# gligen/GLIGEN

Hardware: AMD Instinct MI355X
Metric: 512x512 images/sec @ 50 PLMS steps, box+text (CFG 7.5), UNet step ms (higher is better)
Workload: dtype bf16; 1 GPU; C2: box+text, 8 boxes (30 grounding tokens), 512x512, 50 PLMS steps, CFG 7.5, bf16 storage / fp32 accumulate; plms_steps=50, unet_evals_per_image=102, hipgraph=True, batches_in_flight=3

## Files before the change

gligen_amd/_lib.py:

```python
from __future__ import annotations

import ctypes as C
from pathlib import Path

_HERE = Path(__file__).resolve().parent
LIB_PATH = _HERE / "libgligen_amd.so"


class GligenAmdError(RuntimeError):
    pass


class UNetConfig(C.Structure):
    _fields_ = [
        ("in_channels", C.c_int), ("out_channels", C.c_int), ("model_channels", C.c_int),
        ("num_res_blocks", C.c_int), ("num_heads", C.c_int), ("context_dim", C.c_int),
        ("n_mult", C.c_int), ("channel_mult", C.c_int * 8),
        ("n_attn", C.c_int), ("attention_resolutions", C.c_int * 8),
        ("inpaint_mode", C.c_int), ("grounding_kind", C.c_int),
        ("gr_in_dim", C.c_int), ("gr_out_dim", C.c_int), ("max_persons", C.c_int), ("fuser_kind", C.c_int),
        ("extra_channels", C.c_int), ("tok_resize", C.c_int), ("tok_in_dim", C.c_int),
    ]


# ... 180 lines not shown
    "gl_op_block_train_fuser": (_I, [_P, _I, _P, C.POINTER(_P), _P, _P, _P, _P, _P, _P, _P, _P, C.POINTER(_P), _P]),
    "gl_op_grid_resize": (_I, [_P, _P, _I, _I, _I, _I, _P, _P]),
    "gl_op_grid_resize_backward": (_I, [_P, _P, _I, _I, _I, _I, _P, _P]),
}

_F = C.c_float
TRAIN_PRIM_SYMBOLS = {
    "gl_op_train_attention": (_I, [_P, _I, _I, _I, _I, _I] + [_P] * 9 + [_P]),
    "gl_op_train_linear": (_I, [_P, _I, _I, _I] + [_P] * 8 + [_P]),
    "gl_op_train_layernorm": (_I, [_P, _I, _I, _F, _P, _P, _P, _P, _I] + [_P] * 6 + [_P]),
    "gl_op_train_groupnorm": (_I, [_P, _I, _I, _I, _I, _F, _P, _P, _P, _P, _I] + [_P] * 4 + [_P]),
    "gl_op_train_geglu": (_I, [_P, _I, _I, _P, _P, _P, _P, _P]),
    "gl_op_train_dot": (_I, [_P, C.c_int64, _P, _P, _P, _F, _I, _P, _P]),
}

TRAINER_SYMBOLS = {
    "gl_op_adamw_ema_step": (_I, [_P, _P, _P, _P, _P, _P, C.c_int64, C.c_double, C.c_double, C.c_double, C.c_double, C.c_double, C.c_double, _I, _P]),
}

SAMPLER_SYMBOLS = {
    "gl_set_cfg_shared_prefix": (_I, [_I]),
}

SOLVER_SYMBOLS = {
    "gl_sample_solver": (_I, [_P, C.POINTER(SolverArgs), _P]),
    "gl_op_solver_update": (_I, [_P, _P, _I, C.c_float, C.c_float, _P, _P, _P, _P, _P, _P] + [C.c_float] * 5 + [C.c_int64, _P]),
}


class GemmPlanRecord(C.Structure):
    _fields_ = [("kernel", C.c_char * 96)] + [(n, C.c_int) for n in ("family", "M", "N", "K", "tm", "tn", "splits", "grid", "n_items", "box", "rm", "rz",
                                                                     "units_per_split", "xcd")]


class AttnProjLayout(C.Structure):
    _fields_ = [(n, C.c_int) for n in ("d", "dp", "dpv", "tq", "tk", "tq_pad", "tk_pad", "vt_perm32")]


GEMM_PLAN_SYMBOLS = {
    "gl_gemm_force_plan": (_I, [_I, _I, _I, _I]),
    "gl_gemm_force_knobs": (_I, [_I, _I, _I, _I, _I, _I]),
    "gl_gemm_force_clear": (_I, []),
    "gl_gemm_plan_log_clear": (_I, []),
    "gl_gemm_plan_log": (_I, [C.POINTER(GemmPlanRecord), _I, C.POINTER(_I), C.POINTER(_I)]),
    "gl_op_attention_project": (_I, [_P, _P, _P, _I, _I, _I, _I, _I, _I, _P, _P, _P, _P, _P, _P, C.POINTER(AttnProjLayout), _P]),
}

ATTENTION_CORE_SYMBOLS = {
    "gl_op_attention_core": (_I, [_P, _P, _P, _P, C.POINTER(AttnProjLayout), _I, _I, _I, _I, _P, _I, _I, _I, _P]),
}
ATTN_CORE_KERNELS = {"auto": 0, "attn_kernel": 1, "attn2_kernel_w4": 2, "attn2_kernel_w8": 3, "attn3_kernel": 4}
GL_ERR_UNSUPPORTED = 5

VAE_SYMBOLS = {
    "gl_vae_set_attention": (_I, [_P, _I]),
    "gl_op_vae_attention": (_I, [_P, _P, _P, _P, _I, _I, _I, _I, _P, _P]),
}
VAE_ATTN_MODES = {"auto": 0, "matrix": 1, "flash": 2}

LATENT_SYMBOLS = {
    "gl_op_latent_renoise": (_I, [_P, _P, _I, _I, _I, _I, _P, _I, _I, _I, _F, _F, _P, _I, _P]),
    "gl_latent_resize_taps": (_I, [_I, _I, _I, C.POINTER(_I), C.POINTER(_F)]),
}
LATENT_RESIZE_MODES = {"nearest-exact": 0, "bilinear": 1, "bicubic": 2}

LORA_SYMBOLS = {
    "gl_op_lora_merge": (_I, [_P, _P, _P, _P, _I, _I, _I, _F, _P]),
}

FUSER_KINDS = {"gatedSA": 0, "gatedSA2": 1, "gatedCA": 2}


def fuser_kind(fuser_type) -> int:
    try:
        return FUSER_KINDS[fuser_type or "gatedSA"]
    except KeyError:
        raise ValueError(f"fuser_type {fuser_type!r}: one of {sorted(FUSER_KINDS)}") from None


_lib = None


def load() -> C.CDLL:
    global _lib
    if _lib is not None:
        return _lib
    if not LIB_PATH.exists():
        raise GligenAmdError(
            f"{LIB_PATH} not found: build it with `python -m gligen_amd.build` "
            "(gligen_amd has no fallback path without its HIP library)")
    import torch
    lib = C.CDLL(str(LIB_PATH))
    for name, (res, args) in {**SYMBOLS, **IMAGE_SYMBOLS, **MAP_SYMBOLS, **TRAIN_MAP_SYMBOLS, **TRAIN_INPUT_SYMBOLS, **TRAIN_FUSER_SYMBOLS, **TRAIN_PRIM_SYMBOLS,
                              **TRAINER_SYMBOLS, **SAMPLER_SYMBOLS, **SOLVER_SYMBOLS, **GEMM_PLAN_SYMBOLS, **ATTENTION_CORE_SYMBOLS, **VAE_SYMBOLS, **LATENT_SYMBOLS, **LORA_SYMBOLS}.items():
        fn = getattr(lib, name)
        fn.restype = res
        fn.argtypes = args
    _lib = lib
    return lib


def check(rc: int) -> None:
    if rc != 0:
        msg = load().gl_last_error()
        raise GligenAmdError(f"libgligen_amd error {rc}: {msg.decode() if msg else '?'}")
```

gligen_amd/csrc/capi.hip:

```cpp
#include "classmap.h"
#include "engine_impl.h"
#include "image.h"
#include "latent.h"
#include "lora.h"
#include "train.h"
#include "train_fusers.h"
#include "../../include/gligen_amd_train_maps.h"
#include "../../include/gligen_amd_train_inputs.h"
#include "../../include/gligen_amd_train_fusers.h"
#include "../../include/gligen_amd_train_prims.h"
#include "../../include/gligen_amd_trainer.h"
#include "../../include/gligen_amd_sampler.h"
#include "../../include/gligen_amd_gemm_plans.h"
#include "../../include/gligen_amd_attention_core.h"
#include "../../include/gligen_amd_vae.h"
#include "../../include/gligen_amd_latent.h"
#include "../../include/gligen_amd_lora.h"
#include "gemm_plan.h"

#include <cstdlib>

#include <cmath>

using namespace gl;

struct gl_ctx {
    std::shared_ptr<Engine> holder;
    Engine* eng;
    ImageStage image_stage;
};

#define GL_API_BEGIN try {
#define GL_API_END                                       \
    }                                                    \
    catch (const gl::GlError& e) {                       \
        return gl::set_error(e.code, "%s", e.what());    \
    }                                                    \
    catch (const std::exception& e) {                    \
        return gl::set_error(GL_ERR_STATE, "%s", e.what()); \
    }                                                    \
    return GL_OK;

struct DeviceGuard {
    int prev = -1;
    bool ok = true;
    explicit DeviceGuard(int dev) {
        if (hipGetDevice(&prev) != hipSuccess) prev = -1;
        if (prev != dev) ok = hipSetDevice(dev) == hipSuccess;
        else prev = -1;
    }
    ~DeviceGuard() {
        if (prev >= 0) (void)hipSetDevice(prev);
    }
};
#define NEED(ctx)                                                         \
    if (!(ctx) || !(ctx)->eng) return gl::set_error(GL_ERR_ARG, "null context"); \
    DeviceGuard device_guard_((ctx)->eng->device());                      \
    if (!device_guard_.ok) return gl::set_error(GL_ERR_HIP, "hipSetDevice(%d) failed", (ctx)->eng->device());

static inline hipStream_t S(gl_stream s) { return reinterpret_cast<hipStream_t>(s); }
#define HIPCK_API(expr)                                                                           \
    do {                                                                                          \
        hipError_t _e = (expr);                                                                   \
        if (_e != hipSuccess) throw GlError(GL_ERR_HIP, std::string(#expr) + ": " + hipGetErrorString(_e)); \
    } while (0)

extern "C" {

const char* gl_last_error(void) { return gl::last_error(); }

// ... 1092 lines not shown
        bf16* w4 = ar.get<bf16>((size_t)16 * Cout * Cin);
        const int rp = pack_upconv_phases_launch(w_oihw, w4, Cout, Cin, Cout, S(s));
        if (rp != GL_OK) throw GlError(rp, gl::last_error());
        c.w4 = w4;
        ctx->eng->conv3x3(TRef{(const bf16*)x0, C0, (const bf16*)x1, C1}, B, H, W, c, 1, 1, 1, nullptr, 0, nullptr, S(s), (bf16*)y);
        return GL_OK;
    }
    bf16* wp = ar.get<bf16>((size_t)Cout * 9 * Cin);
    int r = pack_conv_weight_launch(w_oihw, wp, Cout, Cin, 3, 3, Cout, S(s));
    if (r != GL_OK) throw GlError(r, gl::last_error());
    const int Hup = H << ups, Wup = W << ups;
    const int Ho = stride == 1 ? Hup : (pad_lo ? (Hup + 2 - 3) / 2 + 1 : (Hup + 1 - 3) / 2 + 1);
    const int Wo = stride == 1 ? Wup : (pad_lo ? (Wup + 2 - 3) / 2 + 1 : (Wup + 1 - 3) / 2 + 1);
    AOperand A{};
    A.p0 = (const bf16*)x0; A.C0 = C0; A.ld0 = C0; A.p1 = (const bf16*)x1; A.C1 = C1; A.ld1 = C1;
    A.mode = A_CONV3; A.Hin = H; A.Win = W; A.Ho = Ho; A.Wo = Wo; A.stride = stride; A.ups = ups; A.pad_lo = pad_lo;
    Epilogue E;
    epilogue_defaults(E);
    E.out = y; E.ldo = Cout; E.bias = bias; E.res = (const bf16*)res; E.ldres = Cout; E.rows_per_b = Ho * Wo;
    r = gemm_launch(A, wp, B * Ho * Wo, Cout, 9 * Cin, E, ctx->eng->splitk_ws(), ctx->eng->splitk_ws_bytes(), S(s));
    if (r != GL_OK) throw GlError(r, gl::last_error());
    GL_API_END
}

int gl_op_gn_silu_conv3x3(gl_ctx* ctx, const void* x0, int C0, const void* x1, int C1, int B, int H, int W, const float* gamma, const float* beta,
                          float eps, const float* w_oihw, const float* bias, int Cout, const float* bias2, const void* res, void* y, int mode,
                          int* used_prologue, gl_stream s) {
    NEED(ctx);
    if (!x0 || !gamma || !beta || !w_oihw || !y || !used_prologue) return gl::set_error(GL_ERR_ARG, "gl_op_gn_silu_conv3x3: null pointer");
    GL_API_BEGIN
    Engine& eng = *ctx->eng;
    Arena& ar = eng.arena();
    ar.reset();
    const int Cin = C0 + C1;
    bf16* wp = ar.get<bf16>((size_t)Cout * 9 * Cin);
    int r = pack_conv_weight_launch(w_oihw, wp, Cout, Cin, 3, 3, Cout, S(s));
    if (r != GL_OK) throw GlError(r, gl::last_error());
    NormW n;
    n.g = gamma; n.b = beta; n.C = Cin;
    ConvW c;
    c.w = wp; c.b = bias; c.Cin = Cin; c.Cout = Cout;
    const bool saved = eng.gn_prologue_;
    if (mode >= 0) eng.gn_prologue_ = mode != 0;
    const int64_t n0 = eng.n_prologue_convs;
    try {
        eng.gn_silu_conv3x3(TRef{(const bf16*)x0, C0, (const bf16*)x1, C1}, B, H, W, n, eps, c, bias2, Cout, (const bf16*)res, (bf16*)y, S(s));
    } catch (...) {
        eng.gn_prologue_ = saved;
        throw;
    }
    eng.gn_prologue_ = saved;
    *used_prologue = eng.n_prologue_convs > n0 ? 1 : 0;
    if (mode == 1 && !*used_prologue) throw GlError(GL_ERR_UNSUPPORTED, "gl_op_gn_silu_conv3x3: this shape has no GroupNorm prologue (conv_halo_kernel, H W % 256 == 0)");
    GL_API_END
}

int gl_op_groupnorm(gl_ctx* ctx, const void* x0, int C0, const void* x1, int C1, int B, int HW,
                    const float* gamma, const float* beta, float eps, int silu, void* y, gl_stream s) {
    NEED(ctx);
    GL_API_BEGIN
    Arena& ar = ctx->eng->arena();
    ar.reset();
    GNParams P{};
    P.x0 = (const bf16*)x0; P.C0 = C0; P.x1 = (const bf16*)x1; P.C1 = C1; P.B = B; P.HW = HW; P.eps = eps;
    P.gamma = gamma; P.beta = beta; P.y = (bf16*)y; P.silu = silu;
    P.partial = reinterpret_cast<float*>(ar.alloc(gn_partial_bytes(B, HW)));
    int r = groupnorm_launch(P, S(s));
    if (r != GL_OK) throw GlError(r, gl::last_error());
    GL_API_END
}

int gl_op_layernorm(gl_ctx* ctx, const void* x, const void* x2, int B, int N1, int N2, int Tpad, int C,
                    const float* gamma, const float* beta, float eps, void* y, gl_stream s) {
    NEED(ctx);
    GL_API_BEGIN
    LNParams P{};
    P.x = (const bf16*)x; P.x2 = (const bf16*)x2; P.B = B; P.N1 = N1; P.N2 = N2; P.Tpad = Tpad; P.C = C; P.eps = eps;
    P.gamma = gamma; P.beta = beta; P.y = (bf16*)y;
    int r = layernorm_launch(P, S(s));
    if (r != GL_OK) throw GlError(r, gl::last_error());
    GL_API_END
}

static void attention_project(Engine& eng, const void* xq, const void* xkv, int B, int Nq, int Nk, int C, int Ck, int H, const float* wq,
                              const float* wk, const float* wv, bf16* q, bf16* k, bf16* vt, int Tq_pad, int Tk_pad, int dp, int dpv, int vt_layout,
                              hipStream_t s) {
    Arena& ar = eng.arena();
    const int d = C / H, Tq = round_up(Nq, 64), Tk = round_up(Nk, 64);
    bf16* wqb = ar.get<bf16>((size_t)C * C);
    bf16* wkb = ar.get<bf16>((size_t)C * Ck);
    bf16* wvb = ar.get<bf16>((size_t)C * Ck);
    bf16* xqp = ar.get<bf16>((size_t)B * Tq * C);
    bf16* xkp = ar.get<bf16>((size_t)B * Tk * Ck);
    auto ck = [&](int rc) { if (rc != GL_OK) throw GlError(rc, gl::last_error()); };
    ck(cast_f32_bf16_launch(wq, wqb, (int64_t)C * C, s));
    ck(cast_f32_bf16_launch(wk, wkb, (int64_t)C * Ck, s));
    ck(cast_f32_bf16_launch(wv, wvb, (int64_t)C * Ck, s));
    ck(pad_rows_bf16_launch((const bf16*)xq, xqp, B, Nq, Tq, C, s));
    ck(pad_rows_bf16_launch((const bf16*)xkv, xkp, B, Nk, Tk, Ck, s));
    const bool fused = xq == xkv && C == Ck && Nq == Nk && gemm_supports_qkv() && (2 * C) % 128 == 0 &&
                       !(dev_env("GL_QKV_FUSED") && atoi(dev_env("GL_QKV_FUSED")) == 0);
    if (fused) {
        bf16* wqkv = ar.get<bf16>((size_t)3 * C * C);
        ck(cast_f32_bf16_launch(wq, wqkv, (int64_t)C * C, s));
        ck(cast_f32_bf16_launch(wk, wqkv + (size_t)C * C, (int64_t)C * C, s));
        ck(cast_f32_bf16_launch(wv, wqkv + (size_t)2 * C * C, (int64_t)C * C, s));
// ... 159 lines not shown
```

gligen_amd/csrc/engine.h:

```cpp
#pragma once
#include <array>
#include <map>
#include <memory>
#include <stdexcept>
#include <string>
#include <unordered_map>
#include <unordered_set>
#include <vector>

#include "arena.h"
#include "attention.h"
#include "clip.h"
#include "common.h"
#include "convnext.h"
#include "ffn.h"
#include "gemm.h"
#include "misc.h"
#include "norm.h"
#include "train.h"
#include "vae_attention.h"
#include "../../include/gligen_amd.h"
#include "../../include/gligen_amd_solver.h"

namespace gl {
// ... 99 lines not shown
    int sd_conv_step;
};

class Engine {
   public:
    explicit Engine(int device);
    ~Engine();
    static std::shared_ptr<Engine> fork(const std::shared_ptr<Engine>& parent, size_t arena_bytes);
    size_t weight_bytes() const { return persist_bytes_; }
    size_t arena_bytes() const { return arena_.committed(); }
    bool is_fork() const { return (bool)parent_; }

    void upload(const std::string& key, const void* src, int ndim, const int64_t* shape, bool is_device);
    void configure_unet(const gl_unet_config& c);
    void configure_vae(const gl_vae_config& c);
    void configure_clip_text(const gl_clip_text_config& c);
    void configure_clip_vision(const gl_clip_vision_config& c);
    void finalize();
    bool finalized() const { return finalized_; }

    void set_cond(int Beff, const float* context, int n_ctx, const gl_grounding& g, hipStream_t s);
    void set_fuser_scale(float v, hipStream_t s);
    void set_fuser_scales(const float* scales_host, int n, hipStream_t s);
    int n_fusers() const { return (int)unet_.st.size(); }
    void grounding_tokens(float* out, hipStream_t s);
    void spatial_tokens(int B, const float* image, int C, int H, int W, const float* mask, float* out, hipStream_t s);
    void spatial_tokens_classes(int B, const uint8_t* cls, int H, int W, const float* mask, float* out, hipStream_t s);
    int spatial_token_count() const { return unet_.cnx.tokens; }
    void restore_first_conv(const float* w, const float* b, hipStream_t s);
    void unet_forward(int Beff, int h, int w, const float* x, int xB, const int64_t* t, const float* extra,
                      int extraB, float* eps, hipStream_t s, const float* emb_row = nullptr);
    void vae_decode(int B, int h, int w, const float* z, float* out, hipStream_t s);
    void vae_encode(int B, int H, int W, const float* img, const float* noise, float* z, hipStream_t s);
    bool has_vae_encoder() const { return vae_.enc.present; }
    void set_vae_attention(int mode);
    void op_vae_attention(const bf16* q, const bf16* k, const bf16* v, int B, int T, int C, int mode, bf16* o, hipStream_t s);
    void clip_text_encode(const int32_t* ids, const int32_t* eos_index, int S, int T, float* last_hidden, float* pooled, hipStream_t s);
    void clip_vision_encode(const float* pixel_values, int S, float* last_hidden, float* pooled, float* image_embeds, hipStream_t s);
    int clip_vision_tokens() const { const int g = clipv_.cfg.patch ? clipv_.cfg.image_size / clipv_.cfg.patch : 0; return g * g + 1; }
    void sample_plms(const gl_plms_args& a, hipStream_t s);
    void sample_solver(const gl_solver_args& a, hipStream_t s);
    void sampler_timing(float* avg_ms, float* first_ms, int* n);

    Arena& arena() { return arena_; }
    float* splitk_ws() { return ws_; }
    size_t splitk_ws_bytes() const { return ws_bytes_; }
    void* persist(size_t bytes, bool zero);
    void init_workspace();
    AttnBufs& attn_bufs(int B, int H, int d, int Tq, int Tk, int dpv_layout = 0, int slot = 0);
    void attn_regime_counters(int enable, unsigned* out);
    unsigned* attn_counters() const { return attn_counting_ ? attn_ctr_ : nullptr; }

    bf16* gn_silu_conv3x3(const TRef& x, int B, int H, int W, const NormW& n, float eps, const ConvW& c, const float* bias2, int bias2_ld,
                          const bf16* res, bf16* out, hipStream_t s);
    bf16* conv3x3(const TRef& x, int B, int Hin, int Win, const ConvW& c, int stride, int ups, int pad_lo,
                  const float* bias2, int bias2_ld, const bf16* res, hipStream_t s, bf16* out = nullptr);
    static bool upconv_phase_form(int Cin, int Cout);
    bool gn_prologue_ = dev_env("GL_GN_PROLOGUE") && atoi(dev_env("GL_GN_PROLOGUE")) == 1;
    int64_t n_prologue_convs = 0;
    int device() const { return device_; }
    int64_t n_launches = 0;
    static constexpr int kTrainEvents = 64;
    hipEvent_t* train_events();
    bool train_events_recorded = false;
    TrainWeightCache* train_cache = nullptr;

    struct ProfRec { std::string name; int calls = 0; double ms = 0, flops = 0, bytes = 0; };
    void profile_begin();
    std::vector<ProfRec> profile_end(hipStream_t s);

   private:
    struct ProfEvt { std::string name; double flops, bytes; hipEvent_t e0, e1; };
    bool profiling_ = false;
    std::vector<ProfEvt> prof_;
    std::vector<hipEvent_t> prof_pool_;
    struct ProfScope {
        Engine* e; hipStream_t s; size_t idx;
        ProfScope(Engine* eng, hipStream_t st, const std::string& name, double flops, double bytes);
        ~ProfScope();
        void rename(const std::string& n) { if (e->profiling_) e->prof_[idx].name = n; }
    };
    friend struct ProfScope;
    const RawTensor& raw(const std::string& key) const;
    bool has(const std::string& key) const { return raw_.count(key) != 0; }
    const float* F(const std::string& key) const { return raw(key).p; }
    const float* FK(const std::string& key) { keep_raw_.insert(key); return raw(key).p; }
    std::unordered_set<std::string> keep_raw_;
    NormW norm(const std::string& prefix);
    LinW linear(const std::string& prefix, bool bias = true);
    ConvW conv3(const std::string& prefix, int Npad = 0, bool up2x = false);
    ConvW conv3_small(const std::string& prefix, int Cout);
    LinW conv1(const std::string& prefix);
    const bf16* cast_rows(const std::vector<std::string>& weight_keys);
    FFW ffw(const std::string& prefix, int C, const NormW* fold = nullptr, const std::string& pre_key = "", const std::string& post_key = "",
            const float* post_q_w = nullptr, const float* post_q_b = nullptr);
    struct FoldTmp { float* w = nullptr; float* b = nullptr; int N = 0, K = 0; };
    FoldTmp fold_ln(const std::string& weight_key, const float* bias, const NormW& n);
    std::vector<void*> fold_tmps_;
    ResW resw(const std::string& prefix, int Cin, int Cout, bool unet);

    void gemm(const AOperand& A, const bf16* W, int M, int N, int K, const Epilogue& E, hipStream_t s);
    bf16* linear_rows(const bf16* x, int M, const LinW& L, int act, const bf16* res, const float* gate, hipStream_t s, RowStats* stats = nullptr);
    bf16* layernorm_plain(const bf16* x, int B, int N, int C, bool pad64, hipStream_t s);
    bf16* groupnorm(const TRef& x, int B, int HW, const NormW& n, float eps, bool silu, hipStream_t s);
    bf16* layernorm(const bf16* x, int B, int N, int C, const NormW& n, bool pad64, hipStream_t s);
    bf16* conv3x3_small(const ConvW& c, Im2colParams P, int reps, hipStream_t s);
    void gn_silu_conv3x3_nchw(const bf16* x, int C, int B, int H, int W, const NormW& n, float eps, const ConvW& c, int n_real, float* out, hipStream_t s);
    bf16* resblock(const ResW& r, const TRef& x, int B, int H, int W, const float* embout, int emb_ld, float eps, hipStream_t s, bf16* out = nullptr);
    void replicate(const bf16* src, bf16* dst, size_t n, int reps, hipStream_t s);
    void attention(const bf16* q, const bf16* k, const bf16* vt, bf16* o, int B, int H, int d, int Nq, int Nk, int Tq_pad, int Tk_pad, int vt_layout,
                   hipStream_t s);
    void spatial_tokens_tail(int B, const float* img, const float* mask, float* out, hipStream_t s);

    Engine(const Engine&) = default;
    Engine& operator=(const Engine&) = delete;
    std::shared_ptr<Engine> parent_;
    size_t persist_bytes_ = 0;
    int device_;
    bool finalized_ = false;
    std::unordered_map<std::string, RawTensor> raw_;
    std::vector<void*> owned_;
    Arena arena_;
    float* ws_ = nullptr;
    size_t ws_bytes_ = 0;
    typedef std::array<int, 7> AttnKey;
    std::map<AttnKey, AttnBufs> attn_bufs_;
    unsigned* attn_ctr_ = nullptr;
    bool attn_counting_ = false;
    std::vector<hipEvent_t> train_events_;

    struct Unet {
        bool present = false;
        gl_unet_config cfg{};
        LinW te0, te2;
        LinW embcat;
        ConvW conv_in_small;
        std::vector<ResW> res;
        std::vector<STW> st;
        std::vector<ConvW> updown;
        std::vector<UNetBlock> in_blocks, out_blocks;
        UNetBlock mid_block;
        NormW out_norm;
        ConvW out_conv;
        const float* const* alpha_ptrs = nullptr;
        int gkind = 0;
        LinW pn[2][3];
        const float* pn_null_feat[2] = {nullptr, nullptr};
        const float* pn_null_pos = nullptr;
        const float* kp_table = nullptr;
        CnxNet cnx;
    } unet_;
    bool ln_fold_ = false;
    bool ff_rows_ = true;
    int ff_chain_ = 2;
    int qkv_rows_ = 1;
    bool fuser_hoist_ = true;
    void build_unet();
    float* gates_ = nullptr;
    float* fuser_scale_ = nullptr;
    bool fuser_off_ = false;
    struct Cond {
        int Beff = 0, Ng = 0, ctx_T = 0, ctx_Tpad = 0, obj_Tpad = 0;
        bf16* tokens = nullptr;
        int obj_stride = 0;
        std::vector<bf16*> objs;
        std::vector<bf16*> obj_k;
        std::vector<bf16*> obj_vt;
        std::vector<bf16*> ctx_k;
        std::vector<bf16*> ctx_vt;
        std::vector<void*> allocs;
    } cond_;
    void fuser_kv_fill(const STW& t, int B, int HW, hipStream_t s);
    void ensure_fuser_kv(const STW& t, int B, int HW, hipStream_t s);
    struct FuserKV { uint64_t epoch = 0; int B = 0, HW = 0; };
    std::vector<FuserKV> fuser_kv_;
    uint64_t cond_epoch_ = 0;

    bf16* transformer(const STW& t, const bf16* x, int B, int Bp, int H, int W, hipStream_t s);
    bf16* feedforward(const FFW& f, const bf16* ln, int M, const bf16* res, const float* gate, hipStream_t s, const RowStats* in_stats = nullptr,
                      RowStats* out_stats = nullptr, bool raw_rows = false, bool use_rows = false);
    bf16* fuser_ff_tail(const STW& t, const bf16* o, const bf16* t1, int B, int HW, bool rows, hipStream_t s, RowStats* st3, bool* q_done = nullptr);
    AttnBufs& to_q_heads(const LinW& q, const bf16* ln, int B, int Tp, int C, int d, int Tk_pad, const RowStats* st, const float* csum, hipStream_t s);
// ... 107 lines not shown
```

gligen_amd/csrc/engine.hip:

```cpp
#include "engine_impl.h"

#include <algorithm>
#include <cmath>
#include <cstdarg>
#include <cstring>

namespace gl {

static thread_local char g_err[2048] = "";
int set_error(int code, const char* fmt, ...) {
    va_list ap;
    va_start(ap, fmt);
    vsnprintf(g_err, sizeof(g_err), fmt, ap);
    va_end(ap);
    return code;
}
const char* last_error() { return g_err; }

void Arena::init(size_t bytes) {
    off_ = hw_ = 0;
    HIPCK(hipGetDevice(&dev_));
    int vmm = 0;
    const char* sw = dev_env("GL_ARENA_VMM");
    if (!(sw && atoi(sw) == 0) && hipDeviceGetAttribute(&vmm, hipDeviceAttributeVirtualMemoryManagementSupported, dev_) == hipSuccess && vmm) {
// ... 130 lines not shown
    HIPCK(hipStreamSynchronize(s));
    std::vector<ProfRec> out;
    for (auto& pe : prof_) {
        float ms = 0.f;
        HIPCK(hipEventElapsedTime(&ms, pe.e0, pe.e1));
        prof_pool_.push_back(pe.e0);
        prof_pool_.push_back(pe.e1);
        auto it = std::find_if(out.begin(), out.end(), [&](const ProfRec& r) { return r.name == pe.name; });
        if (it == out.end()) { out.push_back(ProfRec{pe.name}); it = out.end() - 1; }
        it->calls += 1; it->ms += ms; it->flops += pe.flops; it->bytes += pe.bytes;
    }
    prof_.clear();
    std::sort(out.begin(), out.end(), [](const ProfRec& a, const ProfRec& b) { return a.ms > b.ms; });
    return out;
}

void Engine::init_workspace() {
    if (ws_) return;
    ws_bytes_ = size_t(256) << 20;
    ws_ = reinterpret_cast<float*>(persist(ws_bytes_, false));
}

void Engine::attn_regime_counters(int enable, unsigned* out) {
    HIPCK(hipDeviceSynchronize());
    if (!attn_ctr_) attn_ctr_ = reinterpret_cast<unsigned*>(persist(ATTN_CTR_N * sizeof(unsigned), true));
    HIPCK(hipMemcpy(out, attn_ctr_, ATTN_CTR_N * sizeof(unsigned), hipMemcpyDeviceToHost));
    HIPCK(hipMemset(attn_ctr_, 0, ATTN_CTR_N * sizeof(unsigned)));
    attn_counting_ = enable != 0;
}

void* Engine::persist(size_t bytes, bool zero) {
    void* p = nullptr;
    HIPCK(hipMalloc(&p, std::max<size_t>(bytes, 256)));
    if (zero) HIPCK(hipMemset(p, 0, std::max<size_t>(bytes, 256)));
    owned_.push_back(p);
    persist_bytes_ += std::max<size_t>(bytes, 256);
    return p;
}

std::shared_ptr<Engine> Engine::fork(const std::shared_ptr<Engine>& parent, size_t arena_bytes) {
    if (!parent || !parent->finalized_) throw GlError(GL_ERR_STATE, "gl_ctx_fork: the parent context is not finalized");
    HIPCK(hipDeviceSynchronize());
    std::shared_ptr<Engine> c(new Engine(*parent));
    Engine& e = *c;
    e.parent_ = parent->parent_ ? parent->parent_ : parent;
    e.owned_.clear();
    e.persist_bytes_ = 0;
    e.fold_tmps_.clear();
    e.arena_ = Arena{};
    e.ws_ = nullptr;
    e.ws_bytes_ = 0;
    e.cond_ = Cond{};
    e.attn_bufs_.clear();
    e.attn_ctr_ = nullptr;
    e.attn_counting_ = false;
    e.smp_ = Sampler{};
    e.train_events_.clear();
    e.fuser_kv_.clear();
    e.emb_table_ = nullptr; e.emb_cur_ = nullptr; e.emb_t_dev_ = nullptr; e.emb_table_cap_ = 0; e.emb_t_cache_.clear();
    e.train_events_recorded = false;
    e.profiling_ = false;
    e.prof_.clear();
    e.prof_pool_.clear();
    e.n_launches = 0;
    try {
        e.arena_.init(arena_bytes ? arena_bytes : parent->arena_.capacity());
        e.init_workspace();
        if (e.unet_.present) {
            const size_t n_st = e.unet_.st.size(), ng = 2 * n_st;
            e.gates_ = reinterpret_cast<float*>(e.persist(std::max<size_t>(ng, 1) * sizeof(float), true));
            e.fuser_scale_ = reinterpret_cast<float*>(e.persist(std::max<size_t>(n_st, 1) * sizeof(float), true));
            if (ng) HIPCK(hipMemcpy(e.gates_, parent->gates_, ng * sizeof(float), hipMemcpyDeviceToDevice));
            if (n_st) HIPCK(hipMemcpy(e.fuser_scale_, parent->fuser_scale_, n_st * sizeof(float), hipMemcpyDeviceToDevice));
            ConvW& c1 = e.unet_.conv_in_small;
            const int mc = e.unet_.cfg.model_channels;
            const size_t wb = (size_t)mc * c1.Kpad * sizeof(bf16);
            bf16* w = reinterpret_cast<bf16*>(e.persist(wb, false));
            float* b = reinterpret_cast<float*>(e.persist(mc * sizeof(float), false));
            HIPCK(hipMemcpy(w, c1.w, wb, hipMemcpyDeviceToDevice));
            HIPCK(hipMemcpy(b, c1.b, mc * sizeof(float), hipMemcpyDeviceToDevice));
            c1.w = w;
            c1.b = b;
        }
    } catch (...) {
        c.reset();
        throw;
    }
    return c;
}

void Engine::upload(const std::string& key, const void* src, int ndim, const int64_t* shape, bool is_device) {
    if (finalized_) throw GlError(GL_ERR_STATE, "weights cannot be uploaded after gl_finalize");
    RawTensor t;
    t.numel = 1;
    for (int i = 0; i < ndim; ++i) {
        t.shape.push_back(shape[i]);
        t.numel *= shape[i];
    }
    HIPCK(hipMalloc(reinterpret_cast<void**>(&t.p), std::max<int64_t>(t.numel, 4) * sizeof(float)));
    HIPCK(hipMemcpy(t.p, src, t.numel * sizeof(float), is_device ? hipMemcpyDeviceToDevice : hipMemcpyHostToDevice));
    auto it = raw_.find(key);
    if (it != raw_.end()) (void)hipFree(it->second.p);
    raw_[key] = t;
}

const RawTensor& Engine::raw(const std::string& key) const {
// ... 176 lines not shown
    return r;
}

void Engine::finalize() {
    if (finalized_) throw GlError(GL_ERR_STATE, "gl_finalize called twice");
    HIPCK(hipSetDevice(device_));
    if (unet_.present) build_unet();
    if (vae_.dec.present) build_vae();
    if (vae_.dec.present && has("vae/encoder.conv_in.weight")) build_vae_encoder();
    if (clipt_.present) build_clip_text();
    if (clipv_.present) build_clip_vision();
    HIPCK(hipDeviceSynchronize());
    for (void* p : fold_tmps_) (void)hipFree(p);
    fold_tmps_.clear();
    for (auto it = raw_.begin(); it != raw_.end();) {
        if (it->second.shape.size() >= 2 && it->first.find("quant_conv") == std::string::npos && !keep_raw_.count(it->first)) {
            (void)hipFree(it->second.p);
            it = raw_.erase(it);
        } else {
            ++it;
        }
    }
    finalized_ = true;
}

FILE* launch_log_file() {
    static FILE* f = dev_env("GL_LAUNCH_LOG") ? fopen(dev_env("GL_LAUNCH_LOG"), "w") : nullptr;
    return f;
}
AttnParams attn_params(const bf16* q, const bf16* k, const bf16* vt, bf16* o, int H, int d, int Nq, int Nk, int Tq_pad, int Tk_pad, int vt_layout) {
    AttnParams P{};
    P.q = q; P.k = k; P.vt = vt; P.o = o;
    P.H = H; P.d = d; P.Nq = Nq; P.Nk = Nk; P.Tq_pad = Tq_pad; P.Tk_pad = Tk_pad;
    P.ldo = H * d; P.o_rows_per_b = Nq; P.vt_layout = vt_layout;
    P.scale_log2e = (float)(1.4426950408889634 / std::sqrt((double)d));
    return P;
}

void Engine::attention(const bf16* q, const bf16* k, const bf16* vt, bf16* o, int B, int H, int d, int Nq, int Nk, int Tq_pad, int Tk_pad, int vt_layout,
                       hipStream_t s) {
    const AttnParams P = attn_params(q, k, vt, o, H, d, Nq, Nk, Tq_pad, Tk_pad, vt_layout);
    const char* sym = attn_kernel_name(d, Nk, vt_layout);
    {
        ProfScope ps(this, s, sym, 4.0 * B * H * (double)Nq * Nk * d, 0.0);
        CK(attn_launch(P, B, s));
        if (FILE* f = launch_log_file()) {
            fprintf(f, "%s|%d|%d|%d|2|%.0f\n", sym, Nq, Nk, d, 2.0 * B * H * d * (2.0 * Nq + 2.0 * Nk));
            fflush(f);
        }
    }
    ++n_launches;
}

void Engine::gemm(const AOperand& A, const bf16* W, int M, int N, int K, const Epilogue& E, hipStream_t s) {
    ProfScope ps(this, s, "gemm", 2.0 * M * N * K, 0.0);
    CK(gemm_launch(A, W, M, N, K, E, ws_, ws_bytes_, s));
    if (profiling_) {
        static const bool by_shape = dev_env("GL_PROF_SHAPES") != nullptr;
        std::string nm = gemm_last_kernel_name();
        if (by_shape) nm += fmt(" M%d N%d K%d", M, N, K);
        ps.rename(nm);
    }
    FILE* launch_log = launch_log_file();
    if (launch_log) {
        const double a_rows = A.mode != A_ROWS ? (double)(M / (A.Ho * A.Wo)) * A.Hin * A.Win : (double)M;
        const double out_b = E.mode == EPI_NCHW_F32 ? 4.0 * M * E.n_real : (E.act == ACT_GEGLU ? 1.0 : 2.0) * M * (double)N * (E.out_f32 ? 2 : 1);
        const double bytes = a_rows * (A.C0 + A.C1) * 2 + (double)N * K * 2 + out_b + (E.res ? 2.0 * M * N : 0.0);
        fprintf(launch_log, "%s|%d|%d|%d|%d|%.0f\n", gemm_last_kernel_name(), M, N, K, A.mode, bytes);
        fflush(launch_log);
    }
    {
        int tm, tn, sp;
        gemm_last_cfg(&tm, &tn, &sp);
        n_launches += sp > 1 ? 2 : 1;
    }
}

bf16* Engine::linear_rows(const bf16* x, int M, const LinW& L, int act, const bf16* res, const float* gate, hipStream_t s, RowStats* stats) {
    bf16* out = arena_.get<bf16>((size_t)M * L.N);
    Epilogue E = e_rows_res(out, L.N, L.b, res);
    E.act = act;
    E.gate = gate;
    if (stats) {
        *stats = RowStats{};
        if (ln_fold_ && L.N % 64 == 0) {
            stats->ld = L.N / 32;
            stats->p = arena_.get<float2>((size_t)M * stats->ld);
            E.stats_out = stats->p;
            E.stats_ld = stats->ld;
        }
    }
    gemm(a_rows(x, L.K), L.w, M, L.N, L.K, E, s);
    if (stats && stats->p) stats->nb = gemm_last_stats_nb();
    return out;
}

bf16* Engine::groupnorm(const TRef& x, int B, int HW, const NormW& n, float eps, bool silu, hipStream_t s) {
    const int C = x.C();
    if (n.C != C) throw GlError(GL_ERR_ARG, fmt("groupnorm: %d channels given to a norm with %d", C, n.C));
    bf16* y = arena_.get<bf16>((size_t)B * HW * C);
    GNParams P{};
    P.x0 = x.p0; P.C0 = x.C0; P.x1 = x.p1; P.C1 = x.C1;
    P.B = B; P.HW = HW; P.eps = eps; P.gamma = n.g; P.beta = n.b; P.y = y; P.silu = silu ? 1 : 0;
    P.partial = reinterpret_cast<float*>(arena_.alloc(gn_partial_bytes(B, HW)));
    ProfScope ps(this, s, HW <= 256 ? "gn_small_kernel" : "gn_stats_kernel + gn_apply_kernel", 0.0, 2.0 * B * HW * (double)C * 2);
    CK(groupnorm_launch(P, s));
    n_launches += HW <= 256 ? 1 : 2;
    return y;
}

bf16* Engine::gn_silu_conv3x3(const TRef& x, int B, int H, int W, const NormW& n, float eps, const ConvW& c, const float* bias2, int bias2_ld,
                              const bf16* res, bf16* out, hipStream_t s) {
    if (x.C() != c.Cin || n.C != c.Cin) throw GlError(GL_ERR_ARG, fmt("gn_silu_conv3x3: %d channels into a norm of %d and a conv of %d", x.C(), n.C, c.Cin));
    const int HW = H * W, M = B * HW;
    if (!out) out = arena_.get<bf16>((size_t)M * c.Cout);
    AOperand A = a_conv3(x, H, W, H, W, 1, 0, 1);
    Epilogue E = e_rows_res(out, c.Cout, c.b, res);
    E.bias2 = bias2; E.bias2_ld = bias2_ld; E.rows_per_b = HW;
    if (gn_prologue_ && gemm_gn_prologue_supported(A, M, c.Cout, 9 * c.Cin, E)) {
        GNParams P{};
        P.x0 = x.p0; P.C0 = x.C0; P.x1 = x.p1; P.C1 = x.C1;
        P.B = B; P.HW = HW; P.eps = eps; P.gamma = n.g; P.beta = n.b; P.silu = 1;
        P.partial = reinterpret_cast<float*>(arena_.alloc(gn_partial_bytes(B, HW)));
        P.coef = reinterpret_cast<float*>(arena_.alloc(gn_coef_bytes(B, c.Cin)));
        {
            const int nl = groupnorm_coef_launches(HW, x.C0, x.C1);
            ProfScope ps(this, s, nl == 1 ? "gn_small_coef_kernel" : "gn_stats_kernel + gn_coef_kernel", 0.0, 1.0 * B * HW * (double)c.Cin * 2);
            CK(groupnorm_coef_launch(P, s));
            n_launches += nl;
        }
        A.gn = P.coef;
        gemm(A, c.w, M, c.Cout, 9 * c.Cin, E, s);
        ++n_prologue_convs;
        return out;
    }
    bf16* a = groupnorm(x, B, HW, n, eps, true, s);
    A.p0 = a; A.C0 = c.Cin; A.ld0 = c.Cin; A.p1 = nullptr; A.C1 = 0; A.ld1 = 0;
    gemm(A, c.w, M, c.Cout, 9 * c.Cin, E, s);
    return out;
}

bf16* Engine::layernorm(const bf16* x, int B, int N, int C, const NormW& n, bool pad64, hipStream_t s) {
    const int Tp = pad64 ? round_up(N, 64) : N;
    bf16* y = arena_.get<bf16>((size_t)B * Tp * C);
    LNParams P{};
    P.x = x; P.x2 = nullptr; P.B = B; P.N1 = N; P.N2 = 0; P.Tpad = Tp; P.C = C; P.eps = 1e-5f;
    P.gamma = n.g; P.beta = n.b; P.y = y;
    ProfScope ps(this, s, "ln_kernel", 0.0, 2.0 * B * N * (double)C * 2);
    CK(layernorm_launch(P, s));
    ++n_launches;
    return y;
}

bf16* Engine::layernorm_plain(const bf16* x, int B, int N, int C, bool pad64, hipStream_t s) {
    NormW none;
    none.C = C;
    return layernorm(x, B, N, C, none, pad64, s);
}

bf16* Engine::conv3x3(const TRef& x, int B, int Hin, int Win, const ConvW& c, int stride, int ups, int pad_lo,
                      const float* bias2, int bias2_ld, const bf16* res, hipStream_t s, bf16* out) {
    if (x.C() != c.Cin) throw GlError(GL_ERR_ARG, fmt("conv3x3: input has %d channels, weight expects %d", x.C(), c.Cin));
    if (c.w4) {
        if (stride != 1 || ups != 1 || pad_lo != 1 || bias2 || res) throw GlError(GL_ERR_ARG, "conv3x3: phase-form weights serve the plain upsample conv only");
        const int Mi = 4 * Hin * Win;
        if (!out) out = arena_.get<bf16>((size_t)B * Mi * c.Cout);
        auto ok = [&](int b) { return gemm_upconv_phases_supported(a_conv2up(x, Hin, Win), b * Mi, c.Cout, 4 * c.Cin, e_rows(out, c.Cout, c.b)); };
        int Bc = B;
        while (Bc > 1 && !ok(Bc)) Bc = (Bc + 1) / 2;
        if (!ok(Bc)) throw GlError(GL_ERR_UNSUPPORTED, fmt("conv3x3: no phase form for a %d x %d x %d -> %d upsample conv", Hin, Win, c.Cin, c.Cout));
        for (int b0 = 0; b0 < B; b0 += Bc) {
            const size_t px = (size_t)b0 * Hin * Win;
            const TRef xb{x.p0 + px * x.C0, x.C0, x.p1 ? x.p1 + px * x.C1 : nullptr, x.C1};
            gemm(a_conv2up(xb, Hin, Win), c.w4, std::min(Bc, B - b0) * Mi, c.Cout, 4 * c.Cin, e_rows(out + (size_t)b0 * Mi * c.Cout, c.Cout, c.b), s);
        }
        return out;
    }
    const int Hup = Hin << ups, Wup = Win << ups;
    const int Ho = stride == 1 ? Hup : (pad_lo ? (Hup + 2 - 3) / 2 + 1 : (Hup + 1 - 3) / 2 + 1);
    const int Wo = stride == 1 ? Wup : (pad_lo ? (Wup + 2 - 3) / 2 + 1 : (Wup + 1 - 3) / 2 + 1);
    const int M = B * Ho * Wo;
    if (!out) out = arena_.get<bf16>((size_t)M * c.Cout);
    Epilogue E = e_rows_res(out, c.Cout, c.b, res);
    E.bias2 = bias2; E.bias2_ld = bias2_ld; E.rows_per_b = Ho * Wo;
    gemm(a_conv3(x, Hin, Win, Ho, Wo, stride, ups, pad_lo), c.w, M, c.Cout, 9 * c.Cin, E, s);
    return out;
}

void Engine::replicate(const bf16* src, bf16* dst, size_t n, int reps, hipStream_t s) {
    ProfScope ps(this, s, "replicate_kernel", 0.0, (1.0 + reps) * n * 2);
    CK(replicate_launch(src, dst, n * sizeof(bf16), reps, s));
    ++n_launches;
}

bf16* Engine::resblock(const ResW& r, const TRef& x, int B, int H, int W, const float* embout, int emb_ld, float eps, hipStream_t s, bf16* out) {
    const int HW = H * W, M = B * HW;
    if (!out) out = arena_.get<bf16>((size_t)M * r.Cout);
    const size_t mk = arena_.mark();
    bf16* h = gn_silu_conv3x3(x, B, H, W, r.n1, eps, r.c1, embout ? embout + r.emb_off : nullptr, emb_ld, nullptr, nullptr, s);
    const bf16* sk;
    if (r.has_skip) {
        bf16* skb = arena_.get<bf16>((size_t)M * r.Cout);
        AOperand A{};
        A.p0 = x.p0; A.C0 = x.C0; A.ld0 = x.C0; A.p1 = x.p1; A.C1 = x.C1; A.ld1 = x.C1; A.mode = A_ROWS;
        gemm(A, r.skip.w, M, r.Cout, r.Cin, e_rows(skb, r.Cout, r.skip.b), s);
        sk = skb;
    } else {
        if (x.p1) throw GlError(GL_ERR_STATE, "identity skip over a concatenated input");
        sk = x.p0;
    }
    gn_silu_conv3x3(TRef{h, r.Cout, nullptr, 0}, B, H, W, r.n2, eps, r.c2, nullptr, 0, sk, out, s);
    arena_.release(mk);
    return out;
}

bf16* Engine::conv3x3_small(const ConvW& c, Im2colParams P, int reps, hipStream_t s) {
    const size_t rows = (size_t)P.B * P.H * P.W;
    bf16* col = arena_.get<bf16>(reps * rows * c.Kpad);
    bf16* out = arena_.get<bf16>(reps * rows * c.Cout);
    P.Kpad = c.Kpad;
    for (int r = 0; r < reps; ++r) {
        P.out = col + r * rows * c.Kpad;
        CK(im2col_small_launch(P, s));
        ++n_launches;
    }
    gemm(a_rows(col, c.Kpad), c.w, (int)(reps * rows), c.Cout, c.Kpad, e_rows(out, c.Cout, c.b), s);
    return out;
}

void Engine::gn_silu_conv3x3_nchw(const bf16* x, int C, int B, int H, int W, const NormW& n, float eps, const ConvW& c, int n_real, float* out, hipStream_t s) {
    const int HW = H * W;
    bf16* a = groupnorm(TRef{x, C, nullptr, 0}, B, HW, n, eps, true, s);
    Epilogue E;
    epilogue_defaults(E);
    E.mode = EPI_NCHW_F32; E.out = out; E.bias = c.b; E.rows_per_b = HW; E.n_real = n_real;
    gemm(a_conv3(TRef{a, C, nullptr, 0}, H, W, H, W, 1, 0, 1), c.w, B * HW, c.Npad, 9 * C, E, s);
}

AttnBufs& Engine::attn_bufs(int B, int H, int d, int Tq, int Tk, int dpv_layout, int slot) {
    const int Tq_pad = round_up(Tq, 128), Tk_pad = round_up(Tk, 64);
    int dp, dpv;
    CK(attn_dims(d, &dp, &dpv));
    if (dpv_layout) dpv = dpv_layout;
    const AttnKey key{{B, H, d, Tq_pad, Tk_pad, dpv, slot}};
    auto it = attn_bufs_.find(key);
    if (it != attn_bufs_.end()) return it->second;
    AttnBufs b;
    b.Tq_pad = Tq_pad;
    b.Tk_pad = Tk_pad;
    b.q = reinterpret_cast<bf16*>(persist((size_t)B * H * Tq_pad * dp * sizeof(bf16), true));
    b.k = reinterpret_cast<bf16*>(persist((size_t)B * H * Tk_pad * dp * sizeof(bf16), true));
    b.vt = reinterpret_cast<bf16*>(persist((size_t)B * H * dpv * Tk_pad * sizeof(bf16), true));
    CK(attn_vt_ones_launch(b.vt, B * H, d, Tk_pad, 0, dpv));
    CK(attn_k_init_launch(b.k, B * H, d, Tk_pad, 0));
    HIPCK(hipStreamSynchronize(0));
    return attn_bufs_.emplace(key, b).first->second;
}

}
```

gligen_amd/csrc/engine_unet.hip:

```cpp
#include "engine_impl.h"
#include <algorithm>
#include <cmath>

namespace gl {

void Engine::configure_unet(const gl_unet_config& c) {
    if (c.n_mult < 1 || c.n_mult > 8 || c.n_attn < 0 || c.n_attn > 8) throw GlError(GL_ERR_ARG, "bad unet config");
    if (c.model_channels % 64 != 0) throw GlError(GL_ERR_UNSUPPORTED, "model_channels must be a multiple of 64");
    if (c.fuser_kind < 0 || c.fuser_kind > 2) throw GlError(GL_ERR_ARG, "fuser_kind: 0 gatedSA, 1 gatedSA2, 2 gatedCA");
    if (c.extra_channels < 0 || c.extra_channels > 64) throw GlError(GL_ERR_ARG, "extra_channels out of range");
    if (c.extra_channels && c.inpaint_mode) throw GlError(GL_ERR_UNSUPPORTED, "inpaint_mode with a grounding downsampler is undefined in the reference");
    unet_.cfg = c;
    unet_.present = true;
}

void Engine::build_unet() {
    const gl_unet_config& c = unet_.cfg;
    const int mc = c.model_channels;
    const std::string U = "unet/";
    auto in_attn = [&](int ds) {
        for (int i = 0; i < c.n_attn; ++i)
            if (c.attention_resolutions[i] == ds) return true;
        return false;
    };
// ... 794 lines not shown
    if ((int)emb_t_cache_.size() == R && std::equal(t_host, t_host + R, emb_t_cache_.begin())) return;
    if (R > emb_table_cap_) {
        const int cap = std::max(R, 64);
        emb_table_ = reinterpret_cast<float*>(persist((size_t)cap * unet_.embcat.N * sizeof(float), false));
        emb_t_dev_ = reinterpret_cast<int64_t*>(persist((size_t)cap * sizeof(int64_t), false));
        if (!emb_cur_) emb_cur_ = reinterpret_cast<float*>(persist((size_t)unet_.embcat.N * sizeof(float), true));
        emb_table_cap_ = cap;
    }
    HIPCK(hipMemcpyAsync(emb_t_dev_, t_host, (size_t)R * sizeof(int64_t), hipMemcpyHostToDevice, s));
    const size_t mk = arena_.mark();
    emb_rows(emb_t_dev_, R, emb_table_, s);
    arena_.release(mk);
    emb_t_cache_.assign(t_host, t_host + R);
}

void Engine::unet_forward(int Beff, int h, int w, const float* x, int xB, const int64_t* t, const float* extra,
                          int extraB, float* eps, hipStream_t s, const float* emb_row) {
    if (!unet_.present || !finalized_) throw GlError(GL_ERR_STATE, "unet not finalized");
    if (cond_.Beff != Beff) throw GlError(GL_ERR_STATE, fmt("unet_forward batch %d but conditioning was set for %d", Beff, cond_.Beff));
    const gl_unet_config& c = unet_.cfg;
    const int extra_C = c.inpaint_mode ? c.in_channels + 1 : c.extra_channels;
    if ((extra_C != 0) != (extra != nullptr))
        throw GlError(GL_ERR_ARG, "the extra first-conv input (inpainting_extra_input / downsampled grounding_extra_input) must be given iff the model has those channels");
    if (xB <= 0 || Beff % xB != 0) throw GlError(GL_ERR_ARG, "x batch must divide the effective batch");
    const int mc = c.model_channels;
    arena_.reset();

    const float* embout = emb_row;
    int emb_ld = 0;
    if (!emb_row) {
        embout = emb_rows(t, Beff, nullptr, s);
        emb_ld = unet_.embcat.N;
        ++n_launches;
    }
    CK(gates_launch(unet_.alpha_ptrs, fuser_scale_, gates_, 2 * (int)unet_.st.size(), s));
    ++n_launches;

    struct Act { bf16* p; int C, H, W; };
    std::vector<Act> hs;
    Act cur{nullptr, 0, h, w};

    int Bp = Beff;
    if (emb_row && Beff / xB > 1 && cfg_shared_prefix()) {
        bool has_st = false;
        for (const UNetBlock& b : unet_.in_blocks)
            for (const Layer& L : b.layers) has_st = has_st || L.kind == L_ST;
        if (has_st) {
            Bp = xB;
            cfg_shared_prefix_note(0);
        }
    }
    bool in_prefix = Bp < Beff;

    auto run_layer = [&](const Layer& L, const TRef& in, int Bl, bool full) {
        PlanAsBatch plan_as(L.kind == L_ST ? 1 : Beff / Bl);
        auto out_for = [&](int HWo, int Co) { return full ? arena_.get<bf16>((size_t)Beff * HWo * Co) : nullptr; };
        auto fill = [&](bf16* o, int HWo, int Co) {
            if (full) replicate(o, o + (size_t)Bl * HWo * Co, (size_t)Bl * HWo * Co, Beff / Bl - 1, s);
        };
        switch (L.kind) {
            case L_CONV_IN: {
                if (extra && extraB != xB) throw GlError(GL_ERR_ARG, "extra first-conv input batch must equal x batch");
                Im2colParams P{};
                P.x0 = x; P.C0 = c.in_channels;
                P.x1 = extra; P.C1 = extra_C;
                P.B = xB; P.H = cur.H; P.W = cur.W;
                cur.p = conv3x3_small(unet_.conv_in_small, P, Beff / xB, s);
                cur.C = mc;
                break;
            }
            case L_RES: {
                const ResW& r = unet_.res[L.idx];
                cur.p = resblock(r, in, Bl, cur.H, cur.W, embout, emb_ld, 1e-5f, s, out_for(cur.H * cur.W, r.Cout));
                cur.C = r.Cout;
                fill(cur.p, cur.H * cur.W, cur.C);
                break;
            }
            case L_ST: {
                if (in.p1) throw GlError(GL_ERR_STATE, "transformer over concatenated input");
                cur.p = transformer(unet_.st[L.idx], in.p0, Beff, Bl, cur.H, cur.W, s);
                break;
            }
            case L_DOWN: {
                const int Ho = (cur.H + 2 - 3) / 2 + 1, Wo = (cur.W + 2 - 3) / 2 + 1;
                cur.p = conv3x3(in, Bl, cur.H, cur.W, unet_.updown[L.idx], 2, 0, 1, nullptr, 0, nullptr, s, out_for(Ho * Wo, unet_.updown[L.idx].Cout));
                cur.H = Ho;
                cur.W = Wo;
                fill(cur.p, Ho * Wo, unet_.updown[L.idx].Cout);
                break;
            }
            case L_UP: {
                cur.p = conv3x3(in, Beff, cur.H, cur.W, unet_.updown[L.idx], 1, 1, 1, nullptr, 0, nullptr, s);
                cur.H *= 2;
                cur.W *= 2;
                break;
            }
        }
    };

    for (const UNetBlock& b : unet_.in_blocks) {
        for (size_t i = 0; i < b.layers.size(); ++i) {
            const Layer& L = b.layers[i];
            const bool pre = in_prefix && L.kind != L_CONV_IN;
            const bool last = i + 1 == b.layers.size();
            run_layer(L, TRef{cur.p, cur.C, nullptr, 0}, pre ? Bp : Beff, pre && L.kind != L_ST && (last || b.layers[i + 1].kind == L_ST));
            if (L.kind == L_ST) in_prefix = false;
        }
// ... 19 lines not shown
```

gligen_amd/csrc/engine_vae.hip:

```cpp
#include "engine_impl.h"
#include <cmath>

namespace gl {

void Engine::configure_vae(const gl_vae_config& c) {
    if (c.n_mult < 1 || c.n_mult > 8) throw GlError(GL_ERR_ARG, "bad vae config");
    vae_.cfg = c;
    vae_.dec.present = true;
}

void Engine::build_vae_mid(VaeHalf& h, const std::string& p, int C) {
    h.mid1 = resw(p + ".block_1", C, C, false);
    h.mid2 = resw(p + ".block_2", C, C, false);
    h.attn.gn = norm(p + ".attn_1.norm");
    h.attn.q = conv1(p + ".attn_1.q");
    h.attn.k = conv1(p + ".attn_1.k");
    h.attn.v = conv1(p + ".attn_1.v");
    h.attn.proj = conv1(p + ".attn_1.proj_out");
}

void Engine::build_vae() {
    const gl_vae_config& c = vae_.cfg;
    const std::string V = "vae/";
    vae_.dec.quant_w = F(V + "post_quant_conv.weight");
// ... 85 lines not shown
    const size_t mk = arena_.mark();
    bf16* n = groupnorm(TRef{x, C, nullptr, 0}, B, HW, a.gn, 1e-6f, false, s);
    bf16* q = linear_rows(n, M, a.q, ACT_NONE, nullptr, nullptr, s);
    bf16* k = linear_rows(n, M, a.k, ACT_NONE, nullptr, nullptr, s);
    bf16* o = arena_.get<bf16>((size_t)M * C);
    if (vae_attn_flash_for(vae_attn_mode_, HW, C, (size_t)C * HW * sizeof(bf16))) {
        bf16* vT = arena_.get<bf16>((size_t)M * C);
        for (int b = 0; b < B; ++b) gemm(a_rows(a.v.w, C), n + (size_t)b * HW * C, C, HW, C, e_rows(vT + (size_t)b * HW * C, HW), s);
        ProfScope ps(this, s, "vae_attn_flash_kernel", 4.0 * B * HW * HW * C, 0.0);
        CK(vae_attn_flash_launch(q, k, vT, a.v.b, o, B, HW, C, s));
        ++n_launches;
    } else {
        for (int b = 0; b < B; ++b) {
            const size_t mb = arena_.mark();
            bf16* vT = arena_.get<bf16>((size_t)C * HW);
            gemm(a_rows(a.v.w, C), n + (size_t)b * HW * C, C, HW, C, e_rows(vT, HW), s);
            vae_attn_matrix(q + (size_t)b * HW * C, k + (size_t)b * HW * C, vT, a.v.b, o + (size_t)b * HW * C, HW, C, s);
            arena_.release(mb);
        }
    }
    gemm(a_rows(o, C), a.proj.w, M, C, C, e_rows_res(out, C, a.proj.b, x), s);
    arena_.release(mk);
    return out;
}

void Engine::op_vae_attention(const bf16* q, const bf16* k, const bf16* v, int B, int T, int C, int mode, bf16* o, hipStream_t s) {
    if (mode < 0 || mode > 2) throw GlError(GL_ERR_ARG, fmt("vae attention mode %d: 0 = auto, 1 = score matrices, 2 = flash", mode));
    if (B <= 0 || T <= 0 || T % 64 || C <= 0 || C % 64)
        throw GlError(GL_ERR_UNSUPPORTED, fmt("vae attention: B=%d T=%d C=%d (T and C positive multiples of 64)", B, T, C));
    const size_t mk = arena_.mark();
    struct Release {
        Arena& ar;
        size_t mk;
        ~Release() { ar.release(mk); }
    } release{arena_, mk};
    const bool flash = vae_attn_flash_for(mode, T, C, (size_t)B * T * C * sizeof(bf16));
    bf16* vT = arena_.get<bf16>((size_t)B * T * C);
    CK(vae_attn_transpose_launch(v, vT, B, T, C, s));
    ++n_launches;
    if (flash) {
        CK(vae_attn_flash_launch(q, k, vT, nullptr, o, B, T, C, s));
        ++n_launches;
        return;
    }
    const size_t img = (size_t)T * C;
    for (int b = 0; b < B; ++b) {
        const size_t mb = arena_.mark();
        vae_attn_matrix(q + b * img, k + b * img, vT + b * img, nullptr, o + b * img, T, C, s);
        arena_.release(mb);
    }
}

void Engine::vae_decode(int B, int h, int w, const float* z, float* out, hipStream_t s) {
    if (!vae_.dec.present || !finalized_) throw GlError(GL_ERR_STATE, "vae not finalized");
    const gl_vae_config& c = vae_.cfg;
    arena_.reset();
    int H = h, W = w;
    int C = vae_.dec.in_small.Cout;
    Im2colParams P{};
    P.x0 = z; P.C0 = c.z_channels; P.B = B; P.H = H; P.W = W;
    P.pre_w = vae_.dec.quant_w; P.pre_b = vae_.dec.quant_b; P.pre_scale = 1.f / c.scale_factor;
    bf16* cur = conv3x3_small(vae_.dec.in_small, P, 1, s);
    const float eps = 1e-6f;
    cur = resblock(vae_.dec.mid1, TRef{cur, C, nullptr, 0}, B, H, W, nullptr, 0, eps, s);
    cur = vae_attn(vae_.dec.attn, cur, B, H * W, s);
    cur = resblock(vae_.dec.mid2, TRef{cur, C, nullptr, 0}, B, H, W, nullptr, 0, eps, s);
    for (int level = c.n_mult - 1; level >= 0; --level) {
        for (const ResW& r : vae_.dec.levels[level].blocks) {
            cur = resblock(r, TRef{cur, C, nullptr, 0}, B, H, W, nullptr, 0, eps, s);
            C = r.Cout;
        }
        if (vae_.dec.levels[level].has_resample) {
            cur = conv3x3(TRef{cur, C, nullptr, 0}, B, H, W, vae_.dec.levels[level].resample, 1, 1, 1, nullptr, 0, nullptr, s);
            H *= 2;
            W *= 2;
        }
    }
    gn_silu_conv3x3_nchw(cur, C, B, H, W, vae_.dec.norm_out, eps, vae_.dec.conv_out, c.out_ch, out, s);
}

void Engine::vae_encode(int B, int H, int W, const float* img, const float* noise, float* z, hipStream_t s) {
    if (!vae_.enc.present || !finalized_) throw GlError(GL_ERR_STATE, "vae encoder weights were not uploaded / not finalized");
    const gl_vae_config& c = vae_.cfg;
    const int total_stride = 1 << (c.n_mult - 1);
    if (H % total_stride || W % total_stride) throw GlError(GL_ERR_ARG, "vae_encode: image size must be divisible by the encoder stride");
    arena_.reset();
    int C = vae_.enc.in_small.Cout;
    Im2colParams P{};
    P.x0 = img; P.C0 = vae_.enc.in_small.Cin; P.B = B; P.H = H; P.W = W;
    P.pre_scale = 1.f;
    bf16* cur = conv3x3_small(vae_.enc.in_small, P, 1, s);
    const float eps = 1e-6f;
    for (int level = 0; level < c.n_mult; ++level) {
        for (const ResW& r : vae_.enc.levels[level].blocks) {
            cur = resblock(r, TRef{cur, C, nullptr, 0}, B, H, W, nullptr, 0, eps, s);
            C = r.Cout;
        }
        if (vae_.enc.levels[level].has_resample) {
            cur = conv3x3(TRef{cur, C, nullptr, 0}, B, H, W, vae_.enc.levels[level].resample, 2, 0, 0, nullptr, 0, nullptr, s);
            H /= 2;
            W /= 2;
        }
    }
    cur = resblock(vae_.enc.mid1, TRef{cur, C, nullptr, 0}, B, H, W, nullptr, 0, eps, s);
    cur = vae_attn(vae_.enc.attn, cur, B, H * W, s);
    cur = resblock(vae_.enc.mid2, TRef{cur, C, nullptr, 0}, B, H, W, nullptr, 0, eps, s);
    const int HW = H * W;
    float* moments = arena_.get<float>((size_t)B * 2 * c.z_channels * HW);
    gn_silu_conv3x3_nchw(cur, C, B, H, W, vae_.enc.norm_out, eps, vae_.enc.conv_out, 2 * c.z_channels, moments, s);
    CK(vae_posterior_launch(moments, vae_.enc.quant_w, vae_.enc.quant_b, noise, z, B, c.z_channels, HW, c.scale_factor, s));
    ++n_launches;
}

}
```

gligen_amd/csrc/gemm.h:

```cpp
#pragma once
#include "common.h"

namespace gl {

enum { A_ROWS = 0, A_CONV3 = 1, A_CONV2UP = 2 };

struct AOperand {
    const bf16* p0;
    const bf16* p1;
    int C0, C1;
    int ld0, ld1;
    int mode;
    int Hin, Win, Ho, Wo;
    int stride, ups, pad_lo;
    const float* gn = nullptr;
};

enum { EPI_ROWMAJOR = 0, EPI_QK_HEADS = 1, EPI_VT_HEADS = 2, EPI_NCHW_F32 = 3, EPI_QKV_HEADS = 4 };
enum { ACT_NONE = 0, ACT_SILU = 1, ACT_GEGLU = 2, ACT_GELU = 3, ACT_QUICK_GELU = 4 };

struct Epilogue {
    int mode;
    int act;
    void* out;
    int ldo;
    int out_f32;
    const float* bias;
    const float* bias2;
    int bias2_ld;
    int rows_per_b;
    unsigned rpb_magic;
    int rpb_shift;
    const bf16* res;
    int ldres;
    const float* gate;
    bf16* q;
    bf16* k;
    int q_tiled;
    int C, H, d, DP, T;
    int Tpad_q, Tpad_k;
    bf16* vt;
    int DPV;
    int tok_off;
    int vt_perm32;
    int n_real;
    int remap_in, remap_out, remap_off;
    int up_win;
    int geglu16;
    float2* stats_out;
    int stats_ld;
    const float2* ln_stats;
    int ln_nb, ln_ld;
    const float* ln_csum;
    float ln_inv_c, ln_eps;
};

__host__ __device__ inline size_t ktile_off(size_t bh, int tpad, int t, int dd, int DP) {
    return (bh * (size_t)tpad + (size_t)(t & ~63)) * DP + (size_t)(dd >> 3) * 512 + (size_t)(t & 63) * 8 + (dd & 7);
}

int gemm_launch(const AOperand& A, const bf16* W, int M, int N, int K, const Epilogue& E,
                float* ws, size_t ws_bytes, hipStream_t stream);

int gemm_launch_t(const bf16* Wrows, int Mw, const bf16* X, int Nx, int K, const Epilogue& E,
                  hipStream_t stream);

void epilogue_defaults(Epilogue& E);
bool gemm_supports_qkv();
void gemm_set_variant(int v);
int gemm_geglu_layout();
void gemm_force_cfg(int tm, int tn, int splits);
void gemm_force_grid(int blocks);
void gemm_set_autotune(int on);
void gemm_set_no_split(int on);
void gemm_set_plan_batch_scale(int scale);
void gemm_last_cfg(int* tm, int* tn, int* splits);
const char* gemm_last_kernel_name();
bool gemm_gn_prologue_supported(const AOperand& A, int M, int N, int K, const Epilogue& E);
bool gemm_upconv_phases_supported(const AOperand& A, int M, int N, int K, const Epilogue& E);
bool gemm_ln_fold_supported(const AOperand& A, int M, int N, int K, const Epilogue& E);
int gemm_last_stats_nb();
void aoperand_rows(AOperand& A, const bf16* p, int K, int ld);

}
```

gligen_amd/csrc/gemm.hip:

```cpp
#include "gemm_plan.h"

#include <algorithm>
#include <climits>
#include <cstdio>
#include <cstdlib>
#include <cstring>
#include <type_traits>

namespace gl {

void epilogue_defaults(Epilogue& E) {
    E = Epilogue{};
    E.mode = EPI_ROWMAJOR;
    E.act = ACT_NONE;
    E.rows_per_b = 1;
    E.rpb_magic = 1; E.rpb_shift = 0;
}

void aoperand_rows(AOperand& A, const bf16* p, int K, int ld) {
    A = AOperand{};
    A.p0 = p;
    A.C0 = K;
    A.ld0 = ld;
    A.mode = A_ROWS;
}

__device__ __forceinline__ int perm_tok4(int t0, int p32 = 0) {
    if (p32) {
        const int g = (t0 >> 2) & 7;
        return (t0 & ~31) | ((((g & 1) << 2) | (g >> 1)) << 2);
    }
    int g = (t0 >> 2) & 3;
    int gp = ((g & 1) << 1) | (g >> 1);
    return (t0 & ~15) | (gp << 2);
}

__device__ __forceinline__ void store_bf16x4(bf16* dst, const float v[4]) {
    U2BF4 o;
    o.e[0] = f2bf(v[0]);
    o.e[1] = f2bf(v[1]);
    o.e[2] = f2bf(v[2]);
    o.e[3] = f2bf(v[3]);
    *reinterpret_cast<uint2*>(dst) = o.u;
}

__device__ __forceinline__ int div_rpb(const Epilogue& E, int m) {
    return (int)((__umulhi((unsigned)m, E.rpb_magic) + (unsigned)m) >> E.rpb_shift);
}

__device__ __forceinline__ void epi_finish4(const Epilogue& E, int m, int n0, float v[4]) {
    if (E.bias) {
        float4 b = *reinterpret_cast<const float4*>(E.bias + n0);
        v[0] += b.x; v[1] += b.y; v[2] += b.z; v[3] += b.w;
    }
    if (E.bias2) {
        int bb = div_rpb(E, m);
        float4 b = *reinterpret_cast<const float4*>(E.bias2 + (size_t)bb * E.bias2_ld + n0);
        v[0] += b.x; v[1] += b.y; v[2] += b.z; v[3] += b.w;
    }
    if (E.act == ACT_SILU) {
#pragma unroll
        for (int i = 0; i < 4; ++i) v[i] = silu_f(v[i]);
    } else if (E.act == ACT_GELU) {
#pragma unroll
        for (int i = 0; i < 4; ++i) v[i] = gelu_erf_f(v[i]);
    } else if (E.act == ACT_QUICK_GELU) {
#pragma unroll
        for (int i = 0; i < 4; ++i) v[i] = quick_gelu_f(v[i]);
    }
    switch (E.mode) {
        case EPI_ROWMAJOR: {
            if (E.remap_in) m = (m / E.remap_in) * E.remap_out + (m % E.remap_in) + E.remap_off;
            if (E.res) {
                U2BF4 r;
                r.u = *reinterpret_cast<const uint2*>(E.res + (size_t)m * E.ldres + n0);
                float g = E.gate ? *E.gate : 1.f;
#pragma unroll
                for (int i = 0; i < 4; ++i) v[i] = bf2f(r.e[i]) + g * v[i];
            }
            if (E.out_f32) {
                float4 o = make_float4(v[0], v[1], v[2], v[3]);
                *reinterpret_cast<float4*>(reinterpret_cast<float*>(E.out) + (size_t)m * E.ldo + n0) = o;
            } else {
                store_bf16x4(reinterpret_cast<bf16*>(E.out) + (size_t)m * E.ldo + n0, v);
            }
            break;
        }
        case EPI_QKV_HEADS:
        case EPI_QK_HEADS: {
            int which = n0 >= E.C;
            int c = n0 - which * E.C;
            int h = c / E.d;
            int dd = c - h * E.d;
            int b = m / E.T;
            int t = m - b * E.T + E.tok_off;
            int tp = which ? E.Tpad_k : E.Tpad_q;
            bf16* base = which ? E.k : E.q;
            const size_t off = (which || E.q_tiled) ? ktile_off((size_t)(b * E.H + h), tp, t, dd, E.DP) : ((size_t)(b * E.H + h) * tp + t) * E.DP + dd;
            store_bf16x4(base + off, v);
            break;
        }
        case EPI_VT_HEADS: {
            int h = m / E.d;
            int dd = m - h * E.d;
            int b = n0 / E.T;
            int t0 = n0 - b * E.T + E.tok_off;
            bf16* base = reinterpret_cast<bf16*>(E.out);
            store_bf16x4(base + ((size_t)(b * E.H + h) * E.DPV + dd) * E.Tpad_k + perm_tok4(t0, E.vt_perm32), v);
            break;
        }
        case EPI_NCHW_F32: {
            int b = div_rpb(E, m);
            int pix = m - b * E.rows_per_b;
            float* o = reinterpret_cast<float*>(E.out);
#pragma unroll
            for (int i = 0; i < 4; ++i)
                if (n0 + i < E.n_real) o[((size_t)b * E.n_real + n0 + i) * E.rows_per_b + pix] = v[i];
            break;
        }
    }
}

template <bool WITH_GELU = true>
__device__ __forceinline__ void epi_store4(const Epilogue& E, int m, int n0, float v[4]) {
    if (E.act == ACT_SILU) {
#pragma unroll
        for (int i = 0; i < 4; ++i) v[i] = silu_f(v[i]);
    } else if (WITH_GELU && E.act == ACT_GELU) {
#pragma unroll
        for (int i = 0; i < 4; ++i) v[i] = gelu_erf_f(v[i]);
    } else if (WITH_GELU && E.act == ACT_QUICK_GELU) {
#pragma unroll
        for (int i = 0; i < 4; ++i) v[i] = quick_gelu_f(v[i]);
    }
    switch (E.mode) {
        case EPI_ROWMAJOR: {
            if (E.out_f32) {
                float4 o = make_float4(v[0], v[1], v[2], v[3]);
                *reinterpret_cast<float4*>(reinterpret_cast<float*>(E.out) + (size_t)m * E.ldo + n0) = o;
            } else {
                store_bf16x4(reinterpret_cast<bf16*>(E.out) + (size_t)m * E.ldo + n0, v);
            }
            break;
        }
        case EPI_QKV_HEADS:
        case EPI_QK_HEADS: {
            int which = n0 >= E.C;
            int c = n0 - which * E.C;
            int h = c / E.d;
            int dd = c - h * E.d;
            int b = m / E.T;
            int t = m - b * E.T + E.tok_off;
            int tp = which ? E.Tpad_k : E.Tpad_q;
            bf16* base = which ? E.k : E.q;
            const size_t off = (which || E.q_tiled) ? ktile_off((size_t)(b * E.H + h), tp, t, dd, E.DP) : ((size_t)(b * E.H + h) * tp + t) * E.DP + dd;
            store_bf16x4(base + off, v);
            break;
        }
        case EPI_VT_HEADS: {
            int h = m / E.d;
            int dd = m - h * E.d;
            int b = n0 / E.T;
            int t0 = n0 - b * E.T + E.tok_off;
            bf16* base = reinterpret_cast<bf16*>(E.out);
            store_bf16x4(base + ((size_t)(b * E.H + h) * E.DPV + dd) * E.Tpad_k + perm_tok4(t0, E.vt_perm32), v);
            break;
        }
        case EPI_NCHW_F32: {
            int b = div_rpb(E, m);
            int pix = m - b * E.rows_per_b;
            float* o = reinterpret_cast<float*>(E.out);
#pragma unroll
            for (int i = 0; i < 4; ++i)
                if (n0 + i < E.n_real) o[((size_t)b * E.n_real + n0 + i) * E.rows_per_b + pix] = v[i];
            break;
        }
    }
}

__device__ __forceinline__ void epi_geglu4(const Epilogue& E, int m, int nv0, float val[4], float gate[4]) {
    if (E.bias) {
        float4 bv = *reinterpret_cast<const float4*>(E.bias + nv0);
        float4 bg = *reinterpret_cast<const float4*>(E.bias + nv0 + 8);
        val[0] += bv.x; val[1] += bv.y; val[2] += bv.z; val[3] += bv.w;
        gate[0] += bg.x; gate[1] += bg.y; gate[2] += bg.z; gate[3] += bg.w;
    }
    int j0 = (nv0 >> 5) * 16 + ((nv0 & 31) >> 4) * 8 + (nv0 & 7);
    float o[4];
#pragma unroll
    for (int i = 0; i < 4; ++i) o[i] = val[i] * gelu_erf_f(gate[i]);
    store_bf16x4(reinterpret_cast<bf16*>(E.out) + (size_t)m * E.ldo + j0, o);
}

template <int TM, int TN>
__device__ __forceinline__ void gemm_epilogue(f32x16 (&acc)[TM][TN], const Epilogue& E, int M, int N, int m0, int n0w,
                                              float* __restrict__ ws) {
    const bool split = gridDim.z > 1;
#pragma unroll
    for (int i = 0; i < TM; ++i) {
        const int m = m0 + i * 32;
        if (m >= M) continue;
#pragma unroll
        for (int j = 0; j < TN; ++j) {
            const int nb = n0w + j * 32;
            if (split) {
                float* dst = ws + ((size_t)blockIdx.z * M + m) * N;
#pragma unroll
                for (int q = 0; q < 4; ++q) {
                    int n0 = nb + 8 * q;
                    if (n0 < N)
                        *reinterpret_cast<float4*>(dst + n0) =
                            make_float4(acc[i][j][4 * q], acc[i][j][4 * q + 1], acc[i][j][4 * q + 2], acc[i][j][4 * q + 3]);
                }
            } else if (E.act == ACT_GEGLU) {
#pragma unroll
                for (int qq = 0; qq < 2; ++qq) {
                    int nv0 = nb + 16 * qq;
                    if (nv0 < N) {
                        float val[4], gate[4];
#pragma unroll
                        for (int e = 0; e < 4; ++e) {
                            val[e] = acc[i][j][8 * qq + e];
                            gate[e] = acc[i][j][8 * qq + 4 + e];
                        }
                        epi_geglu4(E, m, nv0, val, gate);
                    }
                }
            } else {
#pragma unroll
                for (int q = 0; q < 4; ++q) {
                    int n0 = nb + 8 * q;
                    if (n0 < N) {
                        float v[4];
#pragma unroll
                        for (int e = 0; e < 4; ++e) v[e] = acc[i][j][4 * q + e];
                        epi_finish4(E, m, n0, v);
                    }
                }
            }
        }
    }
}

__device__ uint4 g_zero_chunk[8];

#define GL_GLDS16(gsrc, ldst)                                                                      \
    __builtin_amdgcn_global_load_lds((const __attribute__((address_space(1))) void*)(gsrc),       \
                                     (__attribute__((address_space(3))) void*)(ldst), 16, 0, 0)

template <int WM, int WN, int TM, int TN, int AMODE>
__global__ void __launch_bounds__(WM * WN * 64)
gemm_glds_kernel(AOperand A, const bf16* __restrict__ W, int M, int N, int K, Epilogue E,
                 float* __restrict__ ws, int kt_per_split, int tiles_n, int n_tiles) {
    constexpr int NT = WM * WN * 64;
    constexpr int BM = WM * TM * 32;
    constexpr int BN = WN * TN * 32;
    constexpr int RPP = NT / 8;
    constexpr int XP = BM / RPP;
    constexpr int WP = BN / RPP;
    static_assert(BM % RPP == 0 && BN % RPP == 0 && RPP % 16 == 0, "tile/loader mismatch");
    constexpr int STAGE = (BM + BN) * 128;

    extern __shared__ __attribute__((aligned(16))) unsigned char smem[];

    const int t = threadIdx.x;
    const int lane = t & 63;
    const int wave = __builtin_amdgcn_readfirstlane(t >> 6);
    const int wm = wave / WN;
    const int wn = wave % WN;
    const int r0 = t >> 3;
    const int ch8 = ((t & 7) ^ ((r0 >> 1) & 7)) * 8;

    int bid = blockIdx.x;
    {
        const int q = n_tiles >> 3, r = n_tiles & 7, xcd = bid & 7, idx = bid >> 3;
        bid = (xcd < r ? xcd * (q + 1) : r * (q + 1) + (xcd - r) * q) + idx;
    }
    const int tile_m = bid / tiles_n;
    const int tile_n = bid - tile_m * tiles_n;
    const int m_base = tile_m * BM;
    const int n_base = tile_n * BN;

    const int nk = K >> 6;
    const int kt0 = blockIdx.z * kt_per_split;
    const int kt1 = min(nk, kt0 + kt_per_split);

    const bf16* zsrc = reinterpret_cast<const bf16*>(g_zero_chunk);

    int64_t xo0[XP], xo1[XP];
    int xb[XP], xy[XP], xx[XP];
    bool xv[XP];
#pragma unroll
    for (int i = 0; i < XP; ++i) {
        int m = m_base + r0 + i * RPP;
        xv[i] = m < M;
        if constexpr (AMODE == A_ROWS) {
            xo0[i] = (int64_t)m * A.ld0;
            xo1[i] = (int64_t)m * A.ld1;
            xb[i] = xy[i] = xx[i] = 0;
        } else {
            int ox = m % A.Wo;
            int tmp = m / A.Wo;
            int oy = tmp % A.Ho;
            xb[i] = (tmp / A.Ho) * A.Hin;
            xy[i] = oy * A.stride - A.pad_lo;
// ... 57 lines not shown
            for (int r = 0; r < 16; ++r) acc[i][j][r] = 0.f;

    const int frow = lane & 31;
    const int fhalf = lane >> 5;

    auto compute = [&](int buf) {
        const unsigned char* xs = smem + buf * STAGE;
        const unsigned char* wsm = xs + BM * 128;
        auto ldfrag = [&](int s, bf16x8 (&xf)[TM], bf16x8 (&wf)[TN]) {
            const int c = 2 * s + fhalf;
#pragma unroll
            for (int i = 0; i < TM; ++i) {
                int row = (wm * TM + i) * 32 + frow;
                xf[i] = *reinterpret_cast<const bf16x8*>(xs + row * 128 + ((c ^ ((row >> 1) & 7)) << 4));
            }
#pragma unroll
            for (int j = 0; j < TN; ++j) {
                int row = (wn * TN + j) * 32 + frow;
                wf[j] = *reinterpret_cast<const bf16x8*>(wsm + row * 128 + ((c ^ ((row >> 1) & 7)) << 4));
            }
        };
        auto mma = [&](const bf16x8 (&xf)[TM], const bf16x8 (&wf)[TN]) {
#pragma unroll
            for (int i = 0; i < TM; ++i)
#pragma unroll
                for (int j = 0; j < TN; ++j)
                    acc[i][j] = __builtin_amdgcn_mfma_f32_32x32x16_bf16(wf[j], xf[i], acc[i][j], 0, 0, 0);
        };
        bf16x8 xa[TM], wa[TN], xb2[TM], wb2[TN];
        ldfrag(0, xa, wa);
        ldfrag(1, xb2, wb2);
        mma(xa, wa);
        ldfrag(2, xa, wa);
        mma(xb2, wb2);
        ldfrag(3, xb2, wb2);
        mma(xa, wa);
        mma(xb2, wb2);
    };

    if (kt0 < kt1) {
        issue(kt0, 0);
        for (int kt = kt0; kt < kt1; ++kt) {
            const int buf = (kt - kt0) & 1;
            asm volatile("s_waitcnt vmcnt(0)" ::: "memory");
            __syncthreads();
            if (kt + 1 < kt1) issue(kt + 1, buf ^ 1);
            compute(buf);
        }
    }

    gemm_epilogue<TM, TN>(acc, E, M, N, m_base + wm * TM * 32 + frow, n_base + wn * TN * 32 + 4 * fhalf, ws);
}

__device__ __forceinline__ void epi_geglu4_t16(const Epilogue& E, int m, int nv0, float val[4], float gate[4]) {
    if (E.bias) {
        float4 bv = *reinterpret_cast<const float4*>(E.bias + nv0);
        float4 bg = *reinterpret_cast<const float4*>(E.bias + nv0 + 16);
        val[0] += bv.x; val[1] += bv.y; val[2] += bv.z; val[3] += bv.w;
        gate[0] += bg.x; gate[1] += bg.y; gate[2] += bg.z; gate[3] += bg.w;
    }
    const int j0 = (nv0 >> 5) * 16 + (nv0 & 15);
    float o[4];
#pragma unroll
    for (int i = 0; i < 4; ++i) o[i] = val[i] * gelu_erf_f(gate[i]);
    store_bf16x4(reinterpret_cast<bf16*>(E.out) + (size_t)m * E.ldo + j0, o);
}

template <int TM, int TN, int AMODE>
__global__ void __launch_bounds__(256, 2)
gemm_p_kernel(AOperand A, const bf16* __restrict__ W, int M, int N, int K, Epilogue E, float* __restrict__ ws, WorkDesc wd) {
    constexpr int BM = TM * 32;
    constexpr int BN = TN * 32;
    constexpr int XP = BM / 32;
    constexpr int WP = BN / 32;
    constexpr int STAGE = (BM + BN) * 128;

    extern __shared__ __attribute__((aligned(16))) unsigned char smem[];

    const int t = threadIdx.x;
    const int lane = t & 63;
    const int wave = __builtin_amdgcn_readfirstlane(t >> 6);
    const int wm = wave >> 1;
    const int wn = wave & 1;
    const int r0 = t >> 3;
    const int ch8 = ((t & 7) ^ ((r0 >> 1) & 7)) * 8;
    const int nk = K >> 6;
    const bf16* zsrc = reinterpret_cast<const bf16*>(g_zero_chunk);
    const int Cin = A.C0 + A.C1;
    const int Hup = A.Hin << A.ups;
    const int Wup = A.Win << A.ups;

    auto decode = [&](int w, int& tm, int& tn, int& z) {
        const int q = wd.n_items >> 3, r = wd.n_items & 7, xcd = w & 7, idx = w >> 3;
        const int id = (xcd < r ? xcd * (q + 1) : r * (q + 1) + (xcd - r) * q) + idx;
        const int tile = id / wd.splits;
        z = id - tile * wd.splits;
        tm = tile / wd.tiles_n;
        tn = tile - tm * wd.tiles_n;
    };

    int l_item = blockIdx.x, l_kt = 0, l_kt_end = 0;
    int xm[XP], xy[XP], xx[XP];
    int wrow[WP];
    auto setup_load = [&](int item) {
        int tm, tn, z;
        decode(item, tm, tn, z);
        l_kt = z * wd.kt_per_split;
        l_kt_end = min(nk, l_kt + wd.kt_per_split);
#pragma unroll
        for (int i = 0; i < XP; ++i) {
            const int m = tm * BM + r0 + i * 32;
            const bool ok = m < M;
            if constexpr (AMODE == A_ROWS) {
                xm[i] = ok ? m : -1;
                xy[i] = xx[i] = 0;
            } else {
                const int ox = m % A.Wo;
                const int tmp = m / A.Wo;
                const int oy = tmp % A.Ho;
                xm[i] = (tmp / A.Ho) * A.Hin;
                xy[i] = ok ? oy * A.stride - A.pad_lo : -(1 << 20);
                xx[i] = ox * A.stride - A.pad_lo;
            }
// ... 97 lines not shown
                        make_float4(acc[i][j][0], acc[i][j][1], acc[i][j][2], acc[i][j][3]);
                } else if (E.act == ACT_GEGLU) {
                    if constexpr (TN % 2 == 0) {
                        if ((j & 1) == 0) {
                            float val[4], gate[4];
#pragma unroll
                            for (int e = 0; e < 4; ++e) {
                                val[e] = acc[i][j][e];
                                gate[e] = acc[i][j + 1 < TN ? j + 1 : j][e];
                            }
                            epi_geglu4_t16(E, m, n0, val, gate);
                        }
                    }
                } else {
                    float v[4];
#pragma unroll
                    for (int e = 0; e < 4; ++e) v[e] = acc[i][j][e];
                    epi_finish4(E, m, n0, v);
                }
            }
        }
    };

    if (l_item >= wd.n_items) return;
    setup_load(l_item);
    int c_item = l_item, c_tm, c_tn, c_z;
    decode(c_item, c_tm, c_tn, c_z);
    int c_left = l_kt_end - l_kt;
    issue(l_kt, 0);
    int buf = 0;
    for (;;) {
        asm volatile("s_waitcnt vmcnt(0)" ::: "memory");
        __syncthreads();
        bool more = true;
        if (++l_kt >= l_kt_end) {
            l_item += gridDim.x;
            more = l_item < wd.n_items;
            if (more) setup_load(l_item);
        }
        if (more) issue(l_kt, buf ^ 1);
        compute(buf);
        buf ^= 1;
        if (--c_left == 0) {
            epilogue(c_tm, c_tn, c_z);
            c_item += gridDim.x;
            if (c_item >= wd.n_items) break;
            zero_acc();
            decode(c_item, c_tm, c_tn, c_z);
            c_left = min(nk, (c_z + 1) * wd.kt_per_split) - c_z * wd.kt_per_split;
        }
    }
}

template <int OFF>
__device__ __forceinline__ void lds_rd16(bf16x8& d, unsigned addr) {
    asm volatile("ds_read_b128 %0, %1 offset:%2" : "=v"(d) : "v"(addr), "n"(OFF));
}
template <int N, int STRIDE, int I = 0>
__device__ __forceinline__ void lds_rd16_n(bf16x8 (&d)[N], unsigned addr) {
    if constexpr (I < N) {
        lds_rd16<I * STRIDE>(d[I], addr);
        lds_rd16_n<N, STRIDE, I + 1>(d, addr);
    }
}
__device__ __forceinline__ void epi_ready(float4& v) { asm volatile("" : "+v"(v.x), "+v"(v.y), "+v"(v.z), "+v"(v.w)); }
template <int N>
__device__ __forceinline__ void pin_regs(bf16x8 (&d)[N]) {
#pragma unroll
    for (int i = 0; i < N; ++i) asm volatile("" : "+v"(d[i]));
}

#define GL_BLDS16(rsrc, ldst, voff, soff)                                                                   \
    __builtin_amdgcn_raw_ptr_buffer_load_lds(rsrc, (__attribute__((address_space(3))) void*)(ldst), 16, \
                                             (int)(voff), (int)(soff), 0, 0)

template <int WMW, int TM, int TN, int AMODE, int NST, bool QKV = false>
__global__ void __launch_bounds__(WMW * 128, 2)
gemm_u_kernel(AOperand A, const bf16* __restrict__ W, int M, int N, int K, Epilogue E, float* __restrict__ ws, WorkDesc wd) {
    constexpr int NT = WMW * 128;
    constexpr int RPP = NT / 8;
    constexpr int BM = WMW * TM * 16;
    constexpr int BN = TN * 32;
    constexpr int XP = BM / RPP;
    constexpr int WP = BN / RPP;
    constexpr int STAGE = (BM + BN) * 128;
    constexpr unsigned SENT = 0x80000000u;
    constexpr bool UP = AMODE == A_CONV2UP;
    constexpr int TAPW = UP ? 2 : 3;
    static_assert(WMW == 2 && NST == 2, "one geometry: 4 waves, two LDS stages (deeper rings and the 8-wave form lost every A/B, DESIGN.md section 4)");
    static_assert(BM % RPP == 0 && BN % RPP == 0, "tile/loader mismatch");

    extern __shared__ __attribute__((aligned(16))) unsigned char smem[];

    const int t = threadIdx.x;
    const int lane = t & 63;
    const int wave = __builtin_amdgcn_readfirstlane(t >> 6);
    const int wm = wave >> 1;
    const int wn = wave & 1;
    const int r0 = t >> 3;
    const unsigned chb = (((t & 7) ^ ((r0 >> 1) & 7)) * 16);
    const int nk = K >> 6;
    const int Cin = A.C0 + A.C1;
    const int Hup = UP ? A.Hin : A.Hin << A.ups;
    const int Wup = UP ? A.Win : A.Win << A.ups;
    const int MP = UP ? M >> 2 : M;
    const int TPP = (MP + BM - 1) / BM;

    const __amdgpu_buffer_rsrc_t ra0 = __builtin_amdgcn_make_buffer_rsrc((void*)A.p0, 0, 0x80000000u, 0x00020000);
    const __amdgpu_buffer_rsrc_t ra1 = __builtin_amdgcn_make_buffer_rsrc((void*)(A.p1 ? A.p1 : A.p0), 0, 0x80000000u, 0x00020000);
    const __amdgpu_buffer_rsrc_t rw = __builtin_amdgcn_make_buffer_rsrc((void*)W, 0, 0x80000000u, 0x00020000);

    auto decode = [&](int w, int& tm, int& tn, int& z) {
        const int xcd = w & 7, idx = w >> 3;
        int id = idx;
        if (wd.box < 0) {
            const int q = wd.n_items >> 3, r = wd.n_items & 7;
            id += xcd < r ? xcd * (q + 1) : r * (q + 1) + (xcd - r) * q;
        }
        const int tile = id / wd.rz;
        z = id - tile * wd.rz;
        tm = tile / wd.tiles_n;
        tn = tile - tm * wd.tiles_n;
        if (wd.box >= 0) {
            const int lgm = wd.box & 15, lgn = wd.box >> 4;
            z += (xcd >> (lgm + lgn)) * wd.rz;
            tn += ((xcd >> lgm) & ((1 << lgn) - 1)) * wd.tiles_n;
            tm += (xcd & ((1 << lgm) - 1)) * wd.rm;
        }
    };

    int l_item = blockIdx.x, l_kt = 0, l_kt_end = 0;
// ... 623 lines not shown
                    __builtin_amdgcn_wave_barrier();
                }
            }
        }
        };
        if (E.res) rows(std::true_type{});
        else rows(std::false_type{});
        return true;
    };

    if (l_item >= wd.n_items) return;
    setup_load(l_item);
    int c_item = l_item, c_tm, c_tn, c_z;
    decode(c_item, c_tm, c_tn, c_z);
    bool c_swap = QKV && c_tn * BN >= 2 * E.C;
    if constexpr (QKV) {
        if (E.ln_stats) ln_fetch(c_tm);
    }
    int c_left = l_kt_end - l_kt;
    int slot_c = 0;
    if (more) issue_next(slot_c);
    for (;;) {
        c_left = __builtin_amdgcn_readfirstlane(c_left);
        slot_c = __builtin_amdgcn_readfirstlane(slot_c);
        more = __builtin_amdgcn_readfirstlane((int)more) != 0;
        __builtin_amdgcn_s_waitcnt(0x0F70);
        __builtin_amdgcn_s_barrier();
        asm volatile("" ::: "memory");
        if (more) issue_next(slot_c ^ 1);
        compute(slot_c, c_swap);
        const int slot_done = slot_c;
        slot_c ^= 1;
        if (--c_left == 0) {
            if constexpr (QKV) {
                const float2* lst = E.ln_stats ? ln_prepare(c_tm, slot_done) : nullptr;
                if (c_swap) epilogue_vt(c_tm, c_tn, lst);
                else epilogue_qk(c_tm, c_tn, lst);
            } else {
                if (!epilogue_staged(c_tm, c_tn, slot_done)) epilogue(c_tm, c_tn, c_z);
            }
            c_item += gridDim.x;
            if (c_item >= wd.n_items) break;
            zero_acc();
            decode(c_item, c_tm, c_tn, c_z);
            c_swap = QKV && c_tn * BN >= 2 * E.C;
            if constexpr (QKV) {
                if (E.ln_stats) ln_fetch(c_tm);
            }
            c_left = min(nk, (c_z + 1) * wd.kt_per_split) - c_z * wd.kt_per_split;
        }
    }
}

__device__ __forceinline__ float2 ln_row_stats(const Epilogue& E, int m) {
    float s = 0.f, q = 0.f;
    for (int nb = 0; nb < E.ln_nb; ++nb) {
        const float2 v = E.ln_stats[(size_t)m * E.ln_ld + nb];
        s += v.x; q += v.y;
    }
    const float mean = s * E.ln_inv_c;
    const float var = fmaxf(q * E.ln_inv_c - mean * mean, 0.f);
    return make_float2(mean, rsqrtf(var + E.ln_eps));
}

__global__ void __launch_bounds__(256)
splitk_reduce_kernel(const float* __restrict__ ws, int splits, int M, int N, Epilogue E) {
    const int groups = N >> 2;
    const int64_t total = (int64_t)M * groups;
    for (int64_t idx = (int64_t)blockIdx.x * blockDim.x + threadIdx.x; idx < total;
         idx += (int64_t)gridDim.x * blockDim.x) {
        int m = (int)(idx / groups);
        int n0 = (int)(idx - (int64_t)m * groups) << 2;
        if (E.act == ACT_GEGLU && E.geglu16) {
            if (n0 & 16) continue;
            float val[4] = {0, 0, 0, 0}, gate[4] = {0, 0, 0, 0};
            for (int z = 0; z < splits; ++z) {
                const float* p = ws + ((size_t)z * M + m) * N + n0;
                float4 a = *reinterpret_cast<const float4*>(p);
                float4 b = *reinterpret_cast<const float4*>(p + 16);
                val[0] += a.x; val[1] += a.y; val[2] += a.z; val[3] += a.w;
                gate[0] += b.x; gate[1] += b.y; gate[2] += b.z; gate[3] += b.w;
            }
            epi_geglu4_t16(E, m, n0, val, gate);
        } else if (E.act == ACT_GEGLU) {
            if (n0 & 8) continue;
            float val[4] = {0, 0, 0, 0}, gate[4] = {0, 0, 0, 0};
            for (int z = 0; z < splits; ++z) {
                const float* p = ws + ((size_t)z * M + m) * N + n0;
                float4 a = *reinterpret_cast<const float4*>(p);
                float4 b = *reinterpret_cast<const float4*>(p + 8);
                val[0] += a.x; val[1] += a.y; val[2] += a.z; val[3] += a.w;
                gate[0] += b.x; gate[1] += b.y; gate[2] += b.z; gate[3] += b.w;
            }
            epi_geglu4(E, m, n0, val, gate);
        } else {
            const bool fast = E.mode == EPI_ROWMAJOR && !E.out_f32 && !E.remap_in && E.act != ACT_GELU && E.act != ACT_QUICK_GELU && !E.ln_stats;
            const float4 pb = *reinterpret_cast<const float4*>((fast && E.bias) ? E.bias + n0 : ws);
            const float4 pb2 = *reinterpret_cast<const float4*>((fast && E.bias2) ? E.bias2 + (size_t)div_rpb(E, m) * E.bias2_ld + n0 : ws);
            const uint2 pr = *reinterpret_cast<const uint2*>((fast && E.res) ? reinterpret_cast<const void*>(E.res + (size_t)m * E.ldres + n0)
                                                                              : reinterpret_cast<const void*>(ws));
            const float pg = *((fast && E.res && E.gate) ? E.gate : ws);
            float v[4] = {0, 0, 0, 0};
            const float* p0 = ws + (size_t)m * N + n0;
            const size_t zs = (size_t)M * N;
            for (int z = 0; z < splits; z += 4) {
                float4 a[4];
#pragma unroll
                for (int u = 0; u < 4; ++u) a[u] = *reinterpret_cast<const float4*>(p0 + (size_t)min(z + u, splits - 1) * zs);
#pragma unroll
                for (int u = 0; u < 4; ++u) {
                    const bool ok = z + u < splits;
                    v[0] += ok ? a[u].x : 0.f; v[1] += ok ? a[u].y : 0.f; v[2] += ok ? a[u].z : 0.f; v[3] += ok ? a[u].w : 0.f;
                }
            }
            if (E.ln_stats) {
                const float2 st = ln_row_stats(E, m);
                const float4 cs = *reinterpret_cast<const float4*>(E.ln_csum + n0);
                v[0] = st.y * (v[0] - st.x * cs.x); v[1] = st.y * (v[1] - st.x * cs.y);
                v[2] = st.y * (v[2] - st.x * cs.z); v[3] = st.y * (v[3] - st.x * cs.w);
            }
            if (fast) {
                if (E.bias) { v[0] += pb.x; v[1] += pb.y; v[2] += pb.z; v[3] += pb.w; }
                if (E.bias2) { v[0] += pb2.x; v[1] += pb2.y; v[2] += pb2.z; v[3] += pb2.w; }
                if (E.act == ACT_SILU) {
#pragma unroll
                    for (int i = 0; i < 4; ++i) v[i] = silu_f(v[i]);
                }
                if (E.res) {
                    U2BF4 r;
                    r.u = pr;
                    const float g = E.gate ? pg : 1.f;
#pragma unroll
                    for (int i = 0; i < 4; ++i) v[i] = bf2f(r.e[i]) + g * v[i];
                }
                int mo = m;
                if (E.up_win) {
                    const int mp = M >> 2, ph = m / mp, r = m - ph * mp, q = div_rpb(E, r);
                    mo = ((2 * q + (ph >> 1)) * E.up_win + (r - q * E.up_win)) * 2 + (ph & 1);
                }
                store_bf16x4(reinterpret_cast<bf16*>(E.out) + (size_t)mo * E.ldo + n0, v);
            } else {
                epi_finish4(E, m, n0, v);
            }
        }
    }
}

template <int TN, int NW, bool GN = false>
__global__ void __launch_bounds__(NW * 64, 1)
conv_halo_kernel(AOperand A, const bf16* __restrict__ W, int M, int N, int K, Epilogue E, float* __restrict__ ws, HaloDesc hd) {
    constexpr int NT = NW * 64;
    constexpr int RPP = NT / 8;
    constexpr int TM = 32 / NW;
    constexpr int BM = 256;
    constexpr int BN = TN * 32;
    constexpr int HROWS = 448;
    constexpr int HPASS = HROWS / RPP;
    constexpr int HPT = (HPASS + 6) / 7;
    constexpr int HBUF = HROWS * 128;
    constexpr int WSLOT = BN * 128;
    constexpr int WP = (BN + RPP - 1) / RPP;
    constexpr int WREM = BN % RPP;
    constexpr unsigned SENT = 0x80000000u;
    constexpr int COEF0 = 2 * HBUF + 2 * WSLOT;
    static_assert(HPASS * RPP == HROWS && HPT * 7 >= HPASS && WREM % 8 == 0, "loader geometry");
    static_assert(!GN || (HPT == 1 && HPASS == 7), "the prologue rewrites pass p of the next chunk during tap p + 1");

    extern __shared__ __attribute__((aligned(16))) unsigned char smem[];

    const int t = threadIdx.x;
    const int lane = t & 63;
    const int wave = __builtin_amdgcn_readfirstlane(t >> 6);
    const int wm = wave >> 1;
    const int wn = wave & 1;
    const int l15 = lane & 15;
    const int q = lane >> 4;
    const int r0 = t >> 3;
    const unsigned chb = (((t & 7) ^ ((r0 >> 1) & 7)) * 16);
    const unsigned chb_h = (((t & 7) ^ (r0 & 6)) * 16);
    const int Cin = A.C0 + A.C1;

    const int Wd = 1 << hd.lgW, Hd = 1 << hd.lgH;
    const int R = BM >> hd.lgW;
    const int lgHB = min(hd.lgH, 8 - hd.lgW);
    const int HB = 1 << lgHB;
    const int W2 = Wd + 2;
    const int blkrows = (HB + 2) * W2;
    const int NH = (R >> lgHB) * blkrows;

    const __amdgpu_buffer_rsrc_t ra0 = __builtin_amdgcn_make_buffer_rsrc((void*)A.p0, 0, 0x80000000u, 0x00020000);
    const __amdgpu_buffer_rsrc_t ra1 = __builtin_amdgcn_make_buffer_rsrc((void*)(A.p1 ? A.p1 : A.p0), 0, 0x80000000u, 0x00020000);
    const __amdgpu_buffer_rsrc_t rw = __builtin_amdgcn_make_buffer_rsrc((void*)W, 0, 0x80000000u, 0x00020000);

    const unsigned inv_w2 = ((1u << 22) + W2 - 1) / W2, inv_blk = ((1u << 22) + blkrows - 1) / blkrows;
    int hr00;
    {
        const int p = wm * TM * 16 + l15;
        const int blk = p >> (lgHB + hd.lgW);
        const int yl = (p >> hd.lgW) & (HB - 1);
        const int x = p & (Wd - 1);
        hr00 = blk * blkrows + yl * W2 + x;
    }
    auto hr_delta = [&](int i) -> int {
        const int px = i * 16;
        return (px >> hd.lgW) * W2 + (px & (Wd - 1));
    };
    const int foff0 = l15 * 128 + (((q) ^ (l15 >> 1)) << 4);
    const int foff1 = l15 * 128 + (((q + 4) ^ (l15 >> 1)) << 4);
    const int wrow0 = wn * TN * 16 * 128;
    const unsigned lds0 = (unsigned)(uintptr_t)(__attribute__((address_space(3))) unsigned char*)smem;

    int m0 = 0, c_tn = 0, c_z = 0;
    bool top_ok = false, bot_ok = false;
    unsigned vw0 = SENT;
    auto setup = [&](int item) {
        const int tile = item / hd.splits;
        c_z = item - tile * hd.splits;
// ... 127 lines not shown
#pragma unroll
            for (int j = 0; j < TN; ++j)
                acc[i][j] = __builtin_amdgcn_mfma_f32_16x16x32_bf16(wa[j], xa[i], acc[i][j], 0, 0, 0);
        asm volatile("s_waitcnt lgkmcnt(0)");
        pin_regs(xb);
        pin_regs(wb);
        __builtin_amdgcn_sched_barrier(0);
#pragma unroll
        for (int i = 0; i < TM; ++i)
#pragma unroll
            for (int j = 0; j < TN; ++j)
                acc[i][j] = __builtin_amdgcn_mfma_f32_16x16x32_bf16(wb[j], xb[i], acc[i][j], 0, 0, 0);
    };

    bf16x8 xbp[TM], wbp[TN];
    auto k1_mfma = [&](auto LO, auto HI) {
#pragma unroll
        for (int ij = decltype(LO)::value; ij < decltype(HI)::value; ++ij)
            acc[ij / TN][ij % TN] = __builtin_amdgcn_mfma_f32_16x16x32_bf16(wbp[ij % TN], xbp[ij / TN], acc[ij / TN][ij % TN], 0, 0, 0);
    };
    auto compute_k0 = [&](int tapoff, int hb, int wsl) {
        const unsigned hbase = lds0 + hb * HBUF;
        const unsigned wbase = lds0 + 2 * HBUF + wsl * WSLOT + wrow0;
        unsigned ax0[TM], ax1[TM];
#pragma unroll
        for (int i = 0; i < TM; ++i) {
            const unsigned hr = (unsigned)(hr00 + hr_delta(i) + tapoff);
            ax0[i] = hbase + hr * 128u + (((unsigned)q ^ (hr & 6u)) << 4);
            ax1[i] = ax0[i] ^ 64u;
        }
        const unsigned aw0 = wbase + foff0, aw1 = wbase + foff1;
        bf16x8 xa[TM], wa[TN];
#pragma unroll
        for (int i = 0; i < TM; ++i) lds_rd16<0>(xa[i], ax0[i]);
        lds_rd16_n<TN, 2048>(wa, aw0);
#pragma unroll
        for (int i = 0; i < TM; ++i) lds_rd16<0>(xbp[i], ax1[i]);
        lds_rd16_n<TN, 2048>(wbp, aw1);
        asm volatile("s_waitcnt lgkmcnt(%0)" ::"n"(TM + TN));
        pin_regs(xa);
        pin_regs(wa);
        __builtin_amdgcn_sched_barrier(0);
#pragma unroll
        for (int i = 0; i < TM; ++i)
#pragma unroll
            for (int j = 0; j < TN; ++j)
                acc[i][j] = __builtin_amdgcn_mfma_f32_16x16x32_bf16(wa[j], xa[i], acc[i][j], 0, 0, 0);
        asm volatile("s_waitcnt lgkmcnt(0)");
        pin_regs(xbp);
        pin_regs(wbp);
        __builtin_amdgcn_sched_barrier(0);
    };

    auto store_row = [&](int m, int n0, float (&v)[4]) {
        if (E.act == ACT_SILU) {
#pragma unroll
            for (int e = 0; e < 4; ++e) v[e] = silu_f(v[e]);
        }
        if (E.out_f32) *reinterpret_cast<float4*>(reinterpret_cast<float*>(E.out) + (size_t)m * E.ldo + n0) = make_float4(v[0], v[1], v[2], v[3]);
        else store_bf16x4(reinterpret_cast<bf16*>(E.out) + (size_t)m * E.ldo + n0, v);
    };
    auto epilogue = [&]() {
        const int mrow = m0 + wm * TM * 16 + l15;
        const int ncol = c_tn * BN + wn * TN * 16 + q * 4;
        if (hd.splits > 1) {
#pragma unroll
            for (int i = 0; i < TM; ++i) {
                const int m = mrow + i * 16;
#pragma unroll
                for (int j = 0; j < TN; ++j) {
                    const int n0 = ncol + j * 16;
                    *reinterpret_cast<float4*>(ws + ((size_t)c_z * M + m) * N + n0) =
                        make_float4(acc[i][j][0], acc[i][j][1], acc[i][j][2], acc[i][j][3]);
                }
            }
            return;
        }
        float4 bj[TN];
#pragma unroll
        for (int j = 0; j < TN; ++j) {
            bj[j] = make_float4(0.f, 0.f, 0.f, 0.f);
            if (E.bias) bj[j] = *reinterpret_cast<const float4*>(E.bias + ncol + j * 16);
        }
        if (E.bias2) {
#pragma unroll
            for (int i = 0; i < TM; ++i) {
                const int m = mrow + i * 16;
                const float* b2p = E.bias2 + (size_t)div_rpb(E, m) * E.bias2_ld + ncol;
                float4 b2[TN];
#pragma unroll
                for (int j = 0; j < TN; ++j) b2[j] = *reinterpret_cast<const float4*>(b2p + j * 16);
#pragma unroll
                for (int j = 0; j < TN; ++j) {
                    float v[4] = {acc[i][j][0] + bj[j].x + b2[j].x, acc[i][j][1] + bj[j].y + b2[j].y,
                                  acc[i][j][2] + bj[j].z + b2[j].z, acc[i][j][3] + bj[j].w + b2[j].w};
                    store_row(m, ncol + j * 16, v);
                }
            }
        } else if (E.res) {
            const float g = E.gate ? *E.gate : 1.f;
#pragma unroll
            for (int i = 0; i < TM; ++i) {
                const int m = mrow + i * 16;
                uint2 rs[TN];
#pragma unroll
                for (int j = 0; j < TN; ++j) rs[j] = *reinterpret_cast<const uint2*>(E.res + (size_t)m * E.ldres + ncol + j * 16);
#pragma unroll
                for (int j = 0; j < TN; ++j) {
                    const int n0 = ncol + j * 16;
                    U2BF4 r;
                    r.u = rs[j];
                    float v[4] = {acc[i][j][0] + bj[j].x, acc[i][j][1] + bj[j].y, acc[i][j][2] + bj[j].z, acc[i][j][3] + bj[j].w};
                    if (E.act == ACT_SILU) {
#pragma unroll
                        for (int e = 0; e < 4; ++e) v[e] = silu_f(v[e]);
                    }
#pragma unroll
                    for (int e = 0; e < 4; ++e) v[e] = bf2f(r.e[e]) + g * v[e];
                    if (E.out_f32) {
                        *reinterpret_cast<float4*>(reinterpret_cast<float*>(E.out) + (size_t)m * E.ldo + n0) = make_float4(v[0], v[1], v[2], v[3]);
                    } else {
                        store_bf16x4(reinterpret_cast<bf16*>(E.out) + (size_t)m * E.ldo + n0, v);
                    }
                }
            }
        } else {
#pragma unroll
            for (int i = 0; i < TM; ++i) {
                const int m = mrow + i * 16;
#pragma unroll
                for (int j = 0; j < TN; ++j) {
                    float v[4] = {acc[i][j][0] + bj[j].x, acc[i][j][1] + bj[j].y, acc[i][j][2] + bj[j].z, acc[i][j][3] + bj[j].w};
                    store_row(m, ncol + j * 16, v);
                }
            }
        }
    };

    int item = blockIdx.x;
    if (item >= hd.n_items) return;
    int hb = 0, wsl = 0;
    int cc = 0, cc_end = 0;
    auto begin_item = [&](int it) {
        setup(it);
        cc = c_z * hd.chunks_per_split * 64;
        cc_end = min(Cin, cc + hd.chunks_per_split * 64);
#pragma unroll
        for (int p = 0; p < HPASS; ++p) issue_halo(p, cc, hb);
        issue_coef(cc, hb);
        issue_w(0, cc, wsl);
    };
    begin_item(item);
    zero_acc();
    for (;;) {
        hb = __builtin_amdgcn_readfirstlane(hb);
        wsl = __builtin_amdgcn_readfirstlane(wsl);
        cc = __builtin_amdgcn_readfirstlane(cc);
        cc_end = __builtin_amdgcn_readfirstlane(cc_end);
        const bool next_chunk = cc + 64 < cc_end;
        auto one_tap = [&](auto TC) {
            constexpr int tap = decltype(TC)::value;
            __builtin_amdgcn_s_waitcnt(0x0F70);
            bool first_chunk = false;
            if constexpr (GN) {
                first_chunk = tap == 0 && cc == c_z * hd.chunks_per_split * 64;
                if (tap == 0 && first_chunk) {
                    __builtin_amdgcn_s_barrier();
                    XF x;
                    xf_coef(hb, x);
#pragma unroll 1
                    for (int p = 0; p < HPASS; ++p) {
                        XP1 pc;
                        xf_piece(std::integral_constant<int, 0>{}, p, hb, 0, pc);
                        xf_wait(x, pc);
                        xf_write(std::integral_constant<int, 0>{}, pc, xf_math(x, pc));
                    }
                    asm volatile("s_waitcnt lgkmcnt(0)");
                }
            }
            __builtin_amdgcn_s_barrier();
            asm volatile("" ::: "memory");
            if (tap < 8) issue_w(tap + 1, cc, wsl ^ 1);
            else if (next_chunk) issue_w(0, cc + 64, wsl ^ 1);
            if (tap < 7 && next_chunk) {
#pragma unroll
                for (int pp = 0; pp < HPT; ++pp)
                    if (tap * HPT + pp < HPASS) issue_halo(tap * HPT + pp, cc + 64, hb ^ 1);
                if (tap == 0) issue_coef(cc + 64, hb ^ 1);
            }
            if constexpr (GN) {
                constexpr int NMF = TM * TN, HALF = NMF / 2;
                using I0 = std::integral_constant<int, 0>;
                using IH = std::integral_constant<int, HALF>;
                using IN = std::integral_constant<int, NMF>;
                constexpr int PX = (tap >= 1 && tap <= HPASS) ? tap - 1 : -1;
                if (PX >= 0 && next_chunk) {
                    constexpr int PXC = PX >= 0 ? PX : 0;
                    XF x;
                    XP1 p1;
                    xf_piece(std::integral_constant<int, PXC>{}, 0, hb ^ 1, 0, p1);
                    xf_coef(hb ^ 1, x);
                    k1_mfma(I0{}, IH{});
                    xf_wait(x, p1);
                    const u32x4 o = xf_math(x, p1);
                    k1_mfma(IH{}, IN{});
#pragma unroll
                    for (int g = 0; g < NMF - HALF; ++g) {
                        __builtin_amdgcn_sched_group_barrier(0x008, 1, 0);
                        __builtin_amdgcn_sched_group_barrier(0x002, 8, 0);
                    }
                    xf_write(std::integral_constant<int, PXC>{}, p1, o);
                } else if (!first_chunk) {
                    k1_mfma(I0{}, IN{});
                }
                compute_k0((tap / 3) * W2 + tap % 3, hb, wsl);
            } else {
                compute((tap / 3) * W2 + tap % 3, hb, wsl);
            }
            wsl ^= 1;
        };
        one_tap(std::integral_constant<int, 0>{}); one_tap(std::integral_constant<int, 1>{}); one_tap(std::integral_constant<int, 2>{});
        one_tap(std::integral_constant<int, 3>{}); one_tap(std::integral_constant<int, 4>{}); one_tap(std::integral_constant<int, 5>{});
        one_tap(std::integral_constant<int, 6>{}); one_tap(std::integral_constant<int, 7>{}); one_tap(std::integral_constant<int, 8>{});
        cc += 64;
        hb ^= 1;
        if (cc < cc_end) continue;
        if constexpr (GN) k1_mfma(std::integral_constant<int, 0>{}, std::integral_constant<int, TM * TN>{});
        const int done_m0 = m0, done_tn = c_tn, done_z = c_z;
        item += gridDim.x;
        const bool more = item < hd.n_items;
        if (more) begin_item(item);
        {
            const int nm0 = m0, ntn = c_tn, nz = c_z;
            m0 = done_m0; c_tn = done_tn; c_z = done_z;
            epilogue();
            m0 = nm0; c_tn = ntn; c_z = nz;
        }
        if (!more) break;
        zero_acc();
    }
}

#ifndef GL_WIDE_NST
#define GL_WIDE_NST 2
#endif
template <int TN>
__global__ void __launch_bounds__(512, 1)
gemm_wide_kernel(AOperand A, const bf16* __restrict__ W, int M, int N, int K, Epilogue E, float* __restrict__ ws, WideDesc wd) {
    constexpr int TM = 4;
    constexpr int BM = 256;
    constexpr int BN = TN * 32;
    constexpr int XP = BM / 64;
    constexpr int WP = (BN + 63) / 64;
    constexpr int WREM = BN % 64;
    constexpr int STAGE = (BM + BN) * 128;
    constexpr int NST = GL_WIDE_NST;

    extern __shared__ __attribute__((aligned(16))) unsigned char smem[];

    const int t = threadIdx.x;
    const int lane = t & 63;
    const int wave = __builtin_amdgcn_readfirstlane(t >> 6);
    const int wm = wave >> 1;
    const int wn = wave & 1;
    const int l15 = lane & 15;
    const int q = lane >> 4;
    const int r0 = t >> 3;
    const unsigned chb = (((t & 7) ^ ((r0 >> 1) & 7)) * 16);
    const int nk = K >> 6;

    const __amdgpu_buffer_rsrc_t ra0 = __builtin_amdgcn_make_buffer_rsrc((void*)A.p0, 0, 0x80000000u, 0x00020000);
    const __amdgpu_buffer_rsrc_t ra1 = __builtin_amdgcn_make_buffer_rsrc((void*)(A.p1 ? A.p1 : A.p0), 0, 0x80000000u, 0x00020000);
    const __amdgpu_buffer_rsrc_t rw = __builtin_amdgcn_make_buffer_rsrc((void*)W, 0, 0x80000000u, 0x00020000);

    const int foff0 = l15 * 128 + (((q) ^ (l15 >> 1)) << 4);
    const int foff1 = l15 * 128 + (((q + 4) ^ (l15 >> 1)) << 4);
    const int xrow0 = wm * TM * 16 * 128;
    const int wrow0 = BM * 128 + wn * TN * 16 * 128;
    const unsigned lds0 = (unsigned)(uintptr_t)(__attribute__((address_space(3))) unsigned char*)smem;

    int m0 = 0, c_tn = 0, c_z = 0;
    unsigned vx0 = 0, vx1 = 0, vw0 = 0;
    auto setup = [&](int item_) {
        int item = item_;
        if (wd.xcd) {
            const int q = wd.n_items >> 3, r = wd.n_items & 7, xcd = item & 7, idx = item >> 3;
            item = (xcd < r ? xcd * (q + 1) : r * (q + 1) + (xcd - r) * q) + idx;
        }
        const int tile = item / wd.splits;
        c_z = item - tile * wd.splits;
        const int tm = tile / wd.tiles_n;
        c_tn = tile - tm * wd.tiles_n;
        m0 = tm * BM;
        vx0 = (unsigned)((m0 + r0) * A.ld0) * 2u + chb;
        vx1 = (unsigned)((m0 + r0) * A.ld1) * 2u + chb;
        vw0 = (unsigned)((c_tn * BN + r0) * K) * 2u + chb;
    };
    auto issue = [&](int kt_, int st_) {
        const int kt = __builtin_amdgcn_readfirstlane(kt_);
        const int st = __builtin_amdgcn_readfirstlane(st_);
        const int k0 = kt << 6;
// ... 201 lines not shown
        } else {
            __builtin_amdgcn_s_waitcnt(0x0F70);
        }
        __builtin_amdgcn_s_barrier();
        asm volatile("" ::: "memory");
        if (NST == 3) { if (kt + 2 < kt_end) issue(kt + 2, ring_next(ring_next(stg))); }
        else if (kt + 1 < kt_end) issue(kt + 1, stg ^ 1);
        compute(stg, !first);
        stg_done = stg;
        stg = ring_next(stg);
        ++kt;
    };
    for (;;) {
        tile(std::true_type{});
        while (kt < kt_end) tile(std::false_type{});
        finish();
        const int done_m0 = m0, done_tn = c_tn, done_z = c_z;
        float done_s = ln_s, done_q = ln_q;
#pragma unroll
        for (int i = 0; i < LNV; ++i) { done_s += ln_v[i].x; done_q += ln_v[i].y; }
        item += gridDim.x;
        const bool more = item < wd.n_items;
        if (more) begin_item(item);
        {
            const int nm0 = m0, ntn = c_tn, nz = c_z;
            m0 = done_m0; c_tn = done_tn; c_z = done_z;
            const float2* lst = nullptr;
            if (E.ln_stats && wd.splits == 1) {
                float2* l = reinterpret_cast<float2*>(smem + stg_done * STAGE);
                __builtin_amdgcn_s_barrier();
                const int row = t >> 1, part = t & 1;
                float s = done_s, qq = done_q;
                s += __shfl_xor(s, 1, 64); qq += __shfl_xor(qq, 1, 64);
                if (part == 0) {
                    const float mean = s * E.ln_inv_c;
                    const float var = fmaxf(qq * E.ln_inv_c - mean * mean, 0.f);
                    l[row] = make_float2(mean, rsqrtf(var + E.ln_eps));
                }
                __syncthreads();
                lst = l;
            }
            epilogue(lst);
            m0 = nm0; c_tn = ntn; c_z = nz;
        }
        if (!more) break;
        zero_acc();
    }
}



static thread_local GemmPlan t_last = [] { GemmPlan p{}; strcpy(p.name, "gemm"); return p; }();
int gemm_last_stats_nb() { return t_last.stats_nb; }
const char* gemm_last_kernel_name() { return t_last.name; }
void gemm_last_cfg(int* tm, int* tn, int* splits) { *tm = t_last.tm; *tn = t_last.tn; *splits = t_last.splits; }
static thread_local GemmLogEntry t_log[kGemmLogSize];
static thread_local int t_log_n = 0;
void gemm_plan_log_clear() { t_log_n = 0; }
int gemm_plan_log(GemmLogEntry* out, int max, int* launches) {
    if (launches) *launches = t_log_n;
    const int n = std::max(0, std::min(std::min(t_log_n, kGemmLogSize), max));
    for (int i = 0; i < n; ++i) out[i] = t_log[(t_log_n - n + i) % kGemmLogSize];
    return n;
}

namespace {

struct Launch {
    const AOperand& A; const bf16* W; int M, N, K; const Epilogue& E; float* ws;
    hipStream_t stream;
    template <auto KFN, class... Tail> int run(dim3 grid, int block, size_t lds, const Tail&... tail) const {
        return launch_lds<KFN>(grid, dim3(block), lds, stream, A, W, M, N, K, E, ws, tail...);
    }
};

template <int WM, int WN, int TM, int TN>
int exec_glds(const Launch& l, const GemmPlan& p) {
    const dim3 grid(p.grid, 1, p.splits);
    const size_t lds = 2 * (WM * TM * 32 + WN * TN * 32) * 128;
    if (p.amode == A_ROWS) return l.run<gemm_glds_kernel<WM, WN, TM, TN, A_ROWS>>(grid, WM * WN * 64, lds, p.work.kt_per_split, p.work.tiles_n, p.grid);
    return l.run<gemm_glds_kernel<WM, WN, TM, TN, A_CONV3>>(grid, WM * WN * 64, lds, p.work.kt_per_split, p.work.tiles_n, p.grid);
}
template <int TM, int TN>
int exec_p(const Launch& l, const GemmPlan& p) {
    const size_t lds = 2 * (TM * 32 + TN * 32) * 128;
    if (p.amode == A_ROWS) return l.run<gemm_p_kernel<TM, TN, A_ROWS>>(p.grid, 256, lds, p.work);
    return l.run<gemm_p_kernel<TM, TN, A_CONV3>>(p.grid, 256, lds, p.work);
}
template <int TM, int TN>
int exec_u(const Launch& l, const GemmPlan& p) {
    const size_t lds = 2 * (TM * 32 + TN * 32) * 128;
    if (p.qkv) {
        if constexpr (TM == 4 && TN == 5) return set_error(GL_ERR_UNSUPPORTED, "gemm: no 128x160 tile for EPI_QKV_HEADS");
        else return l.run<gemm_u_kernel<2, TM, TN, A_ROWS, 2, true>>(p.grid, 256, lds, p.work);
    }
    if (p.amode == A_ROWS) return l.run<gemm_u_kernel<2, TM, TN, A_ROWS, 2>>(p.grid, 256, lds, p.work);
    if (p.amode == A_CONV2UP) return l.run<gemm_u_kernel<2, TM, TN, A_CONV2UP, 2>>(p.grid, 256, lds, p.work);
    return l.run<gemm_u_kernel<2, TM, TN, A_CONV3, 2>>(p.grid, 256, lds, p.work);
}
constexpr size_t halo_lds(int tn, bool gn) { return 2 * 7 * 64 * 128 + 2 * tn * 32 * 128 + (gn ? 2048 : 0); }
constexpr size_t wide_lds(int tn) { return GL_WIDE_NST * (256 + tn * 32) * 128; }

int execute(const GemmPlan& p, const AOperand& A, const bf16* W, int M, int N, int K, const Epilogue& E_in, float* ws, hipStream_t stream) {
    Epilogue E = E_in;
    if ((p.family == GEMM_P || p.family == GEMM_U) && !p.stats_nb) E.stats_out = nullptr;
    const Launch l{A, W, M, N, K, E, ws, stream};
    int rc = set_error(GL_ERR_UNSUPPORTED, "gemm: unknown tile candidate");
    switch (p.family * 1000 + p.gn * 100 + p.tm * 10 + p.tn) {
        case GEMM_HALO * 1000 + 185: rc = l.run<conv_halo_kernel<5, 8, true>>(p.grid, 512, halo_lds(5, true), p.halo); break;
        case GEMM_HALO * 1000 + 184: rc = l.run<conv_halo_kernel<4, 8, true>>(p.grid, 512, halo_lds(4, true), p.halo); break;
        case GEMM_HALO * 1000 + 85: rc = l.run<conv_halo_kernel<5, 8>>(p.grid, 512, halo_lds(5, false), p.halo); break;
        case GEMM_HALO * 1000 + 84: rc = l.run<conv_halo_kernel<4, 8>>(p.grid, 512, halo_lds(4, false), p.halo); break;
        case GEMM_WIDE * 1000 + 85: rc = l.run<gemm_wide_kernel<5>>(p.grid, 512, wide_lds(5), p.wide); break;
        case GEMM_WIDE * 1000 + 84: rc = l.run<gemm_wide_kernel<4>>(p.grid, 512, wide_lds(4), p.wide); break;
        case GEMM_U * 1000 + 45: rc = exec_u<4, 5>(l, p); break;
        case GEMM_U * 1000 + 44: rc = exec_u<4, 4>(l, p); break;
        case GEMM_U * 1000 + 25: rc = exec_u<2, 5>(l, p); break;
        case GEMM_U * 1000 + 24: rc = exec_u<2, 4>(l, p); break;
        case GEMM_U * 1000 + 22: rc = exec_u<2, 2>(l, p); break;
        case GEMM_P * 1000 + 45: rc = exec_p<4, 5>(l, p); break;
        case GEMM_P * 1000 + 44: rc = exec_p<4, 4>(l, p); break;
        case GEMM_P * 1000 + 25: rc = exec_p<2, 5>(l, p); break;
        case GEMM_P * 1000 + 24: rc = exec_p<2, 4>(l, p); break;
        case GEMM_GLDS * 1000 + 44: rc = exec_glds<2, 2, 2, 2>(l, p); break;
        case GEMM_GLDS * 1000 + 42: rc = exec_glds<2, 2, 2, 1>(l, p); break;
        case GEMM_GLDS * 1000 + 22: rc = exec_glds<2, 2, 1, 1>(l, p); break;
        case GEMM_GLDS * 1000 + 41: rc = exec_glds<4, 1, 1, 1>(l, p); break;
    }
    GL_TRY(rc);
    if (p.splits > 1) {
        int64_t total = (int64_t)M * (N / 4);
        int blocks = (int)fmin((double)cdiv64(total, 256), 4096.0);
        hipLaunchKernelGGL(splitk_reduce_kernel, dim3(blocks), dim3(256), 0, stream, ws, p.splits, M, N, E);
        GL_LAUNCH_CHECK();
    }
    return GL_OK;
}

int tune(const bf16* W, float* ws, hipStream_t stream, const GemmProblem& pb, bool use_u, const char* key, const GemmCand& model, GemmCand* win, bool* cache) {
    hipStreamCaptureStatus cap = hipStreamCaptureStatusNone;
    if (stream) (void)hipStreamIsCapturing(stream, &cap);
    if (cap != hipStreamCaptureStatusNone) return GL_OK;
    auto run = [&](const GemmCand& c, hipStream_t s) -> int {
        GemmPlan plan{};
        GL_TRY(gemm_plan_tile(pb, use_u, c, plan));
        return execute(plan, pb.A, W, pb.M, pb.N, pb.K, pb.E, ws, s);
    };
    GL_HIP(hipDeviceSynchronize());
    hipEvent_t ev[2];
    GL_HIP(hipEventCreate(&ev[0]));
    GL_HIP(hipEventCreate(&ev[1]));
    struct EvGuard { hipEvent_t* e; ~EvGuard() { (void)hipEventDestroy(e[0]); (void)hipEventDestroy(e[1]); } } ev_guard{ev};
    float win_ms = 1e30f;
    const int tune_reps = gemm_knobs().tune_reps, corun = gemm_knobs().corun;
    hipStream_t s2 = nullptr;
    hipEvent_t ev_fork = nullptr, ev_join = nullptr;
    struct CoGuard { hipStream_t& s; hipEvent_t &a, &b; ~CoGuard() { if (a) (void)hipEventDestroy(a); if (b) (void)hipEventDestroy(b); if (s) (void)hipStreamDestroy(s); } } co_guard{s2, ev_fork, ev_join};
    if (corun) {
        GL_HIP(hipStreamCreateWithFlags(&s2, hipStreamNonBlocking));
        GL_HIP(hipEventCreateWithFlags(&ev_fork, hipEventDisableTiming));
        GL_HIP(hipEventCreateWithFlags(&ev_join, hipEventDisableTiming));
    }
    for (const GemmCand& c : gemm_tune_candidates(pb, use_u)) {
        GL_TRY(run(c, stream));
        GL_HIP(hipEventRecord(ev[0], stream));
        if (corun) {
            GL_HIP(hipEventRecord(ev_fork, stream));
            GL_HIP(hipStreamWaitEvent(s2, ev_fork, 0));
            for (int r = 0; r < tune_reps; ++r) {
                GL_TRY(run(c, stream));
                GL_TRY(run(c, s2));
            }
            GL_HIP(hipEventRecord(ev_join, s2));
            GL_HIP(hipStreamWaitEvent(stream, ev_join, 0));
        } else
            for (int r = 0; r < tune_reps; ++r) GL_TRY(run(c, stream));
        GL_HIP(hipEventRecord(ev[1], stream));
        GL_HIP(hipEventSynchronize(ev[1]));
        float ms = 0.f;
        GL_HIP(hipEventElapsedTime(&ms, ev[0], ev[1]));
        if (ms < win_ms) { win_ms = ms; *win = c; }
    }
    *cache = true;
    if (gemm_knobs().tune_log)
        fprintf(stderr, "[gemm autotune] %s -> %dx%d / %d splits @%d (%.1f us; model said %dx%d / %d) cfg %d %d %d\n", key, kGemmTm[win->c] * 32,
                kGemmTn[win->c] * 32, win->sp, win->grid ? win->grid : 512, win_ms * 1e3f / tune_reps, kGemmTm[model.c] * 32, kGemmTn[model.c] * 32, model.sp,
                win->c, win->sp, win->grid);
    return GL_OK;
}

}

int gemm_launch(const AOperand& A, const bf16* W, int M, int N, int K, const Epilogue& E_in, float* ws,
                size_t ws_bytes, hipStream_t stream) {
    t_last.stats_nb = 0;
    Epilogue E = E_in;
    GemmPlan plan;
    GL_TRY(gemm_plan(A, M, N, K, E, ws != nullptr, ws_bytes, plan, [&](auto&&... a) { return tune(W, ws, stream, a...); }));
    t_last = plan;
    t_log[t_log_n % kGemmLogSize] = GemmLogEntry{plan, M, N, K};
    t_log_n = t_log_n == INT_MAX ? kGemmLogSize : t_log_n + 1;
    return execute(plan, A, W, M, N, K, E, ws, stream);
}

int gemm_launch_t(const bf16* Wrows, int Mw, const bf16* X, int Nx, int K, const Epilogue& E, hipStream_t stream) {
    AOperand A;
    aoperand_rows(A, Wrows, K, K);
    return gemm_launch(A, X, Mw, Nx, K, E, nullptr, 0, stream);
}

}
```

gligen_amd/csrc/gemm_plan.h:

```cpp
#pragma once
#include <functional>
#include <vector>

#include "gemm.h"

namespace gl {

struct WorkDesc {
    int tiles_n;
    int splits;
    int kt_per_split;
    int n_items;
    int box, rm, rz;
};
struct HaloDesc {
    int tiles_n, splits, chunks_per_split, n_items;
    int lgW, lgH;
};
struct WideDesc {
    int tiles_n, splits, kt_per_split, n_items;
    int xcd;
};

struct GemmKnobs {
    int variant = 4;
    int wide = 1, wide_splits = 0;
    int halo = 8, halo_splits = 0;
    int xcd_boxes = 1, wide_xcd = -1;
    int autotune = 1, tune_reps = 3, corun = 0;
    bool no_table = false, tune_log = false;
    int force_tm = 0, force_tn = 0, force_splits = 0, force_grid = 0;
};
GemmKnobs& gemm_knobs();
void gemm_force_knobs(int halo_splits, int wide_splits, int wide_xcd, int xcd_boxes, int halo, int wide);
void gemm_force_clear();

struct GemmProblem {
    const AOperand& A;
    int M, N, K;
    const Epilogue& E;
    bool has_ws; size_t ws_bytes;
};

enum GemmFamily { GEMM_GLDS, GEMM_P, GEMM_U, GEMM_HALO, GEMM_WIDE };

struct GemmCand { int c, sp, grid; };
constexpr int kGemmTiles = 5;
extern const int kGemmTm[kGemmTiles], kGemmTn[kGemmTiles];

struct GemmPlan {
    int family;
    int tm, tn, amode;
    bool qkv, gn;
    int splits;
    int grid;
    union { WorkDesc work; HaloDesc halo; WideDesc wide; };
    int stats_nb;
    char name[96];
};

struct GemmLogEntry { GemmPlan plan; int M, N, K; };
constexpr int kGemmLogSize = 32;
void gemm_plan_log_clear();
int gemm_plan_log(GemmLogEntry* out, int max, int* launches);

std::vector<GemmCand> gemm_tune_candidates(const GemmProblem& pb, bool use_u);
int gemm_plan_tile(const GemmProblem& pb, bool use_u, const GemmCand& cand, GemmPlan& plan);

using GemmTuner = std::function<int(const GemmProblem& pb, bool use_u, const char* key, const GemmCand& model, GemmCand* win, bool* cache)>;

int gemm_plan(const AOperand& A, int M, int N, int K, Epilogue& E, bool has_ws, size_t ws_bytes, GemmPlan& plan, const GemmTuner& tuner = nullptr);

}
```

gligen_amd/csrc/gemm_plan.hip:

```cpp
#include "gemm_plan.h"

#include <algorithm>
#include <cmath>
#include <cstdio>
#include <mutex>
#include <string>
#include <unordered_map>

namespace gl {

static GemmKnobs read_knobs() {
    static const struct { const char* env; int GemmKnobs::*knob; } kInt[] = {
        {"GL_GEMM_VARIANT", &GemmKnobs::variant}, {"GL_GEMM_WIDE", &GemmKnobs::wide}, {"GL_GEMM_WIDE_SPLITS", &GemmKnobs::wide_splits},
        {"GL_CONV_HALO", &GemmKnobs::halo}, {"GL_CONV_HALO_SPLITS", &GemmKnobs::halo_splits}, {"GL_GEMM_XCD_BOXES", &GemmKnobs::xcd_boxes},
        {"GL_WIDE_XCD", &GemmKnobs::wide_xcd}, {"GL_GEMM_AUTOTUNE", &GemmKnobs::autotune}, {"GL_GEMM_TUNE_REPS", &GemmKnobs::tune_reps},
        {"GL_GEMM_TUNE_CORUN", &GemmKnobs::corun}};
    GemmKnobs k;
    for (const auto& e : kInt)
        if (const char* v = dev_env(e.env)) k.*e.knob = atoi(v);
    k.tune_reps = std::max(1, k.tune_reps);
    k.no_table = dev_env("GL_GEMM_NO_TABLE") != nullptr;
    k.tune_log = dev_env("GL_GEMM_TUNE_LOG") != nullptr;
    return k;
}
GemmKnobs& gemm_knobs() {
    static GemmKnobs k = read_knobs();
    return k;
}
void gemm_set_variant(int v) { gemm_knobs().variant = v < 0 ? read_knobs().variant : v; }
void gemm_set_autotune(int on) { gemm_knobs().autotune = on < 0 ? read_knobs().autotune : on; }
void gemm_force_cfg(int tm, int tn, int splits) { gemm_knobs().force_tm = tm; gemm_knobs().force_tn = tn; gemm_knobs().force_splits = splits; }
void gemm_force_grid(int g) { gemm_knobs().force_grid = g; }
void gemm_force_knobs(int halo_splits, int wide_splits, int wide_xcd, int xcd_boxes, int halo, int wide) {
    GemmKnobs& k = gemm_knobs();
    k.halo_splits = halo_splits; k.wide_splits = wide_splits; k.wide_xcd = wide_xcd; k.xcd_boxes = xcd_boxes; k.halo = halo; k.wide = wide;
}
void gemm_force_clear() {
    const GemmKnobs d = read_knobs();
    gemm_force_cfg(0, 0, 0);
    gemm_force_grid(0);
    gemm_force_knobs(d.halo_splits, d.wide_splits, d.wide_xcd, d.xcd_boxes, d.halo, d.wide);
}
static thread_local int t_no_split = 0;
void gemm_set_no_split(int on) { t_no_split = on; }
static thread_local int t_plan_scale = 1;
void gemm_set_plan_batch_scale(int scale) { t_plan_scale = scale > 1 ? scale : 1; }

int gemm_geglu_layout() { return gemm_knobs().variant >= 2 ? 1 : 0; }
bool gemm_supports_qkv() { return gemm_knobs().variant == 4; }

static size_t a_rows(const AOperand& A, int M) {
    return A.mode != A_ROWS && A.Ho * A.Wo > 0 ? (size_t)(M / (A.Ho * A.Wo)) * A.Hin * A.Win : (size_t)M;
}
static int row_tiles(const AOperand& A, int M, int bm) { return A.mode == A_CONV2UP ? 4 * cdiv(M / 4, bm) : cdiv(M, bm); }
static bool fits_buffer_offsets(const AOperand& A, int M, int N, int K) {
    return a_rows(A, M) * (size_t)std::max(A.ld0, A.ld1) * 2 < 0x7fff0000ull && (size_t)N * K * 2 * (A.mode == A_CONV2UP ? 4 : 1) < 0x7fff0000ull;
}

static inline int ilog2_exact(int v) {
    int l = 0;
    while ((1 << l) < v) ++l;
    return (1 << l) == v ? l : -1;
}
static bool halo_eligible(const AOperand& A, int M, int N, int K, const Epilogue& E) {
    if (A.mode != A_CONV3 || A.stride != 1 || A.ups || A.pad_lo != 1 || A.Ho != A.Hin || A.Wo != A.Win) return false;
    const int lgW = ilog2_exact(A.Win), lgH = ilog2_exact(A.Hin);
    if (lgW < 3 || lgW > 6 || lgH < 0 || M % 256) return false;
    const int R = 256 >> lgW, HB = std::min(A.Hin, R);
    if ((R / HB) * (HB + 2) * (A.Win + 2) > 448) return false;
    if (A.C0 % 64 || A.C1 % 64 || (N % 160 && N % 128)) return false;
    if (E.mode != EPI_ROWMAJOR || E.remap_in || (E.act != ACT_NONE && E.act != ACT_SILU) || (E.bias2 && E.res)) return false;
    if (E.bias2 && (E.rows_per_b != A.Hin * A.Win)) return false;
    return fits_buffer_offsets(A, M, N, K);
}
static bool wide_eligible(const AOperand& A, int M, int N, int K, const Epilogue& E) {
    if (A.mode != A_ROWS || M % 256 || (N % 160 && N % 128)) return false;
    if (A.C1 && A.C0 % 64) return false;
    if (E.mode != EPI_ROWMAJOR || E.remap_in || E.bias2) return false;
    if (E.act == ACT_GEGLU) { if (N % 128 || !E.geglu16 || E.res || E.out_f32) return false; }
    else if (E.act != ACT_NONE && E.act != ACT_SILU) return false;
    return fits_buffer_offsets(A, M, N, K);
}

static int gemm_route(const AOperand& A, int M, int N, int K, const Epilogue& E, bool honour_force = true) {
    const GemmKnobs& kn = gemm_knobs();
    if (A.mode == A_CONV2UP) return kn.variant == 4 && fits_buffer_offsets(A, M, N, K) ? GEMM_U : GEMM_P;
    if (kn.variant < 2 || (N < 128 && E.act != ACT_GEGLU)) return GEMM_GLDS;
    const bool use_u = kn.variant == 4 && fits_buffer_offsets(A, M, N, K) && !(E.bias2 && (E.res || A.mode == A_ROWS));
    if (!use_u) return GEMM_P;
    const bool forced = honour_force && kn.force_tm;
    if (kn.halo && !forced && N >= 128 && halo_eligible(A, M, N, K, E) && M >= kn.halo * 256) return GEMM_HALO;
    if (kn.wide && !forced && (kn.wide >= 2 || E.act == ACT_GEGLU) && wide_eligible(A, M, N, K, E)) return GEMM_WIDE;
    return GEMM_U;
}

bool gemm_gn_prologue_supported(const AOperand& A, int M, int N, int K, const Epilogue& E) {
    return K % 64 == 0 && gemm_route(A, M, N, K, E) == GEMM_HALO && (A.Hin * A.Win) % 256 == 0;
}

bool gemm_upconv_phases_supported(const AOperand& A, int M, int N, int K, const Epilogue& E) {
    if (A.mode != A_CONV2UP || M <= 0 || M != 4 * (M / (4 * A.Hin * A.Win)) * A.Hin * A.Win || A.Ho != 2 * A.Hin || A.Wo != 2 * A.Win) return false;
    if ((A.C0 + A.C1) % 64 || A.C0 % 64 || K != 4 * (A.C0 + A.C1) || N % 8 || A.gn) return false;
    if (E.mode != EPI_ROWMAJOR || E.act != ACT_NONE || E.out_f32 || E.bias2 || E.res || E.gate || E.remap_in || E.stats_out || E.ln_stats) return false;
    return gemm_route(A, M, N, K, E) == GEMM_U;
}

bool gemm_ln_fold_supported(const AOperand& A, int M, int N, int K, const Epilogue& E) {
    if (A.mode != A_ROWS || A.C1 || K % 64) return false;
    if (E.act == ACT_GEGLU) return E.mode == EPI_ROWMAJOR && gemm_route(A, M, N, K, E, false) == GEMM_WIDE;
    if (E.mode != EPI_QKV_HEADS && E.mode != EPI_QK_HEADS) return false;
    Epilogue Eh = E;
    Eh.bias2 = nullptr;
    return gemm_route(A, M, N, K, Eh, false) == GEMM_U;
}

static int gemm_validate(const AOperand& A, int M, int N, int K, Epilogue& E) {
    if (E.rows_per_b < 1) return set_error(GL_ERR_ARG, "gemm: rows_per_b=%d", E.rows_per_b);
    {
        E.up_win = A.mode == A_CONV2UP ? A.Win : 0;
        const unsigned d = E.up_win ? (unsigned)E.up_win : (unsigned)E.rows_per_b;
        int sh = 0;
        while ((1ull << sh) < d) ++sh;
        E.rpb_shift = sh;
        E.rpb_magic = (unsigned)((((1ull << sh) - d) << 32) / d + 1);
    }
    if (M <= 0 || N <= 0 || K <= 0) return set_error(GL_ERR_ARG, "gemm: empty problem M=%d N=%d K=%d", M, N, K);
    if (E.ln_stats && (!E.ln_csum || !E.bias || E.ln_nb < 1 || E.ln_ld < E.ln_nb || !gemm_ln_fold_supported(A, M, N, K, E)))
        return set_error(GL_ERR_UNSUPPORTED, "gemm: folded LayerNorm needs csum + folded bias + statistics, and an epilogue that applies them");
    if (K % 64 != 0) return set_error(GL_ERR_ARG, "gemm: K=%d must be a multiple of 64", K);
    if (N % 4 != 0) return set_error(GL_ERR_ARG, "gemm: N=%d must be a multiple of 4", N);
    if (A.gn && !gemm_gn_prologue_supported(A, M, N, K, E))
        return set_error(GL_ERR_UNSUPPORTED, "gemm: the GroupNorm prologue (AOperand::gn) exists in conv_halo_kernel only (3x3, stride 1, H W %% 256 == 0)");
    if (A.mode == A_CONV2UP) {
        if (!gemm_upconv_phases_supported(A, M, N, K, E))
            return set_error(GL_ERR_UNSUPPORTED, "conv3x3: no phase form of the upsample conv for this launch (gemm_u_kernel, bias-only bf16 epilogue, K = 4 Cin, N %% 8 == 0)");
    } else if (A.mode == A_CONV3) {
        if ((A.C0 + A.C1) % 64 != 0 || A.C0 % 64 != 0 || K != 9 * (A.C0 + A.C1))
            return set_error(GL_ERR_ARG, "conv3x3: channels (%d,%d) must be multiples of 64 and K=9*Cin (K=%d)", A.C0, A.C1, K);
    } else {
        if (K != A.C0 + A.C1 || (A.C1 && A.C0 % 64 != 0))
            return set_error(GL_ERR_ARG, "gemm: K=%d does not match operand channels (%d,%d)", K, A.C0, A.C1);
    }
    if (A.mode != A_ROWS && (E.gate || E.remap_in))
        return set_error(GL_ERR_UNSUPPORTED, "conv3x3: the gated residual and the row remap are row-GEMM epilogues");
    if ((E.act == ACT_GELU || E.act == ACT_QUICK_GELU) && (E.res || E.bias2 || A.mode != A_ROWS))
        return set_error(GL_ERR_UNSUPPORTED, "gemm: the GELU / quick-GELU epilogues have no residual / broadcast-bias form");
    if (E.act == ACT_GEGLU && (N % 32 != 0 || E.mode != EPI_ROWMAJOR))
        return set_error(GL_ERR_ARG, "gemm: GEGLU epilogue needs packed N %% 32 == 0 (N=%d)", N);
    if (E.act == ACT_GEGLU && E.geglu16 != gemm_geglu_layout())
        return set_error(GL_ERR_STATE, "gemm: GEGLU weights were packed for a different main-loop variant");
// ... 15 lines not shown
    int sp = want;
    if (sp <= 0) {
        sp = 1;
        while (tiles * sp < 200 && units / (sp * 2) >= min_units) sp *= 2;
    }
    sp = std::max(1, std::min(sp, units));
    if (!pb.has_ws || !allowed) sp = 1;
    while (sp > 1 && (size_t)sp * pb.M * pb.N * sizeof(float) > pb.ws_bytes) --sp;
    const int per = cdiv(units, sp);
    splits = cdiv(units, per);
    return per;
}

void plan_glds(const GemmProblem& pb, const GemmProblem& ph, GemmPlan& p) {
    const int M = ph.M, N = pb.N;
    int best = 0;
    float best_score = -1.f;
    for (int c = 0; c < 4; ++c) {
        if (c == 3 && N > 32) continue;
        if (c != 3 && N <= 32) continue;
        const Cfg& cf = kCfgs[c];
        double tm = cdiv(M, cf.bm), tn = cdiv(N, cf.bn);
        double pad = ((double)M * N) / (tm * cf.bm * tn * cf.bn);
        double fill = fmin(1.0, tm * tn / 256.0);
        float score = (float)(pad * cf.speed * (0.35 + 0.65 * fill));
        if (score > best_score) { best_score = score; best = c; }
    }
    const Cfg& cf = kCfgs[best];
    snprintf(p.name, sizeof p.name, "gemm_glds_kernel<%dx%d, %d>", cf.bm, cf.bn, pb.A.mode);
    const int tiles_h = cdiv(M, cf.bm) * cdiv(N, cf.bn), tiles = cdiv(pb.M, cf.bm) * cdiv(N, cf.bn);
    const int nk = pb.K / 64;
    int splits = 1;
    if (pb.has_ws && !t_no_split && tiles_h < 256 && nk >= 8) {
        splits = std::min(std::min(cdiv(512, tiles_h), nk / 4), 16);
        while (splits > 1 && (size_t)splits * M * N * sizeof(float) > pb.ws_bytes) --splits;
    }
    const int kps = cdiv(nk, splits);
    p.splits = cdiv(nk, kps);
    p.tm = cf.bm / 32; p.tn = cf.bn / 32; p.grid = tiles;
    p.work = WorkDesc{cdiv(N, cf.bn), p.splits, kps, tiles, -1, 0, p.splits};
}

void plan_halo(const GemmProblem& pb, const GemmProblem& ph, GemmPlan& p) {
    const AOperand& A = pb.A;
    const int M = pb.M, N = pb.N, tn = N % 160 == 0 ? 5 : 4;
    HaloDesc& hd = p.halo;
    hd.lgW = ilog2_exact(A.Win); hd.lgH = ilog2_exact(A.Hin);
    hd.tiles_n = cdiv(N, tn * 32);
    const int tiles = (M / 256) * hd.tiles_n;
    hd.chunks_per_split = split_units(ph, gemm_knobs().halo_splits, (ph.M / 256) * hd.tiles_n, (A.C0 + A.C1) / 64, 2, true, hd.splits);
    hd.n_items = tiles * hd.splits;
    p.tm = 8; p.tn = tn; p.gn = A.gn != nullptr; p.splits = hd.splits;
    p.grid = std::min(hd.n_items, 256);
    snprintf(p.name, sizeof p.name, "conv_halo_kernel<%d, %d%s>%s", tn, 8, p.gn ? ", gn" : "", reduce_suffix(p.splits));
}

void plan_wide(const GemmProblem& pb, const GemmProblem& ph, GemmPlan& p) {
    const Epilogue& E = pb.E;
    const int M = pb.M, N = pb.N, tn = (E.act != ACT_GEGLU && N % 160 == 0) ? 5 : 4;
    WideDesc& wd = p.wide;
    wd.tiles_n = N / (tn * 32);
    const int tiles = (M / 256) * wd.tiles_n;
    wd.kt_per_split = split_units(ph, gemm_knobs().wide_splits, (ph.M / 256) * wd.tiles_n, pb.K / 64, 4, E.act != ACT_GEGLU, wd.splits);
    wd.n_items = tiles * wd.splits;
    wd.xcd = gemm_knobs().wide_xcd >= 0 ? gemm_knobs().wide_xcd : (wd.tiles_n % 8 != 0 && wd.n_items >= 512);
    if (wd.n_items < 256 || std::min(wd.n_items, 256) % 8) wd.xcd = 0;
    p.tm = 8; p.tn = tn; p.splits = wd.splits;
    p.grid = std::min(wd.n_items, 256);
    snprintf(p.name, sizeof p.name, "gemm_wide_kernel<%d>%s", tn, reduce_suffix(p.splits));
}

}

const int kGemmTm[kGemmTiles] = {4, 4, 2, 2, 2}, kGemmTn[kGemmTiles] = {5, 4, 5, 4, 2};
static const int kSp[10] = {1, 2, 3, 4, 6, 8, 12, 16, 24, 32};

static bool feasible(const GemmProblem& pb, bool use_u, int c, int& sp) {
    const Epilogue& E = pb.E;
    const int tm = kGemmTm[c], tn = kGemmTn[c], nk = pb.K / 64;
    if (c == 4 && !use_u) return false;
    if (E.act == ACT_GEGLU && (tn & 1)) return false;
    if (E.mode == EPI_QKV_HEADS && (sp > 1 || (2 * E.C) % (tn * 32) || (tm == 4 && tn == 5))) return false;
    if (E.mode == EPI_QK_HEADS && E.ln_stats && (sp > 1 || (tm == 4 && tn == 5))) return false;
    if (sp > 1 && (t_no_split || !pb.has_ws || nk / sp < 2 || (size_t)sp * pb.M * pb.N * sizeof(float) > pb.ws_bytes)) return false;
    sp = cdiv(nk, cdiv(nk, sp));
    return true;
}

static void tuned_key(const GemmProblem& pb, bool use_u, char* key, size_t n) {
    const AOperand& A = pb.A; const Epilogue& E = pb.E;
    snprintf(key, n, "%d,%d,%d|%d,%d,%d,%d,%d,%d,%d|%d,%d,%d,%d,%d,%d|%d%s", pb.M, pb.N, pb.K, A.mode, A.C0, A.C1, A.stride, A.ups, A.Win,
             A.Hin, E.mode, E.act, E.res != nullptr, E.bias2 != nullptr, E.out_f32, E.gate != nullptr, (int)use_u,
             (E.mode == EPI_QK_HEADS && E.ln_stats) ? "|ln" : t_no_split ? "|ns" : "");
}

static bool forced_choice(const GemmProblem& pb, bool use_u, GemmCand& out) {
    const GemmKnobs& kn = gemm_knobs();
    const int want = kn.force_splits ? kn.force_splits : 1;
    if (!kn.force_tm || want < 1 || want > kSp[9]) return false;
    for (int c = 0; c < kGemmTiles; ++c) {
        int sp = want;
        if (kGemmTm[c] != kn.force_tm || kGemmTn[c] != kn.force_tn || !feasible(pb, use_u, c, sp) || sp != want) continue;
        out = GemmCand{c, sp, 0};
        return true;
    }
    return false;
}
// ... 152 lines not shown
```

gligen_amd/csrc/norm.h:

```cpp
#pragma once
#include "common.h"

namespace gl {

struct GNParams {
    const bf16* x0;
    const bf16* x1;
    int C0, C1;
    int B, HW;
    float eps;
    const float* gamma;
    const float* beta;
    bf16* y;
    int silu;
    float* partial;
    float* coef;
};
int gn_nsplit(int HW);
size_t gn_partial_bytes(int B, int HW);
int groupnorm_launch(const GNParams& P, hipStream_t stream);
int groupnorm_coef_launch(const GNParams& P, hipStream_t stream);
int groupnorm_coef_launches(int HW, int C0, int C1);
inline size_t gn_coef_bytes(int B, int C) { return (size_t)B * C * 2 * sizeof(float); }

struct LNParams {
    const bf16* x;
    const bf16* x2;
    int B, N1, N2, Tpad, C;
    float eps;
    const float* gamma;
    const float* beta;
    bf16* y;
    int ldx, ldy;
};
int layernorm_launch(const LNParams& P, hipStream_t stream);

int softmax_rows_launch(const float* S, bf16* Pm, int rows, int cols, float scale, hipStream_t stream);

}
```

gligen_amd/csrc/norm.hip:

```cpp
#include "norm.h"

namespace gl {

constexpr int GN_UNR = 8;
static int gn_rows(int C8) { return C8 >= 256 ? 1 : 256 / C8; }
int gn_nsplit_c(int HW, int C8) { return max(1, min(64, cdiv(HW, gn_rows(C8) * GN_UNR))); }
int gn_nsplit(int HW) { return max(1, min(64, HW / 8)); }
size_t gn_partial_bytes(int B, int HW) { return (size_t)B * 64 * 32 * 2 * sizeof(float); }

__global__ void gn_stats_kernel(GNParams P, int nsplit, int C8, int R, int cpg) {
    extern __shared__ __attribute__((aligned(16))) unsigned char smem[];
    float4* tl = reinterpret_cast<float4*>(smem);
    const int t = threadIdx.x;
    const int cx = t % C8;
    const int ry = t / C8;
    const int b = blockIdx.y;
    const int c0 = cx * 8;
    const bool first = c0 < P.C0;
    const int ld = first ? P.C0 : P.C1;
    const bf16* base = (first ? P.x0 + c0 : P.x1 + (c0 - P.C0)) + (size_t)b * P.HW * ld;
    const int per = (P.HW + nsplit - 1) / nsplit;
    const int p0 = blockIdx.x * per;
    const int p1 = min(P.HW, p0 + per);
    const int g_lo = c0 / cpg;
// ... 256 lines not shown
        const double n = (double)P.HW * cpg;
        const double mean = ss / n;
        double var = qq / n - mean * mean;
        if (var < 0.0) var = 0.0;
        stat_s[0] = (float)mean;
        stat_s[1] = (float)(1.0 / sqrt(var + (double)P.eps));
    }
    __syncthreads();
    if (t < cpg) {
        const int c = c_base + t;
        const float a = stat_s[1] * P.gamma[c];
        const float cc = P.beta[c] - stat_s[0] * a;
        float* dst = P.coef + (size_t)b * C * 2;
        dst[(c >> 3) * 16 + (c & 7)] = a;
        dst[(c >> 3) * 16 + 8 + (c & 7)] = cc;
    }
}

static int gn_check(const GNParams& P, int* cpg_out) {
    const int C = P.C0 + P.C1;
    if (C % 64 != 0 || (P.C1 && P.C0 % 8 != 0)) return set_error(GL_ERR_ARG, "groupnorm: C=%d (C0=%d) unsupported", C, P.C0);
    const int cpg = C / 32;
    if (cpg < 4 || (cpg & 1)) return set_error(GL_ERR_UNSUPPORTED, "groupnorm: %d channels per group (need an even number >= 4)", cpg);
    if (C / 8 > 1024) return set_error(GL_ERR_ARG, "groupnorm: C=%d too large", C);
    *cpg_out = cpg;
    return GL_OK;
}

int groupnorm_coef_launch(const GNParams& P, hipStream_t stream) {
    int cpg;
    GL_TRY(gn_check(P, &cpg));
    if (!P.coef) return set_error(GL_ERR_ARG, "groupnorm_coef: no coefficient buffer");
    const int C = P.C0 + P.C1, C8 = C / 8;
    if (P.HW <= 256 && (P.C0 & 3) == 0 && (cpg & 3) == 0) {
        if (P.HW * cpg >= 8192) hipLaunchKernelGGL(gn_small_coef_kernel<1024>, dim3(32, P.B), dim3(1024), 0, stream, P, cpg);
        else hipLaunchKernelGGL(gn_small_coef_kernel<256>, dim3(32, P.B), dim3(256), 0, stream, P, cpg);
        GL_LAUNCH_CHECK();
        return GL_OK;
    }
    const int R = gn_rows(C8);
    const int nsplit = gn_nsplit_c(P.HW, C8);
    const int T = C8 * R;
    hipLaunchKernelGGL(gn_stats_kernel, dim3(nsplit, P.B), dim3(T), T * sizeof(float4), stream, P, nsplit, C8, R, cpg);
    GL_LAUNCH_CHECK();
    hipLaunchKernelGGL(gn_coef_kernel, dim3(P.B), dim3(256), 0, stream, P, nsplit, cpg);
    GL_LAUNCH_CHECK();
    return GL_OK;
}
int groupnorm_coef_launches(int HW, int C0, int C1) {
    const int cpg = (C0 + C1) / 32;
    return (HW <= 256 && (C0 & 3) == 0 && (cpg & 3) == 0) ? 1 : 2;
}

int groupnorm_launch(const GNParams& P, hipStream_t stream) {
    const int C = P.C0 + P.C1;
    if (C % 64 != 0 || (P.C1 && P.C0 % 8 != 0)) return set_error(GL_ERR_ARG, "groupnorm: C=%d (C0=%d) unsupported", C, P.C0);
    const int cpg = C / 32;
    const int C8 = C / 8;
    if (cpg < 4 || (cpg & 1)) return set_error(GL_ERR_UNSUPPORTED, "groupnorm: %d channels per group (need an even number >= 4)", cpg);
    if (C8 > 1024) return set_error(GL_ERR_ARG, "groupnorm: C=%d too large", C);
    if (P.HW <= 256 && (P.C0 & 3) == 0 && (cpg & 3) == 0) {
        if (P.HW * cpg >= 8192) hipLaunchKernelGGL(gn_small_kernel<1024>, dim3(32, P.B), dim3(1024), 0, stream, P, cpg);
        else hipLaunchKernelGGL(gn_small_kernel<256>, dim3(32, P.B), dim3(256), 0, stream, P, cpg);
        GL_LAUNCH_CHECK();
        return GL_OK;
    }
    const int R = gn_rows(C8);
    const int nsplit = gn_nsplit_c(P.HW, C8);
    const int T = C8 * R;
    hipLaunchKernelGGL(gn_stats_kernel, dim3(nsplit, P.B), dim3(T), T * sizeof(float4), stream, P, nsplit, C8, R, cpg);
    GL_LAUNCH_CHECK();
    const int trips = cdiv(P.HW, R * GN_UNR);
    const int nblk = max(1, min(trips, max(1, 2048 / P.B)));
    const int per = cdiv(cdiv(P.HW, nblk), R) * R;
    hipLaunchKernelGGL(gn_apply_kernel, dim3(cdiv(P.HW, per), P.B), dim3(T), 0, stream, P, nsplit, C8, R, cpg, per);
    GL_LAUNCH_CHECK();
    return GL_OK;
}

__global__ void __launch_bounds__(256) ln_kernel(LNParams P) {
    const int lane = threadIdx.x & 63;
    const int wave = threadIdx.x >> 6;
    const int64_t r = (int64_t)blockIdx.x * 4 + wave;
    if (r >= (int64_t)P.B * P.Tpad) return;
    const int b = (int)(r / P.Tpad);
    const int t = (int)(r - (int64_t)b * P.Tpad);
    const int C8 = P.C >> 3;
    const int ldx = P.ldx ? P.ldx : P.C, ldy = P.ldy ? P.ldy : P.C;
    bf16* dst = P.y + r * ldy;
    for (int ch = C8 + lane; ch < (ldy >> 3); ch += 64) *reinterpret_cast<uint4*>(dst + ch * 8) = make_uint4(0, 0, 0, 0);
    const bf16* src;
    if (t < P.N1) src = P.x + ((size_t)b * P.N1 + t) * ldx;
    else if (t < P.N1 + P.N2) src = P.x2 + ((size_t)b * P.N2 + (t - P.N1)) * P.C;
    else {
        for (int ch = lane; ch < C8; ch += 64) *reinterpret_cast<uint4*>(dst + ch * 8) = make_uint4(0, 0, 0, 0);
        return;
    }
    float v[3][8];
    float s = 0.f;
#pragma unroll
    for (int i = 0; i < 3; ++i) {
        const int ch = lane + 64 * i;
        if (ch < C8) {
            U4BF8 u;
            u.u = *reinterpret_cast<const uint4*>(src + ch * 8);
#pragma unroll
// ... 79 lines not shown
```

gligen_amd/engine.py:

```python
from __future__ import annotations

import ctypes as C
from typing import Dict, Mapping, Optional, Sequence

import numpy as np
import torch

from . import _lib
from ._lib import Grounding, PlmsArgs, SolverArgs, UNetConfig, VaeConfig, check

GROUNDING_KINDS = {"text": 0, "text_image": 1, "keypoint": 2, "tokens": 3}


def _stream(device=None) -> C.c_void_p:
    return C.c_void_p(torch.cuda.current_stream(device).cuda_stream)


def _ptr(t: Optional[torch.Tensor]) -> C.c_void_p:
    return C.c_void_p(0 if t is None else t.data_ptr())


def _f32(t: torch.Tensor, device) -> torch.Tensor:
    return t.to(device=device, dtype=torch.float32).contiguous()

# ... 1075 lines not shown
                                             1 if accumulate else 0, *[_ptr(o.get(n)) for n in ("a", "xhat", "rstd", "dx")], _stream(dev)))
        return o

    def op_train_geglu(self, u, dh=None, out=None):
        dev = self.device
        u = _f32(u, dev)
        dh = None if dh is None else _f32(dh, dev)
        R, I2 = u.shape
        if I2 % 2 or (dh is not None and dh.shape != (R, I2 // 2)):
            raise ValueError("op_train_geglu: u [R, 2 I], dh [R, I]")
        shapes = {"h": (R, I2 // 2)}
        if dh is not None:
            shapes.update(du=u.shape)
        o = self._prim_outs(shapes, out)
        check(self.lib.gl_op_train_geglu(self._ctx, int(R), int(I2 // 2), _ptr(u), _ptr(dh), _ptr(o.get("h")), _ptr(o.get("du")), _stream(dev)))
        return o

    def op_train_dot(self, a, b, mode, alpha=None, scale=1.0, out=None):
        dev = self.device
        a, b = _f32(a, dev).reshape(-1), _f32(b, dev).reshape(-1)
        alpha = None if alpha is None else _f32(alpha, dev)
        if a.shape != b.shape:
            raise ValueError("op_train_dot: a and b hold the same number of elements")
        o = self._prim_outs({"out": (1,)}, out, required=("out",))
        check(self.lib.gl_op_train_dot(self._ctx, int(a.numel()), _ptr(a), _ptr(b), _ptr(alpha), C.c_float(scale), int(mode), _ptr(o["out"]), _stream(dev)))
        return o

    def op_conv3x3(self, x0, w_oihw, bias, x1=None, stride=1, ups=0, pad_lo=1, res=None):
        B, H, W, C0 = x0.shape
        C1 = 0 if x1 is None else x1.shape[3]
        Cout = w_oihw.shape[0]
        Hup, Wup = H << ups, W << ups
        if stride == 1:
            Ho, Wo = Hup, Wup
        else:
            Ho = (Hup + (2 if pad_lo else 1) - 3) // 2 + 1
            Wo = (Wup + (2 if pad_lo else 1) - 3) // 2 + 1
        y = torch.empty((B, Ho, Wo, Cout), device=x0.device, dtype=torch.bfloat16)
        check(self.lib.gl_op_conv3x3(self._ctx, _ptr(x0), C0, _ptr(x1), C1, B, H, W, _ptr(w_oihw), _ptr(bias), Cout,
                                     stride, ups, pad_lo, _ptr(res), _ptr(y), _stream(self.device)))
        return y

    def op_gn_silu_conv3x3(self, x0, gamma, beta, eps, w_oihw, bias, x1=None, bias2=None, res=None, mode=-1):
        B, H, W, C0 = x0.shape
        C1 = 0 if x1 is None else x1.shape[3]
        Cout = w_oihw.shape[0]
        y = torch.empty((B, H, W, Cout), device=x0.device, dtype=torch.bfloat16)
        used = C.c_int(0)
        check(self.lib.gl_op_gn_silu_conv3x3(self._ctx, _ptr(x0), C0, _ptr(x1), C1, B, H, W, _ptr(gamma), _ptr(beta), C.c_float(eps),
                                             _ptr(w_oihw), _ptr(bias), Cout, _ptr(bias2), _ptr(res), _ptr(y), int(mode), C.byref(used),
                                             _stream(self.device)))
        return y, bool(used.value)

    def op_groupnorm(self, x0, gamma, beta, eps, silu, x1=None):
        B, HW, C0 = x0.shape
        C1 = 0 if x1 is None else x1.shape[2]
        y = torch.empty((B, HW, C0 + C1), device=x0.device, dtype=torch.bfloat16)
        check(self.lib.gl_op_groupnorm(self._ctx, _ptr(x0), C0, _ptr(x1), C1, B, HW, _ptr(gamma), _ptr(beta),
                                       C.c_float(eps), int(silu), _ptr(y), _stream(self.device)))
        return y

    def op_layernorm(self, x, gamma, beta, eps=1e-5, x2=None, Tpad=None):
        B, N1, Cc = x.shape
        N2 = 0 if x2 is None else x2.shape[1]
        Tpad = Tpad or (N1 + N2)
        y = torch.empty((B, Tpad, Cc), device=x.device, dtype=torch.bfloat16)
        check(self.lib.gl_op_layernorm(self._ctx, _ptr(x), _ptr(x2), B, N1, N2, Tpad, Cc, _ptr(gamma), _ptr(beta),
                                       C.c_float(eps), _ptr(y), _stream(self.device)))
        return y

    def op_ff_chain_q(self, x, pre_w, pre_b, pre_res, gamma, beta, w1, b1, w2, b2, gamma_q, beta_q, wq, pre_gate=None, gate=None):
        B, N, Cc = x.shape
        y = torch.empty_like(x)
        qbuf = torch.zeros((B * 8, N, 48), device=x.device, dtype=torch.bfloat16)
        check(self.lib.gl_op_ff_chain_q(self._ctx, _ptr(x), B, N, Cc, _ptr(pre_w), _ptr(pre_b), _ptr(pre_res), _ptr(pre_gate), _ptr(gamma), _ptr(beta),
                                        _ptr(w1), _ptr(b1), _ptr(w2), _ptr(b2), _ptr(gate), _ptr(gamma_q), _ptr(beta_q), _ptr(wq), _ptr(y), _ptr(qbuf),
                                        _stream(self.device)))
        return y, qbuf.view(B, 8, N, 48)[..., :40]

    def op_proj_attention(self, x, pre_w, pre_b, pre_res, gamma, beta, wq, wk, wv, heads, rows=True):
        B, N, Cc = x.shape
        mid = torch.empty_like(x)
        o = torch.empty_like(x)
        used = C.c_int(1 if rows else 0)
        check(self.lib.gl_op_proj_attention(self._ctx, _ptr(x), B, N, Cc, heads, _ptr(pre_w), _ptr(pre_b), _ptr(pre_res), _ptr(gamma), _ptr(beta),
                                            _ptr(wq), _ptr(wk), _ptr(wv), 0, _ptr(mid), _ptr(o), C.byref(used), _stream(self.device)))
        return mid, o, used.value

    def op_attention(self, xq, xkv, wq, wk, wv, heads):
        B, Nq, Cc = xq.shape
        _, Nk, Ck = xkv.shape
        o = torch.empty((B, Nq, Cc), device=xq.device, dtype=torch.bfloat16)
        check(self.lib.gl_op_attention(self._ctx, _ptr(xq), _ptr(xkv), B, Nq, Nk, Cc, Ck, heads, _ptr(wq), _ptr(wk), _ptr(wv),
                                       _ptr(o), _stream(self.device)))
        return o

    def op_attention_core(self, q, k, vt, layout, B, heads, Nq, Nk, o, ldo, o_rows_per_b, kernel="auto"):
        from ._lib import ATTN_CORE_KERNELS
        check(self.lib.gl_op_attention_core(self._ctx, _ptr(q), _ptr(k), _ptr(vt), C.byref(layout), B, heads, Nq, Nk, _ptr(o), ldo, o_rows_per_b,
                                            ATTN_CORE_KERNELS[kernel], _stream(self.device)))
        return o

    def attn_regime_counters(self, enable):
        lazy, reruns = C.c_uint(0), C.c_uint(0)
        check(self.lib.gl_attn_regime_counters(self._ctx, 1 if enable else 0, C.byref(lazy), C.byref(reruns)))
        return lazy.value, reruns.value
# ... 1 lines not shown
```

Measured before the change: 6.690 images/s.

## Emit GroupNorm partial statistics from conv3x3 halo GEMM epilogue for the next norm

```diff
diff --git a/gligen_amd/_lib.py b/gligen_amd/_lib.py
--- a/gligen_amd/_lib.py
+++ b/gligen_amd/_lib.py
@@ -256,6 +256,9 @@
 ATTN_CORE_KERNELS = {"auto": 0, "attn_kernel": 1, "attn2_kernel_w4": 2, "attn2_kernel_w8": 3, "attn3_kernel": 4}
 GL_ERR_UNSUPPORTED = 5
 
+GN_PRODUCER_SYMBOLS = {
+    "gl_op_conv3x3_groupnorm": (_I, [_P, _P, _I, _P, _I, _I, _I, _I, _P, _P, _I, _P, _P, _P, _P, C.c_float, _I, _P, _P, _I, _P, _P]),
+}
 VAE_SYMBOLS = {
     "gl_vae_set_attention": (_I, [_P, _I]),
     "gl_op_vae_attention": (_I, [_P, _P, _P, _P, _I, _I, _I, _I, _P, _P]),
@@ -296,7 +299,7 @@
     import torch
     lib = C.CDLL(str(LIB_PATH))
     for name, (res, args) in {**SYMBOLS, **IMAGE_SYMBOLS, **MAP_SYMBOLS, **TRAIN_MAP_SYMBOLS, **TRAIN_INPUT_SYMBOLS, **TRAIN_FUSER_SYMBOLS, **TRAIN_PRIM_SYMBOLS,
-                              **TRAINER_SYMBOLS, **SAMPLER_SYMBOLS, **SOLVER_SYMBOLS, **GEMM_PLAN_SYMBOLS, **ATTENTION_CORE_SYMBOLS, **VAE_SYMBOLS, **LATENT_SYMBOLS, **LORA_SYMBOLS}.items():
+                              **TRAINER_SYMBOLS, **SAMPLER_SYMBOLS, **SOLVER_SYMBOLS, **GEMM_PLAN_SYMBOLS, **ATTENTION_CORE_SYMBOLS, **VAE_SYMBOLS, **LATENT_SYMBOLS, **LORA_SYMBOLS, **GN_PRODUCER_SYMBOLS}.items():
         fn = getattr(lib, name)
         fn.restype = res
         fn.argtypes = args
diff --git a/gligen_amd/csrc/capi.hip b/gligen_amd/csrc/capi.hip
--- a/gligen_amd/csrc/capi.hip
+++ b/gligen_amd/csrc/capi.hip
@@ -16,6 +16,7 @@
 #include "../../include/gligen_amd_vae.h"
 #include "../../include/gligen_amd_latent.h"
 #include "../../include/gligen_amd_lora.h"
+#include "../../include/gligen_amd_gn_producer.h"
 #include "gemm_plan.h"
 
 #include <cstdlib>
@@ -1214,6 +1215,29 @@
     eng.gn_prologue_ = saved;
     *used_prologue = eng.n_prologue_convs > n0 ? 1 : 0;
     if (mode == 1 && !*used_prologue) throw GlError(GL_ERR_UNSUPPORTED, "gl_op_gn_silu_conv3x3: this shape has no GroupNorm prologue (conv_halo_kernel, H W % 256 == 0)");
+    GL_API_END
+}
+
+int gl_op_conv3x3_groupnorm(gl_ctx* ctx, const void* x0, int C0, const void* x1, int C1, int B, int H, int W, const float* w_oihw, const float* bias,
+                            int Cout, const float* bias2, const void* res, const float* gamma, const float* beta, float eps, int silu,
+                            void* conv_out, void* y, int mode, int* used_producer, gl_stream s) {
+    NEED(ctx);
+    if (!x0 || !w_oihw || !gamma || !beta || !conv_out || !y || !used_producer) return gl::set_error(GL_ERR_ARG, "gl_op_conv3x3_groupnorm: null pointer");
+    if (bias2 && res) return gl::set_error(GL_ERR_ARG, "gl_op_conv3x3_groupnorm: a per-sample bias or a residual, not both");
+    GL_API_BEGIN
+    Engine& eng = *ctx->eng;
+    Arena& ar = eng.arena();
+    ar.reset();
+    const int Cin = C0 + C1;
+    bf16* wp = ar.get<bf16>((size_t)Cout * 9 * Cin);
+    int r = pack_conv_weight_launch(w_oihw, wp, Cout, Cin, 3, 3, Cout, S(s));
+    if (r != GL_OK) throw GlError(r, gl::last_error());
+    NormW n;
+    n.g = gamma; n.b = beta; n.C = Cout;
+    ConvW c;
+    c.w = wp; c.b = bias; c.Cin = Cin; c.Cout = Cout;
+    *used_producer = eng.op_conv3x3_groupnorm(TRef{(const bf16*)x0, C0, (const bf16*)x1, C1}, B, H, W, c, bias2, (const bf16*)res, n, eps, silu != 0, mode,
+                                              (bf16*)conv_out, (bf16*)y, S(s)) ? 1 : 0;
     GL_API_END
 }
 
diff --git a/gligen_amd/csrc/engine.h b/gligen_amd/csrc/engine.h
--- a/gligen_amd/csrc/engine.h
+++ b/gligen_amd/csrc/engine.h
@@ -175,9 +175,13 @@
     unsigned* attn_counters() const { return attn_counting_ ? attn_ctr_ : nullptr; }
 
     bf16* gn_silu_conv3x3(const TRef& x, int B, int H, int W, const NormW& n, float eps, const ConvW& c, const float* bias2, int bias2_ld,
-                          const bf16* res, bf16* out, hipStream_t s);
+                          const bf16* res, bf16* out, hipStream_t s, float* gn_out = nullptr);
     bf16* conv3x3(const TRef& x, int B, int Hin, int Win, const ConvW& c, int stride, int ups, int pad_lo,
-                  const float* bias2, int bias2_ld, const bf16* res, hipStream_t s, bf16* out = nullptr);
+                  const float* bias2, int bias2_ld, const bf16* res, hipStream_t s, bf16* out = nullptr, float* gn_out = nullptr);
+    bool op_conv3x3_groupnorm(const TRef& x, int B, int H, int W, const ConvW& c, const float* bias2, const bf16* res, const NormW& n, float eps,
+                              bool silu, int mode, bf16* conv_out, bf16* y, hipStream_t s);
+    bool gn_producer_ = true;
+    int64_t n_producer_norms = 0;
     static bool upconv_phase_form(int Cin, int Cout);
     bool gn_prologue_ = dev_env("GL_GN_PROLOGUE") && atoi(dev_env("GL_GN_PROLOGUE")) == 1;
     int64_t n_prologue_convs = 0;
@@ -251,6 +255,13 @@
     unsigned* attn_ctr_ = nullptr;
     bool attn_counting_ = false;
     std::vector<hipEvent_t> train_events_;
+    struct GnStatsRec { const bf16* x; float* partial; int nslot, C, B, HW; };
+    std::vector<GnStatsRec> gn_reg_;
+    std::map<std::pair<const void*, int>, std::pair<float*, size_t>> gn_bufs_;
+    float* gn_stats_buffer(const void* owner, int which, int B, int HW);
+    bool gn_reg_take(const bf16* x, int C, int B, int HW, GnStatsRec* rec);
+    void gn_reg_keep_only(const bf16* x);
+    void conv3_launch(const AOperand& A, const ConvW& c, int B, int HW, Epilogue& E, float* gn_out, hipStream_t s);
 
     struct Unet {
         bool present = false;
diff --git a/gligen_amd/csrc/engine.hip b/gligen_amd/csrc/engine.hip
--- a/gligen_amd/csrc/engine.hip
+++ b/gligen_amd/csrc/engine.hip
@@ -206,6 +206,9 @@
     e.ws_bytes_ = 0;
     e.cond_ = Cond{};
     e.attn_bufs_.clear();
+    e.gn_bufs_.clear();
+    e.gn_reg_.clear();
+    e.n_producer_norms = 0;
     e.attn_ctr_ = nullptr;
     e.attn_counting_ = false;
     e.smp_ = Sampler{};
@@ -488,8 +491,38 @@
     ++n_launches;
 }
 
+float* Engine::gn_stats_buffer(const void* owner, int which, int B, int HW) {
+    const size_t need = gn_partial_bytes(B, HW);
+    auto& slot = gn_bufs_[{owner, which}];
+    if (slot.second < need) slot = {reinterpret_cast<float*>(persist(need, false)), need};
+    return slot.first;
+}
+bool Engine::gn_reg_take(const bf16* x, int C, int B, int HW, GnStatsRec* rec) {
+    for (size_t i = 0; i < gn_reg_.size(); ++i)
+        if (gn_reg_[i].x == x) {
+            *rec = gn_reg_[i];
+            gn_reg_.erase(gn_reg_.begin() + i);
+            return rec->C == C && rec->HW == HW && rec->B >= B;
+        }
+    return false;
+}
+void Engine::gn_reg_keep_only(const bf16* x) {
+    gn_reg_.erase(std::remove_if(gn_reg_.begin(), gn_reg_.end(), [&](const GnStatsRec& r) { return r.x != x; }), gn_reg_.end());
+}
+void Engine::conv3_launch(const AOperand& A, const ConvW& c, int B, int HW, Epilogue& E, float* gn_out, hipStream_t s) {
+    const int M = B * HW, K = 9 * c.Cin;
+    E.gn_cpg = c.Cout / 32;
+    const bool want = gn_out && gn_producer_ && c.Cout % 64 == 0 && gemm_gn_partial_supported(A, M, c.Cout, K, E);
+    E.gn_partial = want ? gn_out : nullptr;
+    gemm(A, c.w, M, c.Cout, K, E, s);
+    const int nslot = want ? gemm_last_gn_slots() : 0;
+    if (nslot) gn_reg_.push_back(GnStatsRec{reinterpret_cast<const bf16*>(E.out), gn_out, nslot, c.Cout, B, HW});
+}
+
 void Engine::gemm(const AOperand& A, const bf16* W, int M, int N, int K, const Epilogue& E, hipStream_t s) {
     ProfScope ps(this, s, "gemm", 2.0 * M * N * K, 0.0);
+    if (!gn_reg_.empty())
+        gn_reg_.erase(std::remove_if(gn_reg_.begin(), gn_reg_.end(), [&](const GnStatsRec& r) { return r.x == E.out; }), gn_reg_.end());
     CK(gemm_launch(A, W, M, N, K, E, ws_, ws_bytes_, s));
     if (profiling_) {
         static const bool by_shape = dev_env("GL_PROF_SHAPES") != nullptr;
@@ -538,6 +571,15 @@
     GNParams P{};
     P.x0 = x.p0; P.C0 = x.C0; P.x1 = x.p1; P.C1 = x.C1;
     P.B = B; P.HW = HW; P.eps = eps; P.gamma = n.g; P.beta = n.b; P.y = y; P.silu = silu ? 1 : 0;
+    GnStatsRec st;
+    if (HW > 256 && !x.p1 && gn_reg_take(x.p0, C, B, HW, &st)) {
+        P.partial = st.partial;
+        ProfScope ps(this, s, "gn_apply_kernel (producer statistics)", 0.0, 2.0 * B * HW * (double)C * 2);
+        CK(groupnorm_apply_launch(P, st.nslot, s));
+        ++n_launches;
+        ++n_producer_norms;
+        return y;
+    }
     P.partial = reinterpret_cast<float*>(arena_.alloc(gn_partial_bytes(B, HW)));
     ProfScope ps(this, s, HW <= 256 ? "gn_small_kernel" : "gn_stats_kernel + gn_apply_kernel", 0.0, 2.0 * B * HW * (double)C * 2);
     CK(groupnorm_launch(P, s));
@@ -546,7 +588,7 @@
 }
 
 bf16* Engine::gn_silu_conv3x3(const TRef& x, int B, int H, int W, const NormW& n, float eps, const ConvW& c, const float* bias2, int bias2_ld,
-                              const bf16* res, bf16* out, hipStream_t s) {
+                              const bf16* res, bf16* out, hipStream_t s, float* gn_out) {
     if (x.C() != c.Cin || n.C != c.Cin) throw GlError(GL_ERR_ARG, fmt("gn_silu_conv3x3: %d channels into a norm of %d and a conv of %d", x.C(), n.C, c.Cin));
     const int HW = H * W, M = B * HW;
     if (!out) out = arena_.get<bf16>((size_t)M * c.Cout);
@@ -557,22 +599,29 @@
         GNParams P{};
         P.x0 = x.p0; P.C0 = x.C0; P.x1 = x.p1; P.C1 = x.C1;
         P.B = B; P.HW = HW; P.eps = eps; P.gamma = n.g; P.beta = n.b; P.silu = 1;
-        P.partial = reinterpret_cast<float*>(arena_.alloc(gn_partial_bytes(B, HW)));
         P.coef = reinterpret_cast<float*>(arena_.alloc(gn_coef_bytes(B, c.Cin)));
-        {
+        GnStatsRec st;
+        if (HW > 256 && !x.p1 && gn_reg_take(x.p0, c.Cin, B, HW, &st)) {
+            P.partial = st.partial;
+            ProfScope ps(this, s, "gn_coef_kernel (producer statistics)", 0.0, 0.0);
+            CK(groupnorm_coef_from_partial_launch(P, st.nslot, s));
+            ++n_launches;
+            ++n_producer_norms;
+        } else {
+            P.partial = reinterpret_cast<float*>(arena_.alloc(gn_partial_bytes(B, HW)));
             const int nl = groupnorm_coef_launches(HW, x.C0, x.C1);
             ProfScope ps(this, s, nl == 1 ? "gn_small_coef_kernel" : "gn_stats_kernel + gn_coef_kernel", 0.0, 1.0 * B * HW * (double)c.Cin * 2);
             CK(groupnorm_coef_launch(P, s));
             n_launches += nl;
         }
         A.gn = P.coef;
-        gemm(A, c.w, M, c.Cout, 9 * c.Cin, E, s);
+        conv3_launch(A, c, B, HW, E, gn_out, s);
         ++n_prologue_convs;
         return out;
     }
     bf16* a = groupnorm(x, B, HW, n, eps, true, s);
     A.p0 = a; A.C0 = c.Cin; A.ld0 = c.Cin; A.p1 = nullptr; A.C1 = 0; A.ld1 = 0;
-    gemm(A, c.w, M, c.Cout, 9 * c.Cin, E, s);
+    conv3_launch(A, c, B, HW, E, gn_out, s);
     return out;
 }
 
@@ -595,7 +644,7 @@
 }
 
 bf16* Engine::conv3x3(const TRef& x, int B, int Hin, int Win, const ConvW& c, int stride, int ups, int pad_lo,
-                      const float* bias2, int bias2_ld, const bf16* res, hipStream_t s, bf16* out) {
+                      const float* bias2, int bias2_ld, const bf16* res, hipStream_t s, bf16* out, float* gn_out) {
     if (x.C() != c.Cin) throw GlError(GL_ERR_ARG, fmt("conv3x3: input has %d channels, weight expects %d", x.C(), c.Cin));
     if (c.w4) {
         if (stride != 1 || ups != 1 || pad_lo != 1 || bias2 || res) throw GlError(GL_ERR_ARG, "conv3x3: phase-form weights serve the plain upsample conv only");
@@ -619,8 +668,31 @@
     if (!out) out = arena_.get<bf16>((size_t)M * c.Cout);
     Epilogue E = e_rows_res(out, c.Cout, c.b, res);
     E.bias2 = bias2; E.bias2_ld = bias2_ld; E.rows_per_b = Ho * Wo;
-    gemm(a_conv3(x, Hin, Win, Ho, Wo, stride, ups, pad_lo), c.w, M, c.Cout, 9 * c.Cin, E, s);
+    if (gn_out && stride == 1 && !ups) conv3_launch(a_conv3(x, Hin, Win, Ho, Wo, stride, ups, pad_lo), c, B, Ho * Wo, E, gn_out, s);
+    else gemm(a_conv3(x, Hin, Win, Ho, Wo, stride, ups, pad_lo), c.w, M, c.Cout, 9 * c.Cin, E, s);
     return out;
+}
+
+bool Engine::op_conv3x3_groupnorm(const TRef& x, int B, int H, int W, const ConvW& c, const float* bias2, const bf16* res, const NormW& n, float eps,
+                                  bool silu, int mode, bf16* conv_out, bf16* y, hipStream_t s) {
+    const int HW = H * W;
+    const bool saved = gn_producer_;
+    if (mode >= 0) gn_producer_ = mode != 0;
+    const int64_t n0 = n_producer_norms;
+    gn_reg_.clear();
+    try {
+        conv3x3(x, B, H, W, c, 1, 0, 1, bias2, c.Cout, res, s, conv_out, gn_stats_buffer(this, 0, B, HW));
+        const bf16* yn = groupnorm(TRef{conv_out, c.Cout, nullptr, 0}, B, HW, n, eps, silu, s);
+        HIPCK(hipMemcpyAsync(y, yn, (size_t)B * HW * c.Cout * sizeof(bf16), hipMemcpyDeviceToDevice, s));
+    } catch (...) {
+        gn_producer_ = saved;
+        throw;
+    }
+    gn_producer_ = saved;
+    const bool used = n_producer_norms > n0;
+    if (mode == 1 && !used)
+        throw GlError(GL_ERR_UNSUPPORTED, "gl_op_conv3x3_groupnorm: this launch cannot write its output's GroupNorm statistics (conv_halo_kernel, H W % 256 == 0 and > 256, whole groups per 80- / 64-column block)");
+    return used;
 }
 
 void Engine::replicate(const bf16* src, bf16* dst, size_t n, int reps, hipStream_t s) {
@@ -633,7 +705,10 @@
     const int HW = H * W, M = B * HW;
     if (!out) out = arena_.get<bf16>((size_t)M * r.Cout);
     const size_t mk = arena_.mark();
-    bf16* h = gn_silu_conv3x3(x, B, H, W, r.n1, eps, r.c1, embout ? embout + r.emb_off : nullptr, emb_ld, nullptr, nullptr, s);
+    gn_reg_keep_only(x.p1 ? nullptr : x.p0);
+    const bool big = HW > 256 && HW % 256 == 0;
+    bf16* h = gn_silu_conv3x3(x, B, H, W, r.n1, eps, r.c1, embout ? embout + r.emb_off : nullptr, emb_ld, nullptr, nullptr, s,
+                              big ? gn_stats_buffer(&r, 0, B, HW) : nullptr);
     const bf16* sk;
     if (r.has_skip) {
         bf16* skb = arena_.get<bf16>((size_t)M * r.Cout);
@@ -645,7 +720,8 @@
         if (x.p1) throw GlError(GL_ERR_STATE, "identity skip over a concatenated input");
         sk = x.p0;
     }
-    gn_silu_conv3x3(TRef{h, r.Cout, nullptr, 0}, B, H, W, r.n2, eps, r.c2, nullptr, 0, sk, out, s);
+    gn_silu_conv3x3(TRef{h, r.Cout, nullptr, 0}, B, H, W, r.n2, eps, r.c2, nullptr, 0, sk, out, s, big ? gn_stats_buffer(&r, 1, B, HW) : nullptr);
+    gn_reg_keep_only(out);
     arena_.release(mk);
     return out;
 }
diff --git a/gligen_amd/csrc/engine_unet.hip b/gligen_amd/csrc/engine_unet.hip
--- a/gligen_amd/csrc/engine_unet.hip
+++ b/gligen_amd/csrc/engine_unet.hip
@@ -870,7 +870,9 @@
     }
     bool in_prefix = Bp < Beff;
 
+    gn_reg_.clear();
     auto run_layer = [&](const Layer& L, const TRef& in, int Bl, bool full) {
+        gn_reg_keep_only(in.p1 ? nullptr : in.p0);
         PlanAsBatch plan_as(L.kind == L_ST ? 1 : Beff / Bl);
         auto out_for = [&](int HWo, int Co) { return full ? arena_.get<bf16>((size_t)Beff * HWo * Co) : nullptr; };
         auto fill = [&](bf16* o, int HWo, int Co) {
diff --git a/gligen_amd/csrc/engine_vae.hip b/gligen_amd/csrc/engine_vae.hip
--- a/gligen_amd/csrc/engine_vae.hip
+++ b/gligen_amd/csrc/engine_vae.hip
@@ -161,6 +161,7 @@
 }
 
 void Engine::vae_decode(int B, int h, int w, const float* z, float* out, hipStream_t s) {
+    gn_reg_.clear();
     if (!vae_.dec.present || !finalized_) throw GlError(GL_ERR_STATE, "vae not finalized");
     const gl_vae_config& c = vae_.cfg;
     arena_.reset();
@@ -189,6 +190,7 @@
 }
 
 void Engine::vae_encode(int B, int H, int W, const float* img, const float* noise, float* z, hipStream_t s) {
+    gn_reg_.clear();
     if (!vae_.enc.present || !finalized_) throw GlError(GL_ERR_STATE, "vae encoder weights were not uploaded / not finalized");
     const gl_vae_config& c = vae_.cfg;
     const int total_stride = 1 << (c.n_mult - 1);
diff --git a/gligen_amd/csrc/gemm.h b/gligen_amd/csrc/gemm.h
--- a/gligen_amd/csrc/gemm.h
+++ b/gligen_amd/csrc/gemm.h
@@ -19,7 +19,7 @@
 enum { EPI_ROWMAJOR = 0, EPI_QK_HEADS = 1, EPI_VT_HEADS = 2, EPI_NCHW_F32 = 3, EPI_QKV_HEADS = 4 };
 enum { ACT_NONE = 0, ACT_SILU = 1, ACT_GEGLU = 2, ACT_GELU = 3, ACT_QUICK_GELU = 4 };
 
-struct Epilogue {
+struct EpilogueArgs {
     int mode;
     int act;
     void* out;
@@ -54,6 +54,10 @@
     const float* ln_csum;
     float ln_inv_c, ln_eps;
 };
+struct Epilogue : EpilogueArgs {
+    float* gn_partial;
+    int gn_cpg;
+};
 
 __host__ __device__ inline size_t ktile_off(size_t bh, int tpad, int t, int dd, int DP) {
     return (bh * (size_t)tpad + (size_t)(t & ~63)) * DP + (size_t)(dd >> 3) * 512 + (size_t)(t & 63) * 8 + (dd & 7);
@@ -80,6 +84,8 @@
 bool gemm_upconv_phases_supported(const AOperand& A, int M, int N, int K, const Epilogue& E);
 bool gemm_ln_fold_supported(const AOperand& A, int M, int N, int K, const Epilogue& E);
 int gemm_last_stats_nb();
+bool gemm_gn_partial_supported(const AOperand& A, int M, int N, int K, const Epilogue& E);
+int gemm_last_gn_slots();
 void aoperand_rows(AOperand& A, const bf16* p, int K, int ld);
 
 }
diff --git a/gligen_amd/csrc/gemm.hip b/gligen_amd/csrc/gemm.hip
--- a/gligen_amd/csrc/gemm.hip
+++ b/gligen_amd/csrc/gemm.hip
@@ -1,3 +1,4 @@
+#ifndef GL_CONV_HALO_BODY
 #include "gemm_plan.h"
 
 #include <algorithm>
@@ -44,11 +45,11 @@
     *reinterpret_cast<uint2*>(dst) = o.u;
 }
 
-__device__ __forceinline__ int div_rpb(const Epilogue& E, int m) {
+__device__ __forceinline__ int div_rpb(const EpilogueArgs& E, int m) {
     return (int)((__umulhi((unsigned)m, E.rpb_magic) + (unsigned)m) >> E.rpb_shift);
 }
 
-__device__ __forceinline__ void epi_finish4(const Epilogue& E, int m, int n0, float v[4]) {
+__device__ __forceinline__ void epi_finish4(const EpilogueArgs& E, int m, int n0, float v[4]) {
     if (E.bias) {
         float4 b = *reinterpret_cast<const float4*>(E.bias + n0);
         v[0] += b.x; v[1] += b.y; v[2] += b.z; v[3] += b.w;
@@ -122,7 +123,7 @@
 }
 
 template <bool WITH_GELU = true>
-__device__ __forceinline__ void epi_store4(const Epilogue& E, int m, int n0, float v[4]) {
+__device__ __forceinline__ void epi_store4(const EpilogueArgs& E, int m, int n0, float v[4]) {
     if (E.act == ACT_SILU) {
 #pragma unroll
         for (int i = 0; i < 4; ++i) v[i] = silu_f(v[i]);
@@ -178,7 +179,7 @@
     }
 }
 
-__device__ __forceinline__ void epi_geglu4(const Epilogue& E, int m, int nv0, float val[4], float gate[4]) {
+__device__ __forceinline__ void epi_geglu4(const EpilogueArgs& E, int m, int nv0, float val[4], float gate[4]) {
     if (E.bias) {
         float4 bv = *reinterpret_cast<const float4*>(E.bias + nv0);
         float4 bg = *reinterpret_cast<const float4*>(E.bias + nv0 + 8);
@@ -193,7 +194,7 @@
 }
 
 template <int TM, int TN>
-__device__ __forceinline__ void gemm_epilogue(f32x16 (&acc)[TM][TN], const Epilogue& E, int M, int N, int m0, int n0w,
+__device__ __forceinline__ void gemm_epilogue(f32x16 (&acc)[TM][TN], const EpilogueArgs& E, int M, int N, int m0, int n0w,
                                               float* __restrict__ ws) {
     const bool split = gridDim.z > 1;
 #pragma unroll
@@ -250,7 +251,7 @@
 
 template <int WM, int WN, int TM, int TN, int AMODE>
 __global__ void __launch_bounds__(WM * WN * 64)
-gemm_glds_kernel(AOperand A, const bf16* __restrict__ W, int M, int N, int K, Epilogue E,
+gemm_glds_kernel(AOperand A, const bf16* __restrict__ W, int M, int N, int K, EpilogueArgs E,
                  float* __restrict__ ws, int kt_per_split, int tiles_n, int n_tiles) {
     constexpr int NT = WM * WN * 64;
     constexpr int BM = WM * TM * 32;
@@ -414,7 +415,7 @@
     gemm_epilogue<TM, TN>(acc, E, M, N, m_base + wm * TM * 32 + frow, n_base + wn * TN * 32 + 4 * fhalf, ws);
 }
 
-__device__ __forceinline__ void epi_geglu4_t16(const Epilogue& E, int m, int nv0, float val[4], float gate[4]) {
+__device__ __forceinline__ void epi_geglu4_t16(const EpilogueArgs& E, int m, int nv0, float val[4], float gate[4]) {
     if (E.bias) {
         float4 bv = *reinterpret_cast<const float4*>(E.bias + nv0);
         float4 bg = *reinterpret_cast<const float4*>(E.bias + nv0 + 16);
@@ -430,7 +431,7 @@
 
 template <int TM, int TN, int AMODE>
 __global__ void __launch_bounds__(256, 2)
-gemm_p_kernel(AOperand A, const bf16* __restrict__ W, int M, int N, int K, Epilogue E, float* __restrict__ ws, WorkDesc wd) {
+gemm_p_kernel(AOperand A, const bf16* __restrict__ W, int M, int N, int K, EpilogueArgs E, float* __restrict__ ws, WorkDesc wd) {
     constexpr int BM = TM * 32;
     constexpr int BN = TN * 32;
     constexpr int XP = BM / 32;
@@ -634,6 +635,12 @@
     }
 }
 
+template <int CTRL>
+__device__ __forceinline__ float dpp_add(float v) {
+    return v + __builtin_bit_cast(float, __builtin_amdgcn_update_dpp(0, __builtin_bit_cast(int, v), CTRL, 0xf, 0xf, true));
+}
+__device__ __forceinline__ float row16_sum(float v) { return dpp_add<0x140>(dpp_add<0x141>(dpp_add<0x4E>(dpp_add<0xB1>(v)))); }
+
 template <int OFF>
 __device__ __forceinline__ void lds_rd16(bf16x8& d, unsigned addr) {
     asm volatile("ds_read_b128 %0, %1 offset:%2" : "=v"(d) : "v"(addr), "n"(OFF));
@@ -658,7 +665,7 @@
 
 template <int WMW, int TM, int TN, int AMODE, int NST, bool QKV = false>
 __global__ void __launch_bounds__(WMW * 128, 2)
-gemm_u_kernel(AOperand A, const bf16* __restrict__ W, int M, int N, int K, Epilogue E, float* __restrict__ ws, WorkDesc wd) {
+gemm_u_kernel(AOperand A, const bf16* __restrict__ W, int M, int N, int K, EpilogueArgs E, float* __restrict__ ws, WorkDesc wd) {
     constexpr int NT = WMW * 128;
     constexpr int RPP = NT / 8;
     constexpr int BM = WMW * TM * 16;
@@ -1388,7 +1395,7 @@
     }
 }
 
-__device__ __forceinline__ float2 ln_row_stats(const Epilogue& E, int m) {
+__device__ __forceinline__ float2 ln_row_stats(const EpilogueArgs& E, int m) {
     float s = 0.f, q = 0.f;
     for (int nb = 0; nb < E.ln_nb; ++nb) {
         const float2 v = E.ln_stats[(size_t)m * E.ln_ld + nb];
@@ -1400,7 +1407,7 @@
 }
 
 __global__ void __launch_bounds__(256)
-splitk_reduce_kernel(const float* __restrict__ ws, int splits, int M, int N, Epilogue E) {
+splitk_reduce_kernel(const float* __restrict__ ws, int splits, int M, int N, EpilogueArgs E) {
     const int groups = N >> 2;
     const int64_t total = (int64_t)M * groups;
     for (int64_t idx = (int64_t)blockIdx.x * blockDim.x + threadIdx.x; idx < total;
@@ -1482,9 +1489,91 @@
     }
 }
 
-template <int TN, int NW, bool GN = false>
-__global__ void __launch_bounds__(NW * 64, 1)
-conv_halo_kernel(AOperand A, const bf16* __restrict__ W, int M, int N, int K, Epilogue E, float* __restrict__ ws, HaloDesc hd) {
+template <int CBW>
+__global__ void __launch_bounds__(CBW * 8)
+splitk_reduce_gn_kernel(const float* __restrict__ ws, int splits, int M, int N, EpilogueArgs E, int lgHW, float* __restrict__ gn_partial, int gn_cpg) {
+    constexpr int NQ = CBW / 4, R = 32;
+    __shared__ float red_s[2][R][CBW];
+    __shared__ float col_s[2][CBW];
+    const int t = threadIdx.x, cq = t % NQ, ry = t / NQ;
+    const int nb = blockIdx.x * CBW, n0 = nb + cq * 4;
+    const int m0 = blockIdx.y * 256;
+    const float4 pb = *reinterpret_cast<const float4*>(E.bias ? E.bias + n0 : ws);
+    const float4 pb2 = *reinterpret_cast<const float4*>(E.bias2 ? E.bias2 + (size_t)div_rpb(E, m0) * E.bias2_ld + n0 : ws);
+    const float pg = *((E.res && E.gate) ? E.gate : ws);
+    const size_t zs = (size_t)M * N;
+    float cs[4] = {0, 0, 0, 0}, cq2[4] = {0, 0, 0, 0};
+    for (int r = ry; r < 256; r += 2 * R) {
+        uint2 pr[2];
+        float v[2][4] = {{0, 0, 0, 0}, {0, 0, 0, 0}};
+#pragma unroll
+        for (int h = 0; h < 2; ++h)
+            pr[h] = *reinterpret_cast<const uint2*>(E.res ? reinterpret_cast<const void*>(E.res + (size_t)(m0 + r + h * R) * E.ldres + n0)
+                                                          : reinterpret_cast<const void*>(ws));
+        for (int z = 0; z < splits; z += 4) {
+            float4 a[2][4];
+#pragma unroll
+            for (int h = 0; h < 2; ++h)
+#pragma unroll
+                for (int u = 0; u < 4; ++u)
+                    a[h][u] = *reinterpret_cast<const float4*>(ws + (size_t)(m0 + r + h * R) * N + n0 + (size_t)min(z + u, splits - 1) * zs);
+#pragma unroll
+            for (int h = 0; h < 2; ++h)
+#pragma unroll
+                for (int u = 0; u < 4; ++u) {
+                    const bool ok = z + u < splits;
+                    v[h][0] += ok ? a[h][u].x : 0.f; v[h][1] += ok ? a[h][u].y : 0.f; v[h][2] += ok ? a[h][u].z : 0.f; v[h][3] += ok ? a[h][u].w : 0.f;
+                }
+        }
+#pragma unroll
+        for (int h = 0; h < 2; ++h) {
+            float* vh = v[h];
+            if (E.bias) { vh[0] += pb.x; vh[1] += pb.y; vh[2] += pb.z; vh[3] += pb.w; }
+            if (E.bias2) { vh[0] += pb2.x; vh[1] += pb2.y; vh[2] += pb2.z; vh[3] += pb2.w; }
+            if (E.act == ACT_SILU) {
+#pragma unroll
+                for (int i = 0; i < 4; ++i) vh[i] = silu_f(vh[i]);
+            }
+            if (E.res) {
+                U2BF4 rr;
+                rr.u = pr[h];
+                const float g = E.gate ? pg : 1.f;
+#pragma unroll
+                for (int i = 0; i < 4; ++i) vh[i] = bf2f(rr.e[i]) + g * vh[i];
+            }
+            U2BF4 o;
+#pragma unroll
+            for (int i = 0; i < 4; ++i) {
+                o.e[i] = f2bf(vh[i]);
+                const float f = bf2f(o.e[i]);
+                cs[i] += f;
+                cq2[i] += f * f;
+            }
+            *reinterpret_cast<uint2*>(reinterpret_cast<bf16*>(E.out) + (size_t)(m0 + r + h * R) * E.ldo + n0) = o.u;
+        }
+    }
+#pragma unroll
+    for (int i = 0; i < 4; ++i) { red_s[0][ry][cq * 4 + i] = cs[i]; red_s[1][ry][cq * 4 + i] = cq2[i]; }
+    __syncthreads();
+    if (t < 2 * CBW) {
+        const int k = t / CBW, c = t - k * CBW;
+        float a = 0.f;
+#pragma unroll
+        for (int y = 0; y < R; ++y) a += red_s[k][y][c];
+        col_s[k][c] = a;
+    }
+    __syncthreads();
+    const int cpg = gn_cpg;
+    if (t * cpg < CBW) {
+        float a = 0.f, b = 0.f;
+        for (int c = 0; c < cpg; ++c) { a += col_s[0][t * cpg + c]; b += col_s[1][t * cpg + c]; }
+        const int smp = m0 >> lgHW, slot = (m0 & ((1 << lgHW) - 1)) >> 8, nslot = 1 << (lgHW - 8);
+        *reinterpret_cast<float2*>(gn_partial + ((size_t)(smp * nslot + slot) * 32 + nb / cpg + t) * 2) = make_float2(a, b);
+    }
+}
+
+#endif
+#ifdef GL_CONV_HALO_BODY
     constexpr int NT = NW * 64;
     constexpr int RPP = NT / 8;
     constexpr int TM = 32 / NW;
@@ -1499,6 +1588,9 @@
     constexpr int WREM = BN % RPP;
     constexpr unsigned SENT = 0x80000000u;
     constexpr int COEF0 = 2 * HBUF + 2 * WSLOT;
+    constexpr int GPROW = 400;
+    constexpr int CB = TN * 16;
+    static_assert(!GP || (!GN && NW == 8 && NW * 2 * CB * 4 <= (HROWS - GPROW) * 128), "GroupNorm partials: LDS scratch");
     static_assert(HPASS * RPP == HROWS && HPT * 7 >= HPASS && WREM % 8 == 0, "loader geometry");
     static_assert(!GN || (HPT == 1 && HPASS == 7), "the prologue rewrites pass p of the next chunk during tap p + 1");
 
@@ -1732,15 +1824,27 @@
         __builtin_amdgcn_sched_barrier(0);
     };
 
-    auto store_row = [&](int m, int n0, float (&v)[4]) {
+    float gs[GP ? TN : 1][4], gq[GP ? TN : 1][4];
+    auto stat4 = [&](int j, const float (&v)[4]) {
+        if constexpr (GP) {
+#pragma unroll
+            for (int e = 0; e < 4; ++e) {
+                const float f = bf2f(f2bf(v[e]));
+                gs[j][e] += f;
+                gq[j][e] += f * f;
+            }
+        }
+    };
+    auto store_row = [&](int m, int j, int n0, float (&v)[4]) {
         if (E.act == ACT_SILU) {
 #pragma unroll
             for (int e = 0; e < 4; ++e) v[e] = silu_f(v[e]);
         }
+        stat4(j, v);
         if (E.out_f32) *reinterpret_cast<float4*>(reinterpret_cast<float*>(E.out) + (size_t)m * E.ldo + n0) = make_float4(v[0], v[1], v[2], v[3]);
         else store_bf16x4(reinterpret_cast<bf16*>(E.out) + (size_t)m * E.ldo + n0, v);
     };
-    auto epilogue = [&]() {
+    auto epilogue = [&](int hb_last) {
         const int mrow = m0 + wm * TM * 16 + l15;
         const int ncol = c_tn * BN + wn * TN * 16 + q * 4;
         if (hd.splits > 1) {
@@ -1762,6 +1866,12 @@
             bj[j] = make_float4(0.f, 0.f, 0.f, 0.f);
             if (E.bias) bj[j] = *reinterpret_cast<const float4*>(E.bias + ncol + j * 16);
         }
+        if constexpr (GP) {
+#pragma unroll
+            for (int j = 0; j < TN; ++j)
+#pragma unroll
+                for (int e = 0; e < 4; ++e) gs[j][e] = gq[j][e] = 0.f;
+        }
         if (E.bias2) {
 #pragma unroll
             for (int i = 0; i < TM; ++i) {
@@ -1774,7 +1884,7 @@
                 for (int j = 0; j < TN; ++j) {
                     float v[4] = {acc[i][j][0] + bj[j].x + b2[j].x, acc[i][j][1] + bj[j].y + b2[j].y,
                                   acc[i][j][2] + bj[j].z + b2[j].z, acc[i][j][3] + bj[j].w + b2[j].w};
-                    store_row(m, ncol + j * 16, v);
+                    store_row(m, j, ncol + j * 16, v);
                 }
             }
         } else if (E.res) {
@@ -1802,6 +1912,7 @@
                     } else {
                         store_bf16x4(reinterpret_cast<bf16*>(E.out) + (size_t)m * E.ldo + n0, v);
                     }
+                    stat4(j, v);
                 }
             }
         } else {
@@ -1811,7 +1922,35 @@
 #pragma unroll
                 for (int j = 0; j < TN; ++j) {
                     float v[4] = {acc[i][j][0] + bj[j].x, acc[i][j][1] + bj[j].y, acc[i][j][2] + bj[j].z, acc[i][j][3] + bj[j].w};
-                    store_row(m, ncol + j * 16, v);
+                    store_row(m, j, ncol + j * 16, v);
+                }
+            }
+        }
+        if constexpr (GP) {
+            float* sc = reinterpret_cast<float*>(smem + hb_last * HBUF + GPROW * 128);
+#pragma unroll
+            for (int j = 0; j < TN; ++j) {
+#pragma unroll
+                for (int e = 0; e < 4; ++e) { gs[j][e] = row16_sum(gs[j][e]); gq[j][e] = row16_sum(gq[j][e]); }
+                if (l15 == j) {
+                    *reinterpret_cast<float4*>(sc + wave * 2 * CB + j * 16 + q * 4) = make_float4(gs[j][0], gs[j][1], gs[j][2], gs[j][3]);
+                    *reinterpret_cast<float4*>(sc + wave * 2 * CB + CB + j * 16 + q * 4) = make_float4(gq[j][0], gq[j][1], gq[j][2], gq[j][3]);
+                }
+            }
+            __syncthreads();
+            const int cpg = gn_cpg, g = t >> 2, w = t & 3;
+            if (g * cpg < BN) {
+                const int c0 = g * cpg, wnr = c0 >= CB ? 1 : 0;
+                const float* ps = sc + (w * 2 + wnr) * 2 * CB + (c0 - wnr * CB);
+                float s = 0.f, qq = 0.f;
+                for (int c = 0; c < cpg; ++c) { s += ps[c]; qq += ps[CB + c]; }
+                s = dpp_add<0xB1>(s); qq = dpp_add<0xB1>(qq);
+                s = dpp_add<0x4E>(s); qq = dpp_add<0x4E>(qq);
+                if (w == 0) {
+                    const int lgHW = hd.lgW + hd.lgH;
+                    const int b = m0 >> lgHW, slot = (m0 & ((1 << lgHW) - 1)) >> 8, nslot = 1 << (lgHW - 8);
+                    float* dst = gn_partial + ((size_t)(b * nslot + slot) * 32 + (c_tn * BN) / cpg + g) * 2;
+                    *reinterpret_cast<float2*>(dst) = make_float2(s, qq);
                 }
             }
         }
@@ -1913,12 +2052,31 @@
         {
             const int nm0 = m0, ntn = c_tn, nz = c_z;
             m0 = done_m0; c_tn = done_tn; c_z = done_z;
-            epilogue();
+            epilogue(hb ^ 1);
             m0 = nm0; c_tn = ntn; c_z = nz;
         }
         if (!more) break;
         zero_acc();
     }
+#else
+template <int TN, int NW, bool GN = false>
+__global__ void __launch_bounds__(NW * 64, 1)
+conv_halo_kernel(AOperand A, const bf16* __restrict__ W, int M, int N, int K, EpilogueArgs E, float* __restrict__ ws, HaloDesc hd) {
+    constexpr bool GP = false;
+    constexpr float* gn_partial = nullptr;
+    constexpr int gn_cpg = 0;
+#define GL_CONV_HALO_BODY
+#include "gemm.hip"
+#undef GL_CONV_HALO_BODY
+}
+template <int TN, int NW>
+__global__ void __launch_bounds__(NW * 64, 1)
+conv_halo_gnstat_kernel(AOperand A, const bf16* __restrict__ W, int M, int N, int K, EpilogueArgs E, float* __restrict__ ws, HaloDesc hd,
+                        float* __restrict__ gn_partial, int gn_cpg) {
+    constexpr bool GN = false, GP = true;
+#define GL_CONV_HALO_BODY
+#include "gemm.hip"
+#undef GL_CONV_HALO_BODY
 }
 
 #ifndef GL_WIDE_NST
@@ -1926,7 +2084,7 @@
 #endif
 template <int TN>
 __global__ void __launch_bounds__(512, 1)
-gemm_wide_kernel(AOperand A, const bf16* __restrict__ W, int M, int N, int K, Epilogue E, float* __restrict__ ws, WideDesc wd) {
+gemm_wide_kernel(AOperand A, const bf16* __restrict__ W, int M, int N, int K, EpilogueArgs E, float* __restrict__ ws, WideDesc wd) {
     constexpr int TM = 4;
     constexpr int BM = 256;
     constexpr int BN = TN * 32;
@@ -2234,6 +2392,7 @@
 
 static thread_local GemmPlan t_last = [] { GemmPlan p{}; strcpy(p.name, "gemm"); return p; }();
 int gemm_last_stats_nb() { return t_last.stats_nb; }
+int gemm_last_gn_slots() { return t_last.gn_slots; }
 const char* gemm_last_kernel_name() { return t_last.name; }
 void gemm_last_cfg(int* tm, int* tn, int* splits) { *tm = t_last.tm; *tn = t_last.tn; *splits = t_last.splits; }
 static thread_local GemmLogEntry t_log[kGemmLogSize];
@@ -2249,7 +2408,7 @@
 namespace {
 
 struct Launch {
-    const AOperand& A; const bf16* W; int M, N, K; const Epilogue& E; float* ws;
+    const AOperand& A; const bf16* W; int M, N, K; const EpilogueArgs& E; float* ws;
     hipStream_t stream;
     template <auto KFN, class... Tail> int run(dim3 grid, int block, size_t lds, const Tail&... tail) const {
         return launch_lds<KFN>(grid, dim3(block), lds, stream, A, W, M, N, K, E, ws, tail...);
@@ -2286,13 +2445,21 @@
 int execute(const GemmPlan& p, const AOperand& A, const bf16* W, int M, int N, int K, const Epilogue& E_in, float* ws, hipStream_t stream) {
     Epilogue E = E_in;
     if ((p.family == GEMM_P || p.family == GEMM_U) && !p.stats_nb) E.stats_out = nullptr;
+    if (!p.gn_slots) E.gn_partial = nullptr;
+    const bool gnstat = p.gn_slots && p.splits == 1;
     const Launch l{A, W, M, N, K, E, ws, stream};
     int rc = set_error(GL_ERR_UNSUPPORTED, "gemm: unknown tile candidate");
     switch (p.family * 1000 + p.gn * 100 + p.tm * 10 + p.tn) {
         case GEMM_HALO * 1000 + 185: rc = l.run<conv_halo_kernel<5, 8, true>>(p.grid, 512, halo_lds(5, true), p.halo); break;
         case GEMM_HALO * 1000 + 184: rc = l.run<conv_halo_kernel<4, 8, true>>(p.grid, 512, halo_lds(4, true), p.halo); break;
-        case GEMM_HALO * 1000 + 85: rc = l.run<conv_halo_kernel<5, 8>>(p.grid, 512, halo_lds(5, false), p.halo); break;
-        case GEMM_HALO * 1000 + 84: rc = l.run<conv_halo_kernel<4, 8>>(p.grid, 512, halo_lds(4, false), p.halo); break;
+        case GEMM_HALO * 1000 + 85:
+            if (gnstat) rc = l.run<conv_halo_gnstat_kernel<5, 8>>(p.grid, 512, halo_lds(5, false), p.halo, E.gn_partial, E.gn_cpg);
+            else rc = l.run<conv_halo_kernel<5, 8>>(p.grid, 512, halo_lds(5, false), p.halo);
+            break;
+        case GEMM_HALO * 1000 + 84:
+            if (gnstat) rc = l.run<conv_halo_gnstat_kernel<4, 8>>(p.grid, 512, halo_lds(4, false), p.halo, E.gn_partial, E.gn_cpg);
+            else rc = l.run<conv_halo_kernel<4, 8>>(p.grid, 512, halo_lds(4, false), p.halo);
+            break;
         case GEMM_WIDE * 1000 + 85: rc = l.run<gemm_wide_kernel<5>>(p.grid, 512, wide_lds(5), p.wide); break;
         case GEMM_WIDE * 1000 + 84: rc = l.run<gemm_wide_kernel<4>>(p.grid, 512, wide_lds(4), p.wide); break;
         case GEMM_U * 1000 + 45: rc = exec_u<4, 5>(l, p); break;
@@ -2310,10 +2477,15 @@
         case GEMM_GLDS * 1000 + 41: rc = exec_glds<4, 1, 1, 1>(l, p); break;
     }
     GL_TRY(rc);
-    if (p.splits > 1) {
+    if (p.splits > 1 && p.gn_slots) {
+        const int lgHW = p.halo.lgW + p.halo.lgH;
+        if (p.tn == 5) hipLaunchKernelGGL(splitk_reduce_gn_kernel<80>, dim3(N / 80, M / 256), dim3(640), 0, stream, ws, p.splits, M, N, l.E, lgHW, E.gn_partial, E.gn_cpg);
+        else hipLaunchKernelGGL(splitk_reduce_gn_kernel<64>, dim3(N / 64, M / 256), dim3(512), 0, stream, ws, p.splits, M, N, l.E, lgHW, E.gn_partial, E.gn_cpg);
+        GL_LAUNCH_CHECK();
+    } else if (p.splits > 1) {
         int64_t total = (int64_t)M * (N / 4);
         int blocks = (int)fmin((double)cdiv64(total, 256), 4096.0);
-        hipLaunchKernelGGL(splitk_reduce_kernel, dim3(blocks), dim3(256), 0, stream, ws, p.splits, M, N, E);
+        hipLaunchKernelGGL(splitk_reduce_kernel, dim3(blocks), dim3(256), 0, stream, ws, p.splits, M, N, l.E);
         GL_LAUNCH_CHECK();
     }
     return GL_OK;
@@ -2376,6 +2548,7 @@
 int gemm_launch(const AOperand& A, const bf16* W, int M, int N, int K, const Epilogue& E_in, float* ws,
                 size_t ws_bytes, hipStream_t stream) {
     t_last.stats_nb = 0;
+    t_last.gn_slots = 0;
     Epilogue E = E_in;
     GemmPlan plan;
     GL_TRY(gemm_plan(A, M, N, K, E, ws != nullptr, ws_bytes, plan, [&](auto&&... a) { return tune(W, ws, stream, a...); }));
@@ -2392,3 +2565,4 @@
 }
 
 }
+#endif
diff --git a/gligen_amd/csrc/gemm_plan.h b/gligen_amd/csrc/gemm_plan.h
--- a/gligen_amd/csrc/gemm_plan.h
+++ b/gligen_amd/csrc/gemm_plan.h
@@ -30,6 +30,7 @@
     int autotune = 1, tune_reps = 3, corun = 0;
     bool no_table = false, tune_log = false;
     int force_tm = 0, force_tn = 0, force_splits = 0, force_grid = 0;
+    int gn_producer = 2;
 };
 GemmKnobs& gemm_knobs();
 void gemm_force_knobs(int halo_splits, int wide_splits, int wide_xcd, int xcd_boxes, int halo, int wide);
@@ -56,6 +57,7 @@
     int grid;
     union { WorkDesc work; HaloDesc halo; WideDesc wide; };
     int stats_nb;
+    int gn_slots;
     char name[96];
 };
 
diff --git a/gligen_amd/csrc/gemm_plan.hip b/gligen_amd/csrc/gemm_plan.hip
--- a/gligen_amd/csrc/gemm_plan.hip
+++ b/gligen_amd/csrc/gemm_plan.hip
@@ -14,7 +14,7 @@
         {"GL_GEMM_VARIANT", &GemmKnobs::variant}, {"GL_GEMM_WIDE", &GemmKnobs::wide}, {"GL_GEMM_WIDE_SPLITS", &GemmKnobs::wide_splits},
         {"GL_CONV_HALO", &GemmKnobs::halo}, {"GL_CONV_HALO_SPLITS", &GemmKnobs::halo_splits}, {"GL_GEMM_XCD_BOXES", &GemmKnobs::xcd_boxes},
         {"GL_WIDE_XCD", &GemmKnobs::wide_xcd}, {"GL_GEMM_AUTOTUNE", &GemmKnobs::autotune}, {"GL_GEMM_TUNE_REPS", &GemmKnobs::tune_reps},
-        {"GL_GEMM_TUNE_CORUN", &GemmKnobs::corun}};
+        {"GL_GEMM_TUNE_CORUN", &GemmKnobs::corun}, {"GL_GN_PRODUCER", &GemmKnobs::gn_producer}};
     GemmKnobs k;
     for (const auto& e : kInt)
         if (const char* v = dev_env(e.env)) k.*e.knob = atoi(v);
@@ -96,6 +96,15 @@
 
 bool gemm_gn_prologue_supported(const AOperand& A, int M, int N, int K, const Epilogue& E) {
     return K % 64 == 0 && gemm_route(A, M, N, K, E) == GEMM_HALO && (A.Hin * A.Win) % 256 == 0;
+}
+
+static bool gn_partial_shape_ok(const AOperand& A, int M, int N, const Epilogue& E) {
+    const int bn = N % 160 == 0 ? 160 : 128;
+    return !A.gn && E.rows_per_b == A.Hin * A.Win && M % E.rows_per_b == 0 && E.rows_per_b % 256 == 0 && E.rows_per_b > 256 && E.rows_per_b <= 64 * 256  && !E.out_f32 &&
+           E.gn_cpg > 0 && N == 32 * E.gn_cpg && bn % E.gn_cpg == 0 && (bn / 2) % E.gn_cpg == 0;
+}
+bool gemm_gn_partial_supported(const AOperand& A, int M, int N, int K, const Epilogue& E) {
+    return K % 64 == 0 && E.rows_per_b >= 1 && gemm_route(A, M, N, K, E) == GEMM_HALO && gn_partial_shape_ok(A, M, N, E);
 }
 
 bool gemm_upconv_phases_supported(const AOperand& A, int M, int N, int K, const Epilogue& E) {
@@ -217,7 +226,10 @@
     hd.n_items = tiles * hd.splits;
     p.tm = 8; p.tn = tn; p.gn = A.gn != nullptr; p.splits = hd.splits;
     p.grid = std::min(hd.n_items, 256);
-    snprintf(p.name, sizeof p.name, "conv_halo_kernel<%d, %d%s>%s", tn, 8, p.gn ? ", gn" : "", reduce_suffix(p.splits));
+    const int want = pb.E.gn_partial ? gemm_knobs().gn_producer : 0;
+    p.gn_slots = (want >= (hd.splits > 1 ? 2 : 1) && gn_partial_shape_ok(A, M, N, pb.E)) ? pb.E.rows_per_b / 256 : 0;
+    if (p.gn_slots) snprintf(p.name, sizeof p.name, hd.splits > 1 ? "conv_halo_kernel<%d, %d> + splitk_reduce_gn_kernel" : "conv_halo_gnstat_kernel<%d, %d>", tn, 8);
+    else snprintf(p.name, sizeof p.name, "conv_halo_kernel<%d, %d%s>%s", tn, 8, p.gn ? ", gn" : "", reduce_suffix(p.splits));
 }
 
 void plan_wide(const GemmProblem& pb, const GemmProblem& ph, GemmPlan& p) {
diff --git a/gligen_amd/csrc/norm.h b/gligen_amd/csrc/norm.h
--- a/gligen_amd/csrc/norm.h
+++ b/gligen_amd/csrc/norm.h
@@ -19,8 +19,10 @@
 int gn_nsplit(int HW);
 size_t gn_partial_bytes(int B, int HW);
 int groupnorm_launch(const GNParams& P, hipStream_t stream);
+int groupnorm_apply_launch(const GNParams& P, int nsplit, hipStream_t stream);
 int groupnorm_coef_launch(const GNParams& P, hipStream_t stream);
 int groupnorm_coef_launches(int HW, int C0, int C1);
+int groupnorm_coef_from_partial_launch(const GNParams& P, int nsplit, hipStream_t stream);
 inline size_t gn_coef_bytes(int B, int C) { return (size_t)B * C * 2 * sizeof(float); }
 
 struct LNParams {
diff --git a/gligen_amd/csrc/norm.hip b/gligen_amd/csrc/norm.hip
--- a/gligen_amd/csrc/norm.hip
+++ b/gligen_amd/csrc/norm.hip
@@ -332,6 +332,28 @@
     return (HW <= 256 && (C0 & 3) == 0 && (cpg & 3) == 0) ? 1 : 2;
 }
 
+int groupnorm_coef_from_partial_launch(const GNParams& P, int nsplit, hipStream_t stream) {
+    int cpg;
+    GL_TRY(gn_check(P, &cpg));
+    if (!P.coef || !P.partial || nsplit < 1 || nsplit > 64) return set_error(GL_ERR_ARG, "groupnorm_coef: %d slots of partials", nsplit);
+    hipLaunchKernelGGL(gn_coef_kernel, dim3(P.B), dim3(256), 0, stream, P, nsplit, cpg);
+    GL_LAUNCH_CHECK();
+    return GL_OK;
+}
+
+int groupnorm_apply_launch(const GNParams& P, int nsplit, hipStream_t stream) {
+    int cpg;
+    GL_TRY(gn_check(P, &cpg));
+    if (!P.partial || nsplit < 1 || nsplit > 64) return set_error(GL_ERR_ARG, "groupnorm_apply: %d slots of partials", nsplit);
+    const int C8 = (P.C0 + P.C1) / 8, R = gn_rows(C8), T = C8 * R;
+    const int trips = cdiv(P.HW, R * GN_UNR);
+    const int nblk = max(1, min(trips, max(1, 2048 / P.B)));
+    const int per = cdiv(cdiv(P.HW, nblk), R) * R;
+    hipLaunchKernelGGL(gn_apply_kernel, dim3(cdiv(P.HW, per), P.B), dim3(T), 0, stream, P, nsplit, C8, R, cpg, per);
+    GL_LAUNCH_CHECK();
+    return GL_OK;
+}
+
 int groupnorm_launch(const GNParams& P, hipStream_t stream) {
     const int C = P.C0 + P.C1;
     if (C % 64 != 0 || (P.C1 && P.C0 % 8 != 0)) return set_error(GL_ERR_ARG, "groupnorm: C=%d (C0=%d) unsupported", C, P.C0);
diff --git a/gligen_amd/engine.py b/gligen_amd/engine.py
--- a/gligen_amd/engine.py
+++ b/gligen_amd/engine.py
@@ -1151,6 +1151,18 @@
                                              _stream(self.device)))
         return y, bool(used.value)
 
+    def op_conv3x3_groupnorm(self, x0, w_oihw, bias, gamma, beta, eps, silu, x1=None, bias2=None, res=None, mode=-1):
+        B, H, W, C0 = x0.shape
+        C1 = 0 if x1 is None else x1.shape[3]
+        Cout = w_oihw.shape[0]
+        conv_out = torch.empty((B, H, W, Cout), device=x0.device, dtype=torch.bfloat16)
+        y = torch.empty_like(conv_out)
+        used = C.c_int(0)
+        check(self.lib.gl_op_conv3x3_groupnorm(self._ctx, _ptr(x0), C0, _ptr(x1), C1, B, H, W, _ptr(w_oihw), _ptr(bias), Cout, _ptr(bias2), _ptr(res),
+                                               _ptr(gamma), _ptr(beta), C.c_float(eps), int(silu), _ptr(conv_out), _ptr(y), int(mode), C.byref(used),
+                                               _stream(self.device)))
+        return conv_out, y, bool(used.value)
+
     def op_groupnorm(self, x0, gamma, beta, eps, silu, x1=None):
         B, HW, C0 = x0.shape
         C1 = 0 if x1 is None else x1.shape[2]
diff --git a/include/gligen_amd_gn_producer.h b/include/gligen_amd_gn_producer.h
--- /dev/null
+++ b/include/gligen_amd_gn_producer.h
@@ -0,0 +1,16 @@
+#ifndef GLIGEN_AMD_GN_PRODUCER_H
+#define GLIGEN_AMD_GN_PRODUCER_H
+#include "gligen_amd.h"
+
+#ifdef __cplusplus
+extern "C" {
+#endif
+
+int gl_op_conv3x3_groupnorm(gl_ctx* ctx, const void* x0, int C0, const void* x1, int C1, int B, int H, int W, const float* w_oihw, const float* bias,
+                            int Cout, const float* bias2, const void* res, const float* gamma, const float* beta, float eps, int silu,
+                            void* conv_out, void* y, int mode, int* used_producer, gl_stream s);
+
+#ifdef __cplusplus
+}
+#endif
+#endif
```

Measured after the change: 6.726 images/s (median of 6 runs). No clear change (+0.5%).
